# matpalm/cartpoleplusplus

Hardware: AMD Instinct MI355X
Metric: DDPG training steps/sec, 64x64x18 pixel obs, batch=256 (higher is better)
Workload: dtype f32-acc/f16x2,bf16x6

## Files before the change

### cartpoleplusplus_amd/_lib.py

```python
import ctypes as C
import os

import numpy as np

_HERE = os.path.dirname(os.path.abspath(__file__))
_variant = os.environ.get("CARTPOLEPP_ABLATION", "")
if _variant and not _variant.replace("_", "").isalnum():
    raise ImportError("cartpoleplusplus_amd: CARTPOLEPP_ABLATION=%r is not a build name" % _variant)
if _variant == "exact":
    raise ImportError("cartpoleplusplus_amd: CARTPOLEPP_ABLATION=exact names a build that no longer exists -- the exact-product "
                      "arithmetic is a mode of the release library (Context.set_precision('exact'), --exact-products, "
                      "bench.py --precision exact)")
LIB_PATH = os.path.join(_HERE, "lib", "libcartpolepp_hip%s.so" % (
    "" if _variant in ("", "0") else "_ablation" if _variant == "1" else "_" + _variant))

CPP_F32, CPP_F16, CPP_U8 = 0, 1, 2
CPP_ACTOR, CPP_CRITIC, CPP_HEAD = 0, 1, 2
CPP_OPT_SGD, CPP_OPT_MOMENTUM, CPP_OPT_ADAM = 0, 1, 2
CPP_PRECISION_FAST, CPP_PRECISION_EXACT = 0, 1


class NetSpec(C.Structure):
    _fields_ = [("kind", C.c_int32), ("pixel", C.c_int32), ("H", C.c_int32), ("W", C.c_int32),
                ("C", C.c_int32), ("state_elems", C.c_int32), ("action_dim", C.c_int32),
# ... 85 lines not shown
    "cpp_replay_set_n_step": (_I, [_P, _I, _F]),
    "cpp_replay_get_n_step": (_I, [_P, C.POINTER(_I), C.POINTER(_F)]),
    "cpp_replay_set_random_shift": (_I, [_P, _I, _I, _I, _U64]),
    "cpp_replay_get_random_shift": (_I, [_P, C.POINTER(_I), C.POINTER(_U64), C.POINTER(_U64)]),
    "cpp_replay_last_shifts": (_I, [_P, _I, _P]),
    "cpp_replay_gather_shifted": (_I, [_P, _I, _P, _I, _P]),
    "cpp_ddpg_create": (_I, [_P, _P, _P, _P, _P, C.POINTER(DdpgHyper), _PP]),
    "cpp_ddpg_destroy": (_I, [_P]),
    "cpp_ddpg_train_actor": (_I, [_P, _P]),
    "cpp_ddpg_train_critic": (_I, [_P, _P]),
    "cpp_ddpg_check_loss": (_I, [_P, _P, _P, _P, _P]),
    "cpp_ddpg_q_gradients_wrt_actions": (_I, [_P, _P, _P, _P, _P]),
    "cpp_ddpg_compute_gradients": (_I, [_P, _P]),
    "cpp_ddpg_grad_buffer": (_I, [_P, _PP, C.POINTER(_L)]),
    "cpp_ddpg_apply_gradients": (_I, [_P, _F]),
    "cpp_ddpg_update_targets": (_I, [_P]),
    "cpp_ddpg_set_optimiser": (_I, [_P, _I, _F, _F, _F, _F]),
    "cpp_ddpg_set_target_smoothing": (_I, [_P, _F, _F, _U64]),
    "cpp_ddpg_last_target_noise": (_I, [_P, _I, _P, C.POINTER(_U64)]),
    "cpp_ddpg_set_policy_delay": (_I, [_P, _I]),
    "cpp_ddpg_policy_delay_status": (_I, [_P, C.POINTER(_I), C.POINTER(_U64), C.POINTER(_I)]),
    "cpp_ddpg_opt_state_size": (_L, [_P]),
    "cpp_ddpg_get_opt_state": (_I, [_P, _P, _P, _L, _P]),
    "cpp_ddpg_set_opt_state": (_I, [_P, _P, _P, _L, _P]),
    "cpp_ddpg_train_step": (_I, [_P, _P, _I, _I, _P, _U64]),
    "cpp_ddpg_train_rows": (_I, [_P, _P, _I, _P]),
    "cpp_ddpg_sample_and_compute": (_I, [_P, _P, _I, _U64]),
    "cpp_ddpg_last_stats": (_I, [_P, _P]),
    "cpp_ddpg_last_values": (_I, [_P, _I, _P, _P, _P, _P]),
    "cpp_ddpg_last_twin_values": (_I, [_P, _I, _P, _P, _P, _P]),
    "cpp_ddpg_last_distribution": (_I, [_P, _I, _P, _P, _P]),
    "cpp_ddpg_set_quantile_target": (_I, [_P, C.c_float, _I]),
    "cpp_ddpg_last_quantiles": (_I, [_P, _I, _P, _P, _P]),
    "cpp_ddpg_set_sac": (_I, [_P, C.c_float, C.c_float, C.c_float, _U64]),
    "cpp_ddpg_last_sac": (_I, [_P, _I, _P, _P, _P, _P, _P, _P, _P, C.POINTER(C.c_float), C.POINTER(C.c_float), C.POINTER(_U64), _P]),
    "cpp_ddpg_sac_temperature": (_I, [_P, _I, C.POINTER(C.c_float), C.POINTER(C.c_float), C.POINTER(C.c_float), C.POINTER(_U64)]),
    "cpp_comm_unique_id": (_I, [_P, _I]),
    "cpp_comm_create": (_I, [_P, _P, _I, _I, _PP]),
    "cpp_comm_destroy": (_I, [_P]),
    "cpp_comm_info": (_I, [_P, C.POINTER(_I), C.POINTER(_I)]),
    "cpp_comm_allreduce": (_I, [_P, _P, _L, _I]),
    "cpp_comm_max_double": (_I, [_P, C.POINTER(C.c_double)]),
    "cpp_comm_max_doubles": (_I, [_P, C.POINTER(C.c_double), _I]),
    "cpp_comm_barrier": (_I, [_P]),
    "cpp_ddpg_allreduce_grads": (_I, [_P, _P]),
    "cpp_ddpg_average_params": (_I, [_P, _P]),
    "cpp_ddpg_dp_train_step": (_I, [_P, _P, _P, _I, _I, _U64, _I, _I]),
    "cpp_naf_sample_and_compute": (_I, [_P, _P, _I, _U64]),
    "cpp_naf_allreduce_grads": (_I, [_P, _P]),
    "cpp_naf_average_params": (_I, [_P, _P]),
    "cpp_naf_dp_train_step": (_I, [_P, _P, _P, _I, _I, _U64, _I]),
    "cpp_naf_clear_numeric_error": (_I, [_P]),
    "cpp_ddpg_dp_status": (_I, [_P, C.POINTER(_I), C.c_char_p, _I]),
    "cpp_naf_dp_status": (_I, [_P, C.POINTER(_I), C.c_char_p, _I]),
    "cpp_naf_create": (_I, [_P, _P, _P, _P, _P, _I, C.POINTER(NafHyper), _PP]),
    "cpp_naf_destroy": (_I, [_P]),
    "cpp_naf_action": (_I, [_P, _P, _I, _I, _P]),
    "cpp_naf_train": (_I, [_P, _P, C.POINTER(_F)]),
    "cpp_naf_debug_values": (_I, [_P, _P, _P, _P, _P, _P, _P]),
    "cpp_naf_compute_gradients": (_I, [_P, _P]),
    "cpp_naf_grad_buffer": (_I, [_P, _PP, C.POINTER(_L)]),
    "cpp_naf_apply_gradients": (_I, [_P, _F]),
    "cpp_naf_update_targets": (_I, [_P]),
    "cpp_naf_train_step": (_I, [_P, _P, _I, _I, _P, _U64]),
    "cpp_naf_train_rows": (_I, [_P, _P, _I, _P, C.POINTER(_F)]),
    "cpp_naf_train_rows_async": (_I, [_P, _P, _I, _P, C.POINTER(_U64)]),
    "cpp_naf_loss_wait": (_I, [_P, _U64, C.POINTER(_F)]),
    "cpp_naf_last_stats": (_I, [_P, _P]),
    "cpp_naf_opt_state_size": (_L, [_P]),
    "cpp_naf_get_opt_state": (_I, [_P, _P, _P, _L, C.POINTER(_U64)]),
    "cpp_naf_set_opt_state": (_I, [_P, _P, _P, _L, _U64]),
}


def _load():
    if not os.path.isfile(LIB_PATH):
        raise ImportError(
            "cartpoleplusplus_amd: %s not found. This package has no CPU fallback; build the HIP "
            "library first (python -c 'import __graft_entry__ as g; g.build()')." % LIB_PATH)
    lib = C.CDLL(LIB_PATH)
    for name, (res, args) in SIGNATURES.items():
        fn = getattr(lib, name)
        fn.restype, fn.argtypes = res, args
    if lib.cpp_abi_version() != 1:
        raise ImportError("cartpoleplusplus_amd: ABI version mismatch")
    return lib


lib = _load()


def check(rc):
    if rc != 0:
        raise RuntimeError((lib.cpp_last_error() or b"").decode("utf-8", "replace"))


def ptr(arr):
    if arr is None:
        return None
    assert arr.flags["C_CONTIGUOUS"]
    return arr.ctypes.data_as(C.c_void_p)


def as_state_array(x):
    x = np.asarray(x)
    if x.dtype == np.float16:
# ... 78 lines not shown
```

### cartpoleplusplus_amd/csrc/common.h

```cpp
#pragma once
#include <hip/hip_runtime.h>
#include <hip/hip_fp16.h>
#include <stdint.h>

typedef float f32x4 __attribute__((ext_vector_type(4)));

#ifdef CPP_ABLATION
#include <cstdlib>
inline bool cpp_switch_off(const char* name) { const char* v = getenv(name); return v != nullptr && atoi(v) == 0; }
inline bool cpp_switch_set(const char* name) { return getenv(name) != nullptr; }
inline int cpp_switch_int(const char* name, int dflt) { const char* v = getenv(name); return v ? atoi(v) : dflt; }
#else
constexpr bool cpp_switch_off(const char*) { return false; }
constexpr bool cpp_switch_set(const char*) { return false; }
constexpr int cpp_switch_int(const char*, int dflt) { return dflt; }
#endif

__host__ __device__ inline bool pair_grid_place(int i, int na, int nb, int order, int* idx) {
  if (order == 1) { if (i < nb) { *idx = i; return true; } *idx = i - nb; return false; }
  if (order == 2 && nb > 0 && na > 0) {
    const int k = (na + nb) / nb;
    const int head = nb * k;
    if (i < head) {
      if (i % k == 0) { *idx = i / k; return true; }
// ... 174 lines not shown
  const float* B; long sBk, sBn;
  float* C; long ldc;
  const float* Y; long ldy;
  int M, N, K, epi;
  int accumulate;
  float* C2; long ldc2;
  const uint64_t* drop_counter; uint32_t drop_seed, drop_layer;
  double* sq_part;
};
#define GEMM_BATCH_MAX 16
struct GemmBatch { GemmArgs g[GEMM_BATCH_MAX]; int tile_start[GEMM_BATCH_MAX + 1]; int n; };
#define CPP_MAX_DEVICES 16
static inline int cpp_dev_slot(const cpp_ctx* ctx) { return ctx->device >= 0 && ctx->device < CPP_MAX_DEVICES ? ctx->device : 0; }
#ifndef GEMM_SUB_MIN_K
#define GEMM_SUB_MIN_K 100000
#endif
static inline __host__ __device__ int gemm_sub(int M, int N, int K) { return (K >= GEMM_SUB_MIN_K && M > 16 && N > 16) ? 2 : 1; }
static inline int gemm_tiles(int M, int N, int K) { const int e = 16 * gemm_sub(M, N, K); return ((M + e - 1) / e) * ((N + e - 1) / e); }
int launch_gemm(cpp_ctx* ctx, const GemmArgs& g);
int launch_gemm_batch(cpp_ctx* ctx, const GemmArgs* list, int n);
int launch_copy_cols(cpp_ctx* ctx, float* dst, long ldd, int dcol0, const float* src, long lds_,
                     int scol0, int ncols, int rows);
int launch_fill(cpp_ctx* ctx, float* dst, long ld, int col0, int ncols, int rows, float v);
int launch_state_to_f32(cpp_ctx* ctx, float* dst, long ldd, const void* src, int dtype, long elems,
                        int rows);
int launch_actor_head_grad(cpp_ctx* ctx, float* dz, const float* dq_da, const float* act, int n);
int launch_td(cpp_ctx* ctx, const float* q, const float* tq, const float* r, const float* mask,
              float discount, int B, float* td, float* dq, float* loss, const float* w = nullptr);
int launch_td_twin(cpp_ctx* ctx, const float* q1, const float* q2, const float* tq1, const float* tq2, const float* r, const float* mask, float discount,
                   int B, float* td1, float* td2, float* dq1, float* dq2, float* loss, const float* w = nullptr);

struct GatherArgs {
  const void* store[2];
  const int32_t* s_idx[2];
  const int32_t* rows;
  int32_t* rows_out;
  const float* action; const float* reward; const float* mask;
  void* out_state[2];
  int32_t* out_slot[2];
  float* out_action; float* out_reward; float* out_mask;
  double* part;
  const double* slot_stats;
  uint64_t seed; const uint64_t* counter;
  int counter_add;
  const __half* lut;
  long elems; int B; int size; int action_dim; int C;
  const int32_t* size_ptr;
  const struct NStepWords* nstep;
  int rows_cap;
  struct ShiftWords* shift;
  int32_t* shifts_out;
  uint64_t shift_seed;
  int shift_pad, shift_H, shift_W, shift_C;
};
struct NStepWords { int32_t n; float discount; };
struct ShiftWords { uint64_t counter; uint32_t ticket; uint32_t reserved; };
constexpr int SHIFT_MAX_PAD = 16;
constexpr int NSTEP_MAX = 64;
int launch_gather_stats(cpp_ctx* ctx, const GatherArgs& a, int dtype);
int launch_slot_stats(cpp_ctx* ctx, const void* store, int dtype, long elems, int C, double* slot_stats, const int32_t* slots, int first, int n,
                      const __half* lut);
struct DwReduceBatch;
int launch_reduce_gather(cpp_ctx* ctx, const DwReduceBatch& rb, const GatherArgs& a, int dtype);
int launch_u8_to_f16(cpp_ctx* ctx, __half* dst, const uint8_t* src, long n, const __half* lut);
int launch_to_u8(cpp_ctx* ctx, uint8_t* dst, const void* src, int src_dtype, long n, const __half* lut, int* bad);
int launch_replay_fill_u8(cpp_ctx* ctx, uint8_t* store, long total, uint64_t seed);
struct BnNet {
  float* z;
  float* stat;
  const float* beta;
  float* pool; long pool_bstride; uint8_t* amax;
  const float* dpool; long dpool_bstride;
  double* part;
  float* means;
  float* dbeta;
};
struct BnBatch { BnNet n[CONV_BATCH_MAX]; int count; int B, H, W, C; };
size_t bn_part_doubles(int C);
int launch_bn_forward(cpp_ctx* ctx, const BnBatch& bb, double eps);
int launch_bn_backward(cpp_ctx* ctx, const BnBatch& bb);
void ctx_route_update(cpp_ctx* ctx);
int ctx_route_publish(cpp_ctx* ctx);
inline hipError_t ctx_sync_stream(cpp_ctx* ctx) {
  const hipError_t e = hipStreamSynchronize(ctx->stream);
  if (e == hipSuccess) ctx->route_done = ctx->route_calls;
  return e;
}
__device__ __forceinline__ void route_publish_device(unsigned* wmax_dev, const unsigned* tag_dev, unsigned long long* pin) {
  const unsigned m = *wmax_dev;
  *wmax_dev = 0u;
  const unsigned t = __hip_atomic_load(tag_dev, __ATOMIC_RELAXED, __HIP_MEMORY_SCOPE_SYSTEM);
  __hip_atomic_store(pin + (t & 1u), ((unsigned long long)t << 32) | (unsigned long long)m, __ATOMIC_RELAXED, __HIP_MEMORY_SCOPE_SYSTEM);
}
int launch_stats_finalize(cpp_ctx* ctx, const double* part, int nparts, int which_count, int C,
                          double count, float* white, double eps = 1e-6, uint64_t* bump = nullptr, unsigned* wmax = nullptr);
int launch_stats_generic(cpp_ctx* ctx, const void* x, int dtype, long npix, int C, float* white, double eps = 1e-6);
int launch_replay_fill(cpp_ctx* ctx, __half* store, long elems, int slots, int32_t* s1, int32_t* s2,
                       float* action, float* reward, float* mask, int rows, int action_dim,
                       uint64_t seed);
int launch_f32_to_f16(cpp_ctx* ctx, __half* dst, const float* src, long n);
int launch_counter_add(cpp_ctx* ctx, uint64_t* counter, uint64_t inc, const int* unless = nullptr);

enum OptKind { OPT_SGD = 0, OPT_MOMENTUM = 1, OPT_ADAM = 2 };
#define OPT_MAX_SEGS 4
struct OptSegs {
  float* p[OPT_MAX_SEGS]; const float* g[OPT_MAX_SEGS]; float* m[OPT_MAX_SEGS]; float* v[OPT_MAX_SEGS];
  long n[OPT_MAX_SEGS]; float lr[OPT_MAX_SEGS]; int group[OPT_MAX_SEGS];
  int nseg; int kind; float momentum, beta1, beta2, epsilon;
  const double* sq; int sq_begin[2], sq_count[2];
  const uint64_t* step;
  const uint64_t* step_seg[OPT_MAX_SEGS];
  uint64_t* bump;
  float* tgt[OPT_MAX_SEGS]; float tgt_coeff;
  unsigned* pub_wmax; const unsigned* pub_tag; unsigned long long* pub_pin;
  const int* skip_if;
  const double* st_part; float* st_white; int st_nparts, st_jobs, st_C; double st_count, st_eps; unsigned* st_wmax;
  int img_n; int img_cin;
  long img_skip[OPT_MAX_SEGS];
  struct { float* w; float* bias; const float* gw; const float* gb; unsigned char* rec; int seg, col, nout;
           const float* white; float* mw; float* mb; float* vw; float* vb; } img[4];
  uint64_t* bump2;
  const uint64_t* hold[OPT_MAX_SEGS];
};
__host__ __device__ inline float sgd_update(float p, float g, float scale, float lr) { return __builtin_fmaf(-lr, g * scale, p); }
__host__ __device__ inline float momentum_accum(float m, float g, float scale, float momentum) { return __builtin_fmaf(momentum, m, g * scale); }
__host__ __device__ inline float momentum_step(float p, float accum, float lr) { return __builtin_fmaf(-lr, accum, p); }
struct AdamElem { float p, m, v; };
__host__ __device__ inline AdamElem adam_update(float p, float g, float m, float v, float scale, float lr_t, float beta1, float beta2, float epsilon) {
  const float gi = g * scale;
  AdamElem e;
  e.m = __builtin_fmaf(beta1, m, (1.f - beta1) * gi);
  e.v = __builtin_fmaf(beta2, v, ((1.f - beta2) * gi) * gi);
  e.p = p - (lr_t * e.m) / (sqrtf(e.v) + epsilon);
  return e;
}
__host__ __device__ inline float adam_rate(float lr, float beta1, float beta2, uint64_t t) {
  const double td = (double)t;
  return (float)((double)lr * sqrt(1.0 - pow((double)beta2, td)) / (1.0 - pow((double)beta1, td)));
}
__host__ __device__ inline float soft_update_value(float t, float s, float coeff) { return __builtin_fmaf(-coeff, t - s, t); }
int launch_sumsq(cpp_ctx* ctx, const OptSegs& s, float grad_scale, double* part, int nparts);
int launch_opt_apply(cpp_ctx* ctx, const OptSegs& s, float grad_scale, float clip, const double* part,
                     int nparts, float* norms_out);
int launch_soft_update(cpp_ctx* ctx, float* t0, const float* s0, long n0, float* t1, const float* s1,
                       long n1, float coeff);

struct TpsArgs {
  const unsigned long long* n;
  float sigma, clip; unsigned seed_lo, seed_hi;
  float* eps;
  unsigned long long* n_out;
};
__device__ __forceinline__ float tps_noise(const TpsArgs& s, unsigned long long n, unsigned row, unsigned comp) {
  const u32x4 r = philox4x32_10(u32x4{row, 0x100u + comp, (uint32_t)n, (uint32_t)(n >> 32)}, s.seed_lo, s.seed_hi);
  const float u1 = (float)((r.x >> 8) + 1u) * 0x1p-24f;
  const float u2 = (float)(r.y >> 8) * 0x1p-24f;
  const float z = sqrtf(-2.f * logf(u1)) * cospif(2.f * u2);
  return fminf(fmaxf(s.sigma * z, -s.clip), s.clip);
}
__device__ __forceinline__ float tps_apply(float a, float eps) { return fminf(fmaxf(a + eps, -1.f), 1.f); }
int launch_tps_smooth(cpp_ctx* ctx, const TpsArgs& s, const float* in, int ld_in, float* out, int ld_out, int B, int A);

struct DdpgHeadsArgs {
  int B, A; float discount;
  const float *h2a, *h2ta; int ld_h2a, n2a;
  const float *Wo, *Wo_t;
  const float *h2c, *h2tc; int ld_h2c, n2c;
  const float *W3, *W3_t; int n3;
  const float *wq, *wq_t;
  const float *act, *r, *mask;
  float *a_out, *dq_da, *adz, *dz_h2a; int relu_x2;
  float* cat_splice;
  float* h3_out; int ld_h3;
  float *q_out, *tq_out, *td, *dzq, *dz3, *dz2c;
  double* loss_part;
// ... 131 lines not shown
```

### cartpoleplusplus_amd/csrc/conv_rs16.h

```cpp
#pragma once
#include "conv_k16.h"

template <int CIN, int NPCS = F16_PIECES>
struct Rs16Geom {
  static constexpr int KS = 5, P = 2, NO = KYO_NO, RK = 30;
  static constexpr int KROW = KS * CIN, NCH = (KROW + RK - 1) / RK, NPC = NPCS;
  static constexpr int NSET = KS + 1;
  static constexpr int NRC = 2 * P + 1;
  static constexpr int NUNIT = KS * NCH * 4 * 16;
  static constexpr int UNIT_BYTES = KS * NCH * NPC * 1024;
  static constexpr int CT_OFF = UNIT_BYTES;
  static constexpr int CT_BYTES = NRC * 5 * 16 * 4;
  static constexpr int PW_OFF = CT_OFF + CT_BYTES;
  static constexpr int PW_BYTES = NCH * 16 * 4;
  static constexpr int SC_OFF = PW_OFF + PW_BYTES;
  static constexpr int REC_BYTES = (SC_OFF + 16 + 255) & ~255;
};

struct Conv1ImageArgs {
  const float* w; const float* bias; const float* scale; const float* shift; float wscale; int nout; unsigned char* rec;
  const float* gw; const float* gb; float lr, gscale;
  float* mw; float* mb; float momentum;
  float* w_out; float* b_out;
  float* vw; float* vb; float beta1, beta2, epsilon;
};
struct Conv1ImageArgsN { Conv1ImageArgs a[CONV_BATCH_MAX]; int n; };

struct Conv1ImageNoPre { __device__ __forceinline__ float operator()(float gscale, float&) const { return gscale; } };
template <int CIN, int NPCS = F16_PIECES, typename Pre = Conv1ImageNoPre, bool ADAM = false>
__device__ __forceinline__ void conv1_image_body(const Conv1ImageArgs& a, unsigned char* lds_raw, Pre pre = Pre()) {
  typedef Rs16Geom<CIN, NPCS> G;
  constexpr int KS = G::KS, P = G::P, NO = G::NO, NCH = G::NCH, NPC = G::NPC, RK = G::RK;
  const int tid = threadIdx.x, lane = tid & 63, wave = tid >> 6;
  const int nout = a.nout;
  unsigned char* rec = lds_raw;
  double* mu = reinterpret_cast<double*>(lds_raw + G::REC_BYTES);
  constexpr int NU = KS * NCH * 4 * NO;
  double* opart = mu + ((CIN + 1) & ~1);
  constexpr int NB = 7 / CIN + 2;
  float* bpart = reinterpret_cast<float*>(opart + NU);
  float* scl = bpart + NU * NB;
  float* dmu = scl + CIN;
  float* red = dmu + CIN;
  float* ctab = red + 8;
  unsigned short* pivot = reinterpret_cast<unsigned short*>(ctab + G::NRC * NO * 4);
  constexpr int NUW = (NU + CONV_THREADS - 1) / CONV_THREADS;
  float* wst = reinterpret_cast<float*>(lds_raw);
  const int nwts = KS * G::KROW * nout;
  float gscale_b = a.gscale, lr = a.lr;
  {
    constexpr int NWT = (KS * G::KROW * NO + CONV_THREADS - 1) / CONV_THREADS;
    float wr[NWT], gr[NWT];
#pragma unroll
    for (int n = 0; n < NWT; ++n) { const int i = tid + n * CONV_THREADS; wr[n] = a.w[i < nwts ? i : 0]; }
    float mr[NWT];
    if (a.gw) {
#pragma unroll
      for (int n = 0; n < NWT; ++n) { const int i = tid + n * CONV_THREADS; gr[n] = a.gw[i < nwts ? i : 0]; }
      if (a.mw && !(ADAM && a.vw)) {
#pragma unroll
        for (int n = 0; n < NWT; ++n) { const int i = tid + n * CONV_THREADS; mr[n] = a.mw[i < nwts ? i : 0]; }
      }
    }
    const float gscale = pre(a.gscale, lr);
    gscale_b = gscale;
    if (ADAM && a.gw && a.vw) {
      float vr[NWT];
      int i0 = 0;
      asm volatile("" : "+v"(i0));
#pragma unroll
      for (int n = 0; n < NWT; ++n) { const int i = tid + n * CONV_THREADS; mr[n] = a.mw[i < nwts ? i : i0]; }
#pragma unroll
      for (int n = 0; n < NWT; ++n) { const int i = tid + n * CONV_THREADS; vr[n] = a.vw[i < nwts ? i : i0]; }
#pragma unroll
      for (int n = 0; n < NWT; ++n) {
        const int i = tid + n * CONV_THREADS;
        if (i < nwts) {
          const AdamElem e = adam_update(wr[n], gr[n], mr[n], vr[n], gscale, lr, a.beta1, a.beta2, a.epsilon);
          a.mw[i] = e.m; a.vw[i] = e.v;
          wst[i] = e.p;
          if (a.w_out) a.w_out[i] = e.p;
        }
        if ((n & 3) == 3) __builtin_amdgcn_sched_barrier(0);
      }
    } else {
#pragma unroll
    for (int n = 0; n < NWT; ++n) {
      const int i = tid + n * CONV_THREADS;
      if (i < nwts) {
        float w = wr[n];
        if (a.gw && a.mw) {
          const float acc = momentum_accum(mr[n], gr[n], gscale, a.momentum);
          a.mw[i] = acc;
          w = momentum_step(w, acc, lr);
        } else if (a.gw) w = sgd_update(w, gr[n], gscale, lr);
        wst[i] = w;
        if (a.gw && a.w_out) a.w_out[i] = w;
      }
    }
    }
  }
  __syncthreads();
  float wv[NUW][8];
  float vmax = 0.f;
#pragma unroll
  for (int n = 0; n < NUW; ++n) {
    const int u = tid + n * CONV_THREADS;
    const int o = u % NO, g = (u / NO) & 3, ch = (u / (4 * NO)) % NCH, ky = u / (4 * NO * NCH);
#pragma unroll
    for (int e = 0; e < 8; ++e) {
      const int kl = 8 * g + e, k = RK * ch + kl;
      const bool real = u < NU && o < nout && kl < RK && k < G::KROW;
      wv[n][e] = real ? wst[(ky * G::KROW + k) * nout + o] : 0.f;
    }
  }
  float* biasn = reinterpret_cast<float*>(pivot + ((CIN + 7) & ~7));
  if (tid < 16) {
    float bo = (a.bias && tid < nout) ? a.bias[tid] : 0.f;
    if (a.bias && a.gb && tid < nout) {
      if (ADAM && a.vb) { const AdamElem e = adam_update(bo, a.gb[tid], a.mb[tid], a.vb[tid], gscale_b, lr, a.beta1, a.beta2, a.epsilon); a.mb[tid] = e.m; a.vb[tid] = e.v; bo = e.p; }
      else if (a.mb) { const float acc = momentum_accum(a.mb[tid], a.gb[tid], gscale_b, a.momentum); a.mb[tid] = acc; bo = momentum_step(bo, acc, lr); }
      else bo = sgd_update(bo, a.gb[tid], gscale_b, lr);
      if (a.b_out) a.b_out[tid] = bo;
    }
    biasn[tid] = bo;
  }
  if (tid < CIN) {
    const float s_c = a.scale[tid], t_c = a.shift[tid];
    const double m_c = s_c != 0.f ? -(double)t_c / (double)s_c : 0.0;
    const _Float16 p_c = (_Float16)(float)m_c;
    mu[tid] = m_c;
    pivot[tid] = __builtin_bit_cast(unsigned short, p_c);
    scl[tid] = s_c;
    dmu[tid] = (float)((double)(float)p_c - m_c);
  }
  __syncthreads();
#pragma unroll
  for (int n = 0; n < NUW; ++n) {
    const int u = tid + n * CONV_THREADS;
    const int g = (u / NO) & 3, ch = (u / (4 * NO)) % NCH;
#pragma unroll
    for (int e = 0; e < 8; ++e) {
      float v = wv[n][e];
      v *= scl[(RK * ch + 8 * g + e) % CIN];
      if (a.wscale != 0.f) v *= a.wscale;
      wv[n][e] = v;
      vmax = fmaxf(vmax, fabsf(v));
    }
  }
  for (int o = 32; o > 0; o >>= 1) vmax = fmaxf(vmax, __shfl_xor(vmax, o));
  if (lane == 0) red[wave] = vmax;
  __syncthreads();
  vmax = fmaxf(fmaxf(red[0], red[1]), fmaxf(red[2], red[3]));
  for (int i = tid; i < G::REC_BYTES / 16; i += CONV_THREADS) reinterpret_cast<k16_u32x4*>(rec)[i] = (k16_u32x4){0u, 0u, 0u, 0u};
  __syncthreads();
  int S = 0;
  if (vmax > 0.f && vmax < 3.0e38f) S = 14 - ilogbf(vmax);
  S = S > 100 ? 100 : (S < -100 ? -100 : S);
  const float sc = ldexpf(1.f, S), inv = ldexpf(1.f, -S);
#pragma unroll
  for (int n = 0; n < NUW; ++n) {
    const int u = tid + n * CONV_THREADS;
    const int o = u % NO, g = (u / NO) & 3, ch = (u / (4 * NO)) % NCH, ky = u / (4 * NO * NCH);
    unsigned short pcs[3][8];
    double po = 0.0;
    float pb[NB];
#pragma unroll
    for (int b = 0; b < NB; ++b) pb[b] = 0.f;
    const int kx0 = (RK * ch + 8 * g) / CIN;
#pragma unroll
    for (int e = 0; e < 8; ++e) {
      const float v = wv[n][e] * sc;
      const _Float16 hh = (_Float16)v;
      const float r1 = v - (float)hh;
      const _Float16 mm = (_Float16)r1;
      const float r2 = r1 - (float)mm;
      const _Float16 ll = (_Float16)r2;
// ... 409 lines not shown
```

### cartpoleplusplus_amd/csrc/gather_body.h

```cpp
#pragma once
#include "common.h"
constexpr int GATHER_SH = 16;
constexpr int GATHER_LDS_BYTES = 256 * GATHER_SH * 4 + CPP_MAX_CHANNELS * 16 * 8 + 256 * 4;

__device__ __forceinline__ int sample_row(uint64_t seed, uint64_t counter, int b, int size) {
  u32x4 c = {(uint32_t)b, 0u, (uint32_t)counter, (uint32_t)(counter >> 32)};
  const u32x4 r = philox4x32_10(c, (uint32_t)seed, (uint32_t)(seed >> 32));
  return (int)(((uint64_t)r.x * (uint64_t)size) >> 32);
}

template <typename T> struct Vec8;
template <> struct Vec8<__half> {
  typedef __half Out;
  uint4 raw;
  __device__ void load(const __half* p) { raw = *reinterpret_cast<const uint4*>(p); }
  __device__ void store(__half* p) const { *reinterpret_cast<uint4*>(p) = raw; }
  __device__ float get(int e) const {
    const uint32_t w = e < 2 ? raw.x : (e < 4 ? raw.y : (e < 6 ? raw.z : raw.w));
    const unsigned short h = (e & 1) ? (unsigned short)(w >> 16) : (unsigned short)(w & 0xffffu);
    return __half2float(__ushort_as_half(h));
  }
};
template <> struct Vec8<uint8_t> {
  typedef __half Out;
// ... 129 lines not shown
      }
#pragma unroll
      for (int j = 0; j < NW; ++j) o[j] = __builtin_amdgcn_alignbit(m[j + 1], m[j], bits);
    }
    set_raw(x, o);
  }
  static __device__ __forceinline__ void set_raw(Vec8<__half>& x, const uint32_t* o) { x.raw = make_uint4(o[0], o[1], o[2], o[3]); }
  static __device__ __forceinline__ void set_raw(Vec8<uint8_t>& x, const uint32_t* o) { x.raw = make_uint2(o[0], o[1]); }
};

__device__ __forceinline__ void shift_draw(const GatherArgs& a, const int b, const int which, int* shw, int* dy, int* dx) {
  if (threadIdx.x == 0) {
    const uint64_t n = __hip_atomic_load(&a.shift->counter, __ATOMIC_RELAXED, __HIP_MEMORY_SCOPE_AGENT);
    u32x4 c = {(uint32_t)b, 2u + (uint32_t)which, (uint32_t)n, (uint32_t)(n >> 32)};
    const u32x4 r = philox4x32_10(c, (uint32_t)a.shift_seed, (uint32_t)(a.shift_seed >> 32));
    const uint64_t span = 2u * (uint32_t)a.shift_pad + 1u;
    const int y = (int)(((uint64_t)r.x * span) >> 32) - a.shift_pad, x = (int)(((uint64_t)r.y * span) >> 32) - a.shift_pad;
    shw[0] = y; shw[1] = x;
    a.shifts_out[((long)which * a.B + b) * 2] = y; a.shifts_out[((long)which * a.B + b) * 2 + 1] = x;
    const uint32_t ticket = __hip_atomic_fetch_add(&a.shift->ticket, 1u, __ATOMIC_ACQ_REL, __HIP_MEMORY_SCOPE_AGENT);
    if (ticket == 2u * (uint32_t)a.B - 1u) {
      __hip_atomic_store(&a.shift->counter, n + 1, __ATOMIC_RELAXED, __HIP_MEMORY_SCOPE_AGENT);
      __hip_atomic_store(&a.shift->ticket, 0u, __ATOMIC_RELAXED, __HIP_MEMORY_SCOPE_AGENT);
    }
  }
  __syncthreads();
  *dy = shw[0]; *dx = shw[1];
}

template <typename T, bool NSTEP = false, bool SHIFT = false>
__device__ __forceinline__ void gather_stats_body(const GatherArgs& a, const int b, const int which, float* sh, double* dsh, float* lut) {
  const int tid = threadIdx.x, lane = tid & 63, wave = tid >> 6;
  constexpr bool U8 = sizeof(T) == 1;
  if (U8) { lut[tid] = __half2float(a.lut[tid]); __syncthreads(); }
  typedef typename Vec8<T>::Out OutT;

  int row = 0, slot = 0;
  if (lane == 0) {
    if (a.s_idx[0] == nullptr) { row = b; slot = b; }
    else {
      row = a.rows ? a.rows[b] : sample_row(a.seed, (a.counter ? *a.counter : 0) + (uint64_t)a.counter_add, b, a.size_ptr ? *a.size_ptr : a.size);
      if (!NSTEP) slot = a.s_idx[which][row];
    }
  }
  row = __shfl(row, 0);
  slot = __shfl(slot, 0);
  float nreward = 0.f, nmask = 0.f;
  if (NSTEP && a.s_idx[0] != nullptr) nstep_walk(a, row, which, lane, &slot, &nreward, &nmask);
  int shift_dy = 0, shift_dx = 0;
  if constexpr (SHIFT) shift_draw(a, b, which, reinterpret_cast<int*>(dsh), &shift_dy, &shift_dx);

  if (tid == 0 && a.out_slot[which]) a.out_slot[which][b] = slot;
  if (which == 0 && a.s_idx[0] != nullptr) {
    if (tid == 0 && a.rows_out) a.rows_out[b] = row;
    if (tid < a.action_dim) a.out_action[(long)b * a.action_dim + tid] = a.action[(long)row * a.action_dim + tid];
    if (tid == 64) a.out_reward[b] = NSTEP ? nreward : a.reward[row];
    if (tid == 65) a.out_mask[b] = NSTEP ? nmask : a.mask[row];
  }

  const T* src = (const T*)a.store[which] + (long)slot * a.elems;
  OutT* dst = a.out_state[which] ? (OutT*)a.out_state[which] + (long)b * a.elems : nullptr;
  const long nvec = a.elems >> 3;
  const int C = a.C;

  if (a.slot_stats != nullptr && dst == nullptr && C > 0) {
    if (tid < 2 * C) a.part[((long)which * a.B + b) * 2 * C + tid] = a.slot_stats[(long)slot * 2 * C + tid];
    return;
  }

  if (C <= 0) {
    for (long v = tid; v < nvec; v += 256) { Vec8<T> x; vec_init(x, lut); x.load(src + v * 8); if (dst) x.store(dst + v * 8); }
    for (long e = nvec * 8 + tid; e < a.elems; e += 256) if (dst) dst[e] = elem_convert<T, OutT>(src[e], lut);
    return;
  }

  const int P = C / gcd_int(8, C);
  const int act = (64 / P) * P;
  double s[8], ss[8];
#pragma unroll
  for (int e = 0; e < 8; ++e) { s[e] = 0.0; ss[e] = 0.0; }
  if constexpr (SHIFT) {
    if (lane < act) {
      constexpr int GU = 6;
      ShiftGeom g;
      g.L = a.shift_W * a.shift_C; g.H = a.shift_H; g.C = a.shift_C; g.dy = shift_dy; g.dxC = shift_dx * a.shift_C; g.nvec = nvec;
#pragma unroll
      for (int e = 0; e < 8; ++e) g.ch[e] = (8 * (wave * act + lane) + e) % a.shift_C;
      long v = wave * act + lane;
      const long stride = 4 * act;
      for (; v + (GU - 1) * stride < nvec; v += GU * stride) {
        ShiftVec<T> s0, s1, s2, s3, s4, s5;
        static_assert(GU == 6, "one ShiftVec per vector in flight");
        s0.issue(src, g, v); s1.issue(src, g, v + stride); s2.issue(src, g, v + 2 * stride);
        s3.issue(src, g, v + 3 * stride); s4.issue(src, g, v + 4 * stride); s5.issue(src, g, v + 5 * stride);
        auto finish = [&](const ShiftVec<T>& sv, const long vo) __attribute__((always_inline)) {
          Vec8<T> x;
          vec_init(x, lut);
          sv.finish(x);
          x.store(dst + vo * 8);
#pragma unroll
          for (int e = 0; e < 8; ++e) { const double f = (double)x.get(e); s[e] += f; ss[e] = fma(f, f, ss[e]); }
        };
        finish(s0, v); finish(s1, v + stride); finish(s2, v + 2 * stride);
        finish(s3, v + 3 * stride); finish(s4, v + 4 * stride); finish(s5, v + 5 * stride);
      }
      for (; v < nvec; v += stride) {
        ShiftVec<T> sv;
// ... 67 lines not shown
```

### cartpoleplusplus_amd/csrc/optim.hip

```cpp
#include "common.h"
#include "stats_body.h"
#include "conv_rs16.h"

constexpr int OPT_THREADS = 256;
static_assert(OPT_THREADS == CONV_THREADS, "conv1_image_body (the rider in opt_apply_kernel) strides its loops by CONV_THREADS and assumes four waves");

__global__ __launch_bounds__(OPT_THREADS) void sumsq_kernel(const OptSegs s, float grad_scale,
                                                            double* part, int nparts) {
  __shared__ double red[OPT_THREADS];
  const int seg = blockIdx.y;
  const float* g = s.g[seg];
  const long n = s.n[seg];
  double acc = 0.0;
  const long stride = (long)nparts * OPT_THREADS;
  long i = (long)blockIdx.x * OPT_THREADS + threadIdx.x;
  for (; i + 7 * stride < n; i += 8 * stride) {
    float v[8];
#pragma unroll
    for (int u = 0; u < 8; ++u) v[u] = g[i + u * stride] * grad_scale;
#pragma unroll
    for (int u = 0; u < 8; ++u) acc += (double)v[u] * (double)v[u];
  }
  for (; i < n; i += stride) {
    const float v = g[i] * grad_scale;
    acc += (double)v * (double)v;
  }
  red[threadIdx.x] = acc;
  __syncthreads();
  for (int o = OPT_THREADS / 2; o > 0; o >>= 1) {
    if (threadIdx.x < o) red[threadIdx.x] += red[threadIdx.x + o];
    __syncthreads();
  }
  if (threadIdx.x == 0) part[seg * nparts + blockIdx.x] = red[0];
}

int launch_sumsq(cpp_ctx* ctx, const OptSegs& s, float grad_scale, double* part, int nparts) {
  prof_begin(ctx);
  hipLaunchKernelGGL(sumsq_kernel, dim3(nparts, s.nseg), dim3(OPT_THREADS), 0, ctx->stream, s, grad_scale,
                     part, nparts);
  LAUNCH_CHECK();
  prof_end(ctx, K_SUMSQ);
  return 0;
}

__device__ __forceinline__ double lane_sum_f64(const double* q, const int count, const int lane, double tot = 0.0) {
  for (int i = lane; i < count; i += 8 * 64) {
    double v[8];
#pragma unroll
    for (int u = 0; u < 8; ++u) { const int j = i + 64 * u; v[u] = q[j < count ? j : i]; }
#pragma unroll
    for (int u = 0; u < 8; ++u) tot += (i + 64 * u < count) ? v[u] : 0.0;
  }
  return tot;
}

template <bool ADAM>
__global__ __launch_bounds__(OPT_THREADS) void opt_apply_kernel(const OptSegs s, float grad_scale,
                                                                float clip, const double* part,
                                                                int nparts, float* norms_out) {
  __shared__ float sh_scale, sh_lr;
  const int seg = blockIdx.y;
  if (s.img_n > 0 && seg == s.nseg + (s.st_part ? 1 : 0)) {
    if ((int)blockIdx.x >= s.img_n) return;
    extern __shared__ __attribute__((aligned(16))) unsigned char img_lds[];
    __shared__ float wh[2 * CPP_MAX_CHANNELS];
    const int j = blockIdx.x, ws = s.img[j].seg;
    const float* const gwj = (s.hold[ws] && *s.hold[ws]) ? nullptr : s.img[j].gw;
    auto pre = [&](float, float& lr_io) __attribute__((always_inline)) -> float {
      if (gwj) {
        double tot = 0.0;
        if (threadIdx.x < 64) {
          if (s.sq) {
            const int gr = s.group[ws];
            const double* q = s.sq + s.sq_begin[gr];
            tot = lane_sum_f64(q, s.sq_count[gr], (int)threadIdx.x);
          } else {
            for (int k = 0; k < s.nseg; ++k)
              if (s.group[k] == s.group[ws])
                tot = lane_sum_f64(part + k * nparts, nparts, (int)threadIdx.x, tot);
          }
          for (int o = 32; o > 0; o >>= 1) tot += __shfl_xor(tot, o);
        }
        if (threadIdx.x == 0) {
          const float norm = (float)sqrt(tot);
          float sc = 1.f;
          if (clip > 0.f) sc = clip * fminf(1.f / norm, 1.f / clip);
          sh_scale = sc * grad_scale;
          if (ADAM) sh_lr = adam_rate(s.lr[ws], s.beta1, s.beta2, *(s.step_seg[ws] ? s.step_seg[ws] : s.step));
        }
      }
      if (s.img[j].white) {
        if ((int)threadIdx.x < 2 * s.img_cin) wh[threadIdx.x] = s.img[j].white[threadIdx.x];
      } else {
        constexpr int NW = OPT_THREADS / 64, MAXC = (18 + NW - 1) / NW, MAXR = 8;
        const int wv = (int)(threadIdx.x >> 6), ln = (int)(threadIdx.x & 63), C = s.st_C, np_ = s.st_nparts;
        if (np_ <= 64 * MAXR) {
          double v[MAXC][MAXR][2];
#pragma unroll
          for (int k = 0; k < MAXC; ++k) {
            const int c = wv + NW * k;
#pragma unroll
            for (int r = 0; r < MAXR; ++r) {
              const int b = ln + 64 * r;
              const bool ok = c < C && b < np_;
              const double* q = s.st_part + ((long)s.img[j].col * np_ + (ok ? b : 0)) * 2 * C;
              v[k][r][0] = ok ? q[c] : 0.0; v[k][r][1] = ok ? q[C + c] : 0.0;
            }
          }
#pragma unroll
          for (int k = 0; k < MAXC; ++k) {
            const int c = wv + NW * k;
            double a0 = 0.0, a1 = 0.0;
#pragma unroll
            for (int r = 0; r < MAXR; ++r) if (ln + 64 * r < np_) { a0 += v[k][r][0]; a1 += v[k][r][1]; }
            for (int o = 32; o > 0; o >>= 1) { a0 += __shfl_xor(a0, o); a1 += __shfl_xor(a1, o); }
            if (ln == 0 && c < C) white_from_moments(a0, a1, s.st_count, s.st_eps, &wh[c], &wh[C + c]);
          }
        } else {
          for (int c = wv; c < C; c += NW)
            stats_finalize_wave_to(s.st_part, np_, C, s.st_count, &wh[c], &wh[C + c], s.st_eps, s.img[j].col, c, ln);
        }
      }
      __syncthreads();
      if (ADAM && gwj) lr_io = sh_lr;
      return gwj ? sh_scale : 0.f;
    };
    Conv1ImageArgs ia;
    ia.w = s.img[j].w; ia.bias = s.img[j].bias; ia.scale = wh; ia.shift = wh + s.img_cin; ia.wscale = 0.f; ia.nout = s.img[j].nout; ia.rec = s.img[j].rec;
    ia.gw = gwj; ia.gb = s.img[j].gb; ia.lr = gwj ? s.lr[ws] : 0.f; ia.gscale = 0.f;
    ia.w_out = gwj ? s.img[j].w : nullptr; ia.b_out = gwj ? s.img[j].bias : nullptr;
    const bool slots = gwj && (ADAM || s.kind == OPT_MOMENTUM), adam = ADAM && gwj;
    ia.mw = slots ? s.img[j].mw : nullptr; ia.mb = slots ? s.img[j].mb : nullptr; ia.momentum = s.momentum;
    ia.vw = adam ? s.img[j].vw : nullptr; ia.vb = adam ? s.img[j].vb : nullptr; ia.beta1 = s.beta1; ia.beta2 = s.beta2; ia.epsilon = s.epsilon;
    switch (s.img_cin) {
      case 3: conv1_image_body<3, F16_PIECES, decltype(pre), ADAM>(ia, img_lds, pre); break;
      case 6: conv1_image_body<6, F16_PIECES, decltype(pre), ADAM>(ia, img_lds, pre); break;
      case 9: conv1_image_body<9, F16_PIECES, decltype(pre), ADAM>(ia, img_lds, pre); break;
      case 12: conv1_image_body<12, F16_PIECES, decltype(pre), ADAM>(ia, img_lds, pre); break;
      default: conv1_image_body<18, F16_PIECES, decltype(pre), ADAM>(ia, img_lds, pre); break;
    }
    return;
  }
  if (s.st_part && seg == s.nseg) {
    const int job = (int)blockIdx.x * (OPT_THREADS / 64) + (int)(threadIdx.x >> 6);
    if (job < s.st_jobs) stats_finalize_wave(s.st_part, s.st_nparts, s.st_C, s.st_count, s.st_white, s.st_eps, job, (int)(threadIdx.x & 63), s.st_wmax);
    return;
  }
  if (s.skip_if && *s.skip_if) return;
  double tot = 0.0;
  if (threadIdx.x < 64) {
    if (s.sq) {
      const int gr = s.group[seg];
      const double* q = s.sq + s.sq_begin[gr];
      tot = lane_sum_f64(q, s.sq_count[gr], (int)threadIdx.x);
    } else {
      for (int k = 0; k < s.nseg; ++k)
        if (s.group[k] == s.group[seg])
          tot = lane_sum_f64(part + k * nparts, nparts, (int)threadIdx.x, tot);
    }
    for (int o = 32; o > 0; o >>= 1) tot += __shfl_xor(tot, o);
  }
  if (threadIdx.x == 0) {
    const float norm = (float)sqrt(tot);
    float sc = 1.f;
    if (clip > 0.f) sc = clip * fminf(1.f / norm, 1.f / clip);
    sh_scale = sc * grad_scale;
    float lr = s.lr[seg];
    if (ADAM) lr = adam_rate(lr, s.beta1, s.beta2, *(s.step_seg[seg] ? s.step_seg[seg] : s.step));
    sh_lr = lr;
    if (blockIdx.x == 0 && norms_out && s.n[seg] > 0) norms_out[s.group[seg]] = norm;
    if (blockIdx.x == 0 && seg == 0 && s.bump) *s.bump += 1;
    if (blockIdx.x == 0 && seg == 0 && s.bump2) *s.bump2 += 1;
    if (blockIdx.x == 0 && seg == 0 && s.pub_wmax) route_publish_device(s.pub_wmax, s.pub_tag, s.pub_pin);
  }
  __syncthreads();
  const float sc = sh_scale, lr = sh_lr;
  const long skip = s.img_n > 0 ? s.img_skip[seg] : 0;
  float* p = s.p[seg] + skip;
  const float* g = s.g[seg] + skip;
  const long n = s.n[seg] - skip;
  const long stride = (long)gridDim.x * OPT_THREADS;
  float* tp = s.tgt[seg] ? s.tgt[seg] + skip : nullptr;
  const float tc = s.tgt_coeff;
  if (s.hold[seg] && *s.hold[seg]) {
    if (tp)
      for (long i = (long)blockIdx.x * OPT_THREADS + threadIdx.x; i < n; i += stride) tp[i] = soft_update_value(tp[i], p[i], tc);
    return;
  }
  if (!ADAM && s.kind == OPT_SGD) {
    long i = (long)blockIdx.x * OPT_THREADS + threadIdx.x;
    for (; i + 3 * stride < n; i += 4 * stride) {
      float pv[4], gv[4], tv[4];
#pragma unroll
      for (int u = 0; u < 4; ++u) { pv[u] = p[i + u * stride]; gv[u] = g[i + u * stride]; if (tp) tv[u] = tp[i + u * stride]; }
#pragma unroll
      for (int u = 0; u < 4; ++u) {
        const float pn = sgd_update(pv[u], gv[u], sc, lr);
        p[i + u * stride] = pn;
        if (tp) tp[i + u * stride] = soft_update_value(tv[u], pn, tc);
      }
    }
    for (; i < n; i += stride) {
      const float pn = sgd_update(p[i], g[i], sc, lr);
      p[i] = pn;
      if (tp) tp[i] = soft_update_value(tp[i], pn, tc);
    }
  } else if (!ADAM) {
    float* m = s.m[seg] + skip;
    for (long i = (long)blockIdx.x * OPT_THREADS + threadIdx.x; i < n; i += stride) {
      const float acc = momentum_accum(m[i], g[i], sc, s.momentum);
      m[i] = acc;
      const float pn = momentum_step(p[i], acc, lr);
      p[i] = pn;
      if (tp) tp[i] = soft_update_value(tp[i], pn, tc);
    }
  } else {
    float* m = s.m[seg] + skip;
    float* v = s.v[seg] + skip;
    const float b1 = s.beta1, b2 = s.beta2;
    long i = (long)blockIdx.x * OPT_THREADS + threadIdx.x;
    for (; i + 3 * stride < n; i += 4 * stride) {
      float pv[4], gv[4], mv[4], vv[4], tv[4];
#pragma unroll
      for (int u = 0; u < 4; ++u) {
        pv[u] = p[i + u * stride]; gv[u] = g[i + u * stride]; mv[u] = m[i + u * stride]; vv[u] = v[i + u * stride];
        if (tp) tv[u] = tp[i + u * stride];
      }
#pragma unroll
      for (int u = 0; u < 4; ++u) {
        const AdamElem e = adam_update(pv[u], gv[u], mv[u], vv[u], sc, lr, b1, b2, s.epsilon);
        m[i + u * stride] = e.m; v[i + u * stride] = e.v; p[i + u * stride] = e.p;
        if (tp) tp[i + u * stride] = soft_update_value(tv[u], e.p, tc);
      }
    }
    for (; i < n; i += stride) {
      const AdamElem e = adam_update(p[i], g[i], m[i], v[i], sc, lr, b1, b2, s.epsilon);
      m[i] = e.m; v[i] = e.v; p[i] = e.p;
      if (tp) tp[i] = soft_update_value(tp[i], e.p, tc);
    }
  }
}

static_assert(Rs16ImageLds<18>::BYTES >= Rs16ImageLds<12>::BYTES && Rs16ImageLds<18>::BYTES >= Rs16ImageLds<9>::BYTES &&
              Rs16ImageLds<18>::BYTES >= Rs16ImageLds<6>::BYTES && Rs16ImageLds<18>::BYTES >= Rs16ImageLds<3>::BYTES, "the rider's LDS is sized for the largest instance");
int launch_opt_apply(cpp_ctx* ctx, const OptSegs& s, float grad_scale, float clip, const double* part,
                     int nparts, float* norms_out) {
  prof_begin(ctx);
  const bool img = s.img_n > 0 && (s.st_part || s.img[0].white);
  const size_t lds = img ? (size_t)Rs16ImageLds<18>::BYTES : 0;
  if (img) {
    if ((s.kind != OPT_SGD && s.kind != OPT_MOMENTUM && s.kind != OPT_ADAM) || (s.st_part && s.st_C != s.img_cin) || !conv_rs16_channels_ok(s.img_cin) || s.skip_if) {
      cpp_set_error("opt_apply: the conv1 image rider needs a known optimiser kind and a channel count conv_rs16.h is instantiated for (%d)", s.img_cin); return 1;
    }
    static bool attr_done[CPP_MAX_DEVICES] = {};
    if (!attr_done[cpp_dev_slot(ctx)]) {
      HIP_CHECK(hipFuncSetAttribute((const void*)opt_apply_kernel<false>, hipFuncAttributeMaxDynamicSharedMemorySize, (int)Rs16ImageLds<18>::BYTES));
      HIP_CHECK(hipFuncSetAttribute((const void*)opt_apply_kernel<true>, hipFuncAttributeMaxDynamicSharedMemorySize, (int)Rs16ImageLds<18>::BYTES));
      attr_done[cpp_dev_slot(ctx)] = true;
    }
  }
  hipLaunchKernelGGL(s.kind == OPT_ADAM ? opt_apply_kernel<true> : opt_apply_kernel<false>, dim3(128, s.nseg + (s.st_part ? 1 : 0) + (img ? 1 : 0)), dim3(OPT_THREADS), lds, ctx->stream, s, grad_scale,
                     clip, part, nparts, norms_out);
  LAUNCH_CHECK();
  prof_end(ctx, K_CLIP_SGD);
  return 0;
}

__global__ void soft_update_kernel(float* t0, const float* s0, long n0, float* t1, const float* s1,
                                   long n1, float coeff, unsigned* wmax_dev, const unsigned* tag_dev, unsigned long long* pin) {
  if (wmax_dev && blockIdx.x == 0 && blockIdx.y == 0 && threadIdx.x == 0) route_publish_device(wmax_dev, tag_dev, pin);
  float* t = blockIdx.y == 0 ? t0 : t1;
  const float* s = blockIdx.y == 0 ? s0 : s1;
  const long n = blockIdx.y == 0 ? n0 : n1;
  for (long i = (long)blockIdx.x * blockDim.x + threadIdx.x; i < n; i += (long)gridDim.x * blockDim.x) t[i] = soft_update_value(t[i], s[i], coeff);
}

int launch_soft_update(cpp_ctx* ctx, float* t0, const float* s0, long n0, float* t1, const float* s1,
                       long n1, float coeff) {
  prof_begin(ctx);
  const bool pub = ctx->route_rider && ctx->route_pin_dev != nullptr;
  ctx->route_rider = false;
  hipLaunchKernelGGL(soft_update_kernel, dim3(128, t1 ? 2 : 1), dim3(256), 0, ctx->stream, t0, s0, n0,
                     t1, s1, n1, coeff, pub ? ctx->white_max_dev : nullptr, ctx->route_tag_dev, ctx->route_pin_dev);
  LAUNCH_CHECK();
  prof_end(ctx, K_SOFT_UPDATE);
  return 0;
}
```

### cartpoleplusplus_amd/csrc/rt_core.cpp

```cpp
#include "rt_internal.h"

static thread_local char g_err[1024] = "";

void cpp_set_error(const char* fmt, ...) {
  va_list ap;
  va_start(ap, fmt);
  vsnprintf(g_err, sizeof(g_err), fmt, ap);
  va_end(ap);
}

extern "C" const char* cpp_last_error(void) { return g_err; }

#include <map>
#include <mutex>
static std::mutex g_arena_mu;
static std::map<const char*, size_t> g_arena_blocks;
void cpp_arena_register(const void* raw, size_t bytes) {
  std::lock_guard<std::mutex> lk(g_arena_mu);
  g_arena_blocks[(const char*)raw] = bytes;
}
void cpp_arena_unregister(const void* raw) {
  std::lock_guard<std::mutex> lk(g_arena_mu);
  g_arena_blocks.erase((const char*)raw);
}
// ... 119 lines not shown
    *last_max_scale = m;
  }
  return CPP_OK;
}
extern "C" int cpp_ctx_set_precision(cpp_ctx* c, int mode) {
  ARG_CHECK(c, "cpp_ctx_set_precision: ctx is NULL");
  ARG_CHECK(mode == CPP_PRECISION_FAST || mode == CPP_PRECISION_EXACT, "cpp_ctx_set_precision: mode %d is neither CPP_PRECISION_FAST nor CPP_PRECISION_EXACT", mode);
  ARG_CHECK(c->n_trainers == 0 || mode == c->precision,
            "cpp_ctx_set_precision: %d trainer(s) exist on this ctx (their step graphs hold the kernels of the current mode): set the mode first", c->n_trainers);
  c->precision = mode;
  return CPP_OK;
}

extern "C" int cpp_ctx_get_precision(cpp_ctx* c, int* mode) {
  ARG_CHECK(c && mode, "cpp_ctx_get_precision: NULL argument");
  *mode = c->precision;
  return CPP_OK;
}

extern "C" int cpp_ctx_destroy(cpp_ctx* c) {
  if (!c) return CPP_OK;
  (void)hipSetDevice(c->device);
  (void)hipStreamSynchronize(c->stream);
  (void)hipEventDestroy(c->t0); (void)hipEventDestroy(c->t1);
  (void)hipEventDestroy(c->pe0); (void)hipEventDestroy(c->pe1);
  if (c->sq_part) (void)hipFree(c->sq_part);
  if (c->white_max_dev) (void)hipFree(c->white_max_dev);
  if (c->route_tag_dev) (void)hipFree(c->route_tag_dev);
  if (c->route_pin) { (void)hipHostFree(c->route_pin); for (hipEvent_t e : c->route_ev) (void)hipEventDestroy(e); }
  if (c->own_stream) (void)hipStreamDestroy(c->stream);
  delete c;
  return CPP_OK;
}

extern "C" int cpp_sync(cpp_ctx* c) {
  ARG_CHECK(c, "cpp_sync: ctx is NULL");
  HIP_CHECK(ctx_sync_stream(c));
  return CPP_OK;
}

void StepGraph::drop() {
  if (e) { (void)hipGraphExecDestroy(e); e = nullptr; }
  if (g) { (void)hipGraphDestroy(g); g = nullptr; }
  ok = false;
}
int StepGraph::capture(cpp_ctx* ctx, const GraphKey& k, const std::function<int()>& body) {
  drop();
  HIP_CHECK(hipStreamBeginCapture(ctx->stream, hipStreamCaptureModeThreadLocal));
  int rc = body();
  const hipError_t err = hipStreamEndCapture(ctx->stream, &g);
  if (!rc && err != hipSuccess) { cpp_set_error("hipStreamEndCapture -> %s", hipGetErrorString(err)); rc = CPP_ERR_HIP; }
  if (!rc) rc = [this]() -> int { HIP_CHECK(hipGraphInstantiate(&e, g, nullptr, nullptr, 0)); return CPP_OK; }();
  if (rc) { drop(); return rc; }
  key = k; ok = true;
  return CPP_OK;
}
int StepGraph::launch(cpp_ctx* ctx) {
  HIP_CHECK(hipGraphLaunch(e, ctx->stream));
  return CPP_OK;
}
int StepGraph::rebuild(cpp_ctx* ctx, const GraphKey& k, const std::function<int()>& body, StepRan* ran) {
  drop();
  RC(body());
  HIP_CHECK(ctx_sync_stream(ctx));
  const int rc = capture(ctx, k, body);
  *ran = rc ? STEP_CAPTURE_FAILED : STEP_CAPTURED;
  return rc;
}
int dp_graph_refused(DpGraph& D, const char* learner) {
  (void)hipGetLastError();
  D.graph.drop();
  D.refused = true;
  snprintf(D.reason, sizeof(D.reason), "%s", cpp_last_error());
  fprintf(stderr, "cartpolepp: the data-parallel %s step could not be captured as a hipGraph (%s); running it as stream launches\n", learner, D.reason);
  return CPP_OK;
}

extern "C" int cpp_timer_begin(cpp_ctx* c) {
  ARG_CHECK(c, "ctx is NULL");
  HIP_CHECK(hipEventRecord(c->t0, c->stream));
  return CPP_OK;
}
extern "C" int cpp_timer_end(cpp_ctx* c, float* ms) {
  ARG_CHECK(c && ms, "ctx/ms is NULL");
  HIP_CHECK(hipEventRecord(c->t1, c->stream));
  HIP_CHECK(hipEventSynchronize(c->t1));
  HIP_CHECK(hipEventElapsedTime(ms, c->t0, c->t1));
  return CPP_OK;
}
extern "C" int cpp_prof_enable(cpp_ctx* c, int on) { ARG_CHECK(c, "ctx is NULL"); c->prof = on != 0; return CPP_OK; }
extern "C" int cpp_prof_reset(cpp_ctx* c) {
  ARG_CHECK(c, "ctx is NULL");
  memset(c->prof_ms, 0, sizeof(c->prof_ms)); memset(c->prof_n, 0, sizeof(c->prof_n));
  return CPP_OK;
}
extern "C" int cpp_prof_num_kernels(void) { return K_NUM_KERNELS; }
extern "C" const char* cpp_prof_kernel_name(int k) { return (k >= 0 && k < K_NUM_KERNELS) ? kKernelNames[k] : ""; }
extern "C" int cpp_prof_read(cpp_ctx* c, int k, double* total_ms, int64_t* launches) {
  ARG_CHECK(c && k >= 0 && k < K_NUM_KERNELS, "cpp_prof_read: bad kernel id %d", k);
  if (total_ms) *total_ms = c->prof_ms[k];
  if (launches) *launches = c->prof_n[k];
  return CPP_OK;
}
```

### cartpoleplusplus_amd/csrc/rt_ddpg.cpp

```cpp
#include "rt_internal.h"


struct cpp_ddpg {
  cpp_ctx* ctx; cpp_net *actor, *critic, *tactor, *tcritic; cpp_ddpg_hyper hp;
  int maxB; long nA, nC;
  float* gradbuf; float *dq_da, *td, *dq, *loss_norms , *ones;
  double* norm_part;
  double* heads_part;
  int heads_grid, heads_B;
  int loss_parts, loss_B;
  StepGraph graph;
  cpp_batch* step_batch;
  StepGraph rgraph;
  uint64_t graph_gen = 0;
  uint64_t epoch;
  bool publish_in_apply;
  bool targets_in_apply, targets_applied;
  DpGraph dgraph;
  struct HalfGraphs { StepGraph g[3][2]; int next[3] = {0, 0, 0}; } hg[2];
  GraphKey half_key; uint64_t h_write_gen;
  uint64_t dp_local;
  int sq_cnt[2];
  int pre_variant;
  int32_t* slot_set[2][2];
  const float* per_w; std::function<int()> per_hook;
  int opt_kind; float opt_momentum, opt_beta1, opt_beta2, opt_epsilon;
  float *opt_m, *opt_v; uint64_t* opt_step;
  bool bump_in_heads;
  bool step_bumped;
  bool tps_on; float tps_sigma, tps_clip; uint64_t tps_seed; uint64_t* tps_n; float *tps_eps, *tps_act;
  bool tps_pending;
  int pd_d; uint64_t* pd;
  Arena arena;
  bool twin = false; float* td2 = nullptr;
  int dist_n = 0; float *dist_p = nullptr, *dist_tp = nullptr, *dist_m = nullptr;
  bool quant = false; float quant_kappa = 1.f; int quant_drop = 0;
  bool sac = false; float sac_hbar = 0.f, sac_lr = 0.f; uint64_t sac_seed = 0;
  float* sac_w = nullptr; uint64_t* sac_step = nullptr; double* sac_part = nullptr; int sac_B = 0;
  float *sac_eps[2] = {nullptr, nullptr}, *sac_logp[2] = {nullptr, nullptr}, *sac_rsoft = nullptr;
};

static SacSampleArgs sac_sample_args(const cpp_ddpg* d, bool target, bool draw, const cpp_batch* b = nullptr) {
  const cpp_net* n = target ? d->tactor : d->actor;
  SacSampleArgs s; memset(&s, 0, sizeof(s));
  s.logits = n->ws[0].logits; s.A = n->spec.action_dim; s.lo = n->ls_lo; s.hi = n->ls_hi;
  s.n = draw ? (const unsigned long long*)d->tps_n : nullptr;
  s.stream = target ? 0x300u : 0x200u; s.seed_lo = (unsigned)d->sac_seed; s.seed_hi = (unsigned)(d->sac_seed >> 32);
  s.eps = d->sac_eps[target ? 1 : 0]; s.a_out = n->ws[0].out; s.logp = d->sac_logp[target ? 1 : 0];
  if (target) {
    s.n_out = draw ? (unsigned long long*)(d->tps_n + 1) : nullptr;
    s.log_alpha = d->sac_w + SAC_W_TARGET; s.r = b->r; s.mask = b->m; s.discount = d->hp.discount; s.r_soft = d->sac_rsoft;
  }
  return s;
}
static SacGradArgs sac_grad_args(const cpp_ddpg* d, int B) {
  const cpp_net* a = d->actor;
  SacGradArgs g; memset(&g, 0, sizeof(g));
  g.logits = a->ws[0].logits; g.a = a->ws[0].out; g.eps = d->sac_eps[0]; g.dq_da = d->dq_da; g.logp = d->sac_logp[0];
  g.log_alpha = d->sac_w + SAC_W_LOG_ALPHA; g.B = B; g.A = a->spec.action_dim; g.lo = a->ls_lo; g.hi = a->ls_hi; g.target_entropy = d->sac_hbar;
  g.dz = a->ws[0].dz[a->fc.size() - 1]; g.part = d->sac_part; g.alpha_out = d->sac_w + SAC_W_ALPHA;
  return g;
}
static int sac_sync_target(cpp_ddpg* d) {
  hipStream_t st = d->ctx->stream;
  if (d->tactor != d->actor)
    HIP_CHECK(hipMemcpyAsync(d->tactor->params, d->actor->params, (size_t)d->nA * sizeof(float), hipMemcpyDeviceToDevice, st));
  HIP_CHECK(hipMemcpyAsync(d->sac_w + SAC_W_TARGET, d->sac_w + SAC_W_LOG_ALPHA, sizeof(float), hipMemcpyDeviceToDevice, st));
  d->tactor->wimg_key = nullptr;
  return CPP_OK;
}
static void reconfigured(cpp_ddpg* d);
static int sac_configure(cpp_ddpg* d, float init_temperature, float target_entropy, float lr, uint64_t seed) {
  cpp_ctx* ctx = d->ctx;
  HIP_CHECK(ctx_sync_stream(ctx));
  float w[SAC_WORDS]; memset(w, 0, sizeof(w));
  w[SAC_W_LOG_ALPHA] = w[SAC_W_TARGET] = logf(init_temperature); w[SAC_W_ALPHA] = init_temperature;
  HIP_CHECK(hipMemcpyAsync(d->sac_w, w, sizeof(w), hipMemcpyHostToDevice, ctx->stream));
// ... 3 lines not shown
  HIP_CHECK(ctx_sync_stream(ctx));
  d->sac_hbar = target_entropy; d->sac_lr = lr; d->sac_seed = seed; d->sac_B = 0; d->tps_pending = false;
  reconfigured(d);
  return CPP_OK;
}

static float loss_of_parts(const double* parts, int n, int B) {
  double s = 0.0;
  for (int i = 0; i < n; ++i) s += parts[i];
  return (float)(s / (double)B);
}

static int dist_td(cpp_ddpg* d, const cpp_batch* b, int B, bool backward, const float* w) {
  cpp_net *c = d->critic, *tc = d->tcritic;
  if (d->quant)
    return launch_quant_td(d->ctx, c->ws[0].logits, tc->ws[0].logits, b->r, b->m, d->hp.discount, B, d->dist_n, d->quant_kappa, d->quant_drop,
                           c->ws[0].out, tc->ws[0].out, d->dist_p, d->dist_tp, d->dist_m, d->td, backward ? c->ws[0].dz[c->fc.size() - 1] : nullptr,
                           d->heads_part, w);
  return launch_dist_td(d->ctx, c->ws[0].logits, tc->ws[0].logits, b->r, b->m, d->hp.discount, B, d->dist_n, c->dist_vmin, c->dist_vmax,
                        c->ws[0].out, tc->ws[0].out, d->dist_p, d->dist_tp, d->dist_m, d->td, backward ? c->ws[0].dz[c->fc.size() - 1] : nullptr,
                        d->heads_part, w);
}

extern "C" int cpp_ddpg_create(cpp_ctx* ctx, cpp_net* actor, cpp_net* critic, cpp_net* tactor, cpp_net* tcritic,
                               const cpp_ddpg_hyper* hp, cpp_ddpg** out) {
  ARG_CHECK(ctx && actor && critic && tactor && tcritic && hp && out, "cpp_ddpg_create: NULL argument");
  ARG_CHECK(actor->spec.kind == CPP_ACTOR && tactor->spec.kind == CPP_ACTOR, "cpp_ddpg_create: actor kinds");
  ARG_CHECK(critic->spec.kind == CPP_CRITIC && tcritic->spec.kind == CPP_CRITIC, "cpp_ddpg_create: critic kinds");
  ARG_CHECK(!actor->twin && !tactor->twin, "cpp_ddpg_create: a twin actor");
  ARG_CHECK(critic->twin == tcritic->twin, "cpp_ddpg_create: a twin critic needs a twin target critic (and a plain one a plain one)");
  ARG_CHECK(!actor->dist_n && !tactor->dist_n, "cpp_ddpg_create: a distributional actor");
  ARG_CHECK(critic->dist_n == tcritic->dist_n && critic->dist_vmin == tcritic->dist_vmin && critic->dist_vmax == tcritic->dist_vmax,
            "cpp_ddpg_create: critic and target critic must carry one value distribution (N, v_min, v_max), or none");
  ARG_CHECK(!(critic->dist_n && critic->twin), "cpp_ddpg_create: a distributional critic with twin Q heads");
  ARG_CHECK(critic->quant == tcritic->quant, "cpp_ddpg_create: a quantile critic needs a quantile target critic with the same N (never a categorical or a plain one)");
  ARG_CHECK(actor->gauss == tactor->gauss && actor->ls_lo == tactor->ls_lo && actor->ls_hi == tactor->ls_hi,
            "cpp_ddpg_create: a Gaussian actor needs a Gaussian target actor with the same log std bounds (and a plain one a plain one)");
  ARG_CHECK(!(actor->gauss && critic->dist_n), "cpp_ddpg_create: a Gaussian actor with a distributional or quantile critic");
  for (cpp_net* n : {actor, critic, tactor, tcritic})
    ARG_CHECK(!(actor->gauss && (n->spec.use_batch_norm || n->spec.use_dropout)), "cpp_ddpg_create: a Gaussian actor with batch norm or dropout");
  ARG_CHECK(actor->nparams == tactor->nparams && critic->nparams == tcritic->nparams, "cpp_ddpg_create: target shapes differ");
  ARG_CHECK(actor->state_elems == critic->state_elems && actor->spec.action_dim == critic->spec.action_dim,
            "cpp_ddpg_create: actor/critic input shapes differ");
  HIP_CHECK(hipSetDevice(ctx->device));
  cpp_ddpg* d = new cpp_ddpg();
  d->arena.stream = ctx->stream;
  d->ctx = ctx; d->actor = actor; d->critic = critic; d->tactor = tactor; d->tcritic = tcritic; d->hp = *hp;
  d->maxB = actor->maxB < critic->maxB ? actor->maxB : critic->maxB;
  d->nA = actor->nparams; d->nC = critic->nparams;
  d->step_batch = nullptr;
  d->epoch = ctx->kernel_epoch;
  d->dp_local = 0; d->sq_cnt[0] = d->sq_cnt[1] = 0;
  d->h_write_gen = 0; d->pre_variant = 0;
  memset(d->slot_set, 0, sizeof(d->slot_set));
  d->heads_grid = d->heads_B = d->loss_parts = d->loss_B = 0;
  d->per_w = nullptr;
  d->opt_kind = OPT_SGD; d->opt_momentum = 0.f; d->opt_beta1 = 0.9f; d->opt_beta2 = 0.999f; d->opt_epsilon = 1e-8f;
  d->opt_m = d->opt_v = nullptr; d->opt_step = nullptr; d->bump_in_heads = d->step_bumped = false;
  d->pd_d = 1; d->pd = nullptr;
  d->tps_on = d->tps_pending = false; d->tps_sigma = d->tps_clip = 0.f; d->tps_seed = 0; d->tps_n = nullptr; d->tps_eps = d->tps_act = nullptr;
  const int A = actor->spec.action_dim;
  int rc = dalloc(d->arena, &d->gradbuf, (size_t)(d->nA + d->nC));
  if (!rc) rc = dalloc(d->arena, &d->dq_da, (size_t)d->maxB * A);
  if (!rc) rc = dalloc(d->arena, &d->td, (size_t)d->maxB);
  if (!rc) rc = dalloc(d->arena, &d->dq, (size_t)d->maxB);
  if (!rc) rc = dalloc(d->arena, &d->ones, (size_t)d->maxB);
  if (!rc) rc = dalloc(d->arena, &d->loss_norms, (size_t)4);
  if (!rc) rc = dalloc(d->arena, &d->norm_part, (size_t)OPT_MAX_SEGS * NORM_PARTS);
  if (!rc) rc = dalloc(d->arena, &d->heads_part, (size_t)DDPG_HEADS_MAX_WGS);
  d->twin = critic->twin;
  if (!rc && d->twin) rc = dalloc(d->arena, &d->td2, (size_t)d->maxB);
  d->dist_n = critic->dist_n; d->quant = critic->quant;
  if (d->dist_n && dist_td_grid(d->maxB) > DDPG_HEADS_MAX_WGS) {
    cpp_set_error("cpp_ddpg_create: a distributional trainer takes batches up to %d (got %d)", 4 * DDPG_HEADS_MAX_WGS, d->maxB);
    rc = CPP_ERR_ARG;
  }
  for (float** p : {&d->dist_p, &d->dist_tp, &d->dist_m})
    if (!rc && d->dist_n) rc = dalloc(d->arena, p, (size_t)d->maxB * d->dist_n);
  d->sac = actor->gauss;
  if (d->sac && sac_grid(d->maxB) > DDPG_HEADS_MAX_WGS) {
    cpp_set_error("cpp_ddpg_create: a soft actor-critic trainer takes batches up to %d (got %d)", 4 * DDPG_HEADS_MAX_WGS, d->maxB);
    rc = CPP_ERR_ARG;
  }
  if (d->sac) {
    if (!rc) rc = dalloc(d->arena, &d->sac_w, (size_t)SAC_WORDS);
    if (!rc) rc = dalloc(d->arena, &d->sac_step, (size_t)1);
    if (!rc) rc = dalloc(d->arena, &d->tps_n, (size_t)2);
    if (!rc) rc = dalloc(d->arena, &d->sac_part, (size_t)DDPG_HEADS_MAX_WGS);
    if (!rc) rc = dalloc(d->arena, &d->sac_rsoft, (size_t)d->maxB);
    for (int k = 0; k < 2; ++k) {
      if (!rc) rc = dalloc(d->arena, &d->sac_eps[k], (size_t)d->maxB * A);
      if (!rc) rc = dalloc(d->arena, &d->sac_logp[k], (size_t)d->maxB);
    }
    if (!rc) rc = sac_configure(d, 0.1f, -(float)A, 1e-4f, 0);
  }
  if (!rc) rc = launch_fill(ctx, d->ones, 1, 0, 1, d->maxB, 1.0f);
  if (rc) { d->arena.release(); delete d; return rc; }
  actor->grads = d->gradbuf; critic->grads = d->gradbuf + d->nA;
  HIP_CHECK(ctx_sync_stream(ctx));
  ctx->n_trainers += 1;
  *out = d;
  return CPP_OK;
}

static void invalidate_graphs(cpp_ddpg* d) { ++d->graph_gen; }
static void reconfigured(cpp_ddpg* d) { invalidate_graphs(d); d->pre_variant = 0; }

static void after_replay(cpp_ddpg* d, bool step) {
  if (step) d->pre_variant = 0;
  d->loss_parts = d->heads_grid; d->loss_B = d->heads_B;
}
static int step_ran(cpp_ddpg* d, int rc, StepRan how) {
  if (!rc && how == STEP_REPLAYED) after_replay(d, true);
  return rc;
}

static void route_check(cpp_ddpg* d) {
  if (route_check(d->ctx, &d->epoch, &d->graph_gen, {d->actor, d->critic, d->tactor, d->tcritic})) d->pre_variant = 0;
}

extern "C" int cpp_ddpg_destroy(cpp_ddpg* d) {
  if (!d) return CPP_OK;
  (void)hipSetDevice(d->ctx->device);
  (void)ctx_sync_stream(d->ctx);
  if (d->step_batch) cpp_batch_destroy(d->step_batch);
  d->actor->grads = nullptr; d->critic->grads = nullptr;
  d->ctx->n_trainers -= 1;
  d->arena.release(); delete d; return CPP_OK;
}

static int check_batch(cpp_ddpg* d, cpp_batch* b, const char* who) {
  ARG_CHECK(d && b, "%s: NULL argument", who);
  ARG_CHECK(b->B >= 1 && b->B <= d->maxB, "%s: batch size %d outside [1,%d]", who, b->B, d->maxB);
  ARG_CHECK(b->elems == d->actor->state_elems && b->A == d->actor->spec.action_dim, "%s: batch shape does not match the networks", who);
  return CPP_OK;
}

static TpsArgs tps_args(const cpp_ddpg* d) {
  TpsArgs t; memset(&t, 0, sizeof(t));
  if (!d->tps_on) return t;
  t.n = (const unsigned long long*)d->tps_n; t.n_out = (unsigned long long*)(d->tps_n + 1); t.eps = d->tps_eps;
  t.sigma = d->tps_sigma; t.clip = d->tps_clip; t.seed_lo = (unsigned)d->tps_seed; t.seed_hi = (unsigned)(d->tps_seed >> 32);
  return t;
}
static int tps_settle(cpp_ddpg* d, int rc) {
  const bool owed = d->tps_pending;
  d->tps_pending = false;
  if (rc) return rc;
  return owed ? launch_counter_add(d->ctx, d->tps_n, 1) : CPP_OK;
}

const float* white_of(cpp_batch* b, int which, int C) { return b->white + (long)which * 2 * C; }

static int critic_prefix(cpp_net* c, const void* state, int dtype, const float* white, int B) {
  RC(net_forward_trunk(c, c->ws[0], state, dtype, white, B));
  if (c->cat_layer > 0) {
    for (int l = 0; l < c->cat_layer; ++l) {
      const FcL& L = c->fc[l];
      RC(gemm(c->ctx, c->ws[0].fcin[l], L.n_in + 1, 1, c->params + L.w_off, L.n_out, 1, c->ws[0].fcin[l + 1],
              c->fc[l + 1].n_in + 1, B, L.n_out, L.n_in + 1, L.act));
    }
  }
// ... 53 lines not shown
static int critic_gradients(cpp_ddpg* d, cpp_batch* b, bool critic_prefix_done, bool backward) {
  cpp_net* nets[3] = {d->critic, d->tactor, d->tcritic};
  for (cpp_net* n : nets) n->is_training = backward;
  const int rc = critic_gradients_impl(d, b, critic_prefix_done, backward);
  for (cpp_net* n : nets) n->is_training = true;
  return rc;
}
static int critic_gradients_impl(cpp_ddpg* d, cpp_batch* b, bool critic_prefix_done, bool backward) {
  cpp_net *c = d->critic, *ta = d->tactor, *tc = d->tcritic;
  const int B = b->B, C = c->spec.pixel ? c->spec.C : 0;
  const float *w1 = white_of(b, 0, C), *w2 = white_of(b, 1, C);
  RC(net_forward_trunk(ta, ta->ws[0], b->s[1], b->dtype, w2, B));
  RC(net_forward_fc(ta, ta->ws[0], 0, B, nullptr));
  RC(critic_prefix(tc, b->s[1], b->dtype, w2, B));
  const float* tact = ta->ws[0].out;
  if (d->sac) {
    SacSampleArgs st = sac_sample_args(d, true, backward, b); st.B = B;
    RC(launch_sac_sample(d->ctx, st));
    if (backward) d->tps_pending = true;
  }
  const float* rw = d->sac ? d->sac_rsoft : b->r;
  if (backward && d->tps_on) {
    const int A = ta->spec.action_dim;
    RC(launch_tps_smooth(d->ctx, tps_args(d), tact, A, d->tps_act, A, B, A));
    tact = d->tps_act;
    d->tps_pending = true;
  }
  RC(critic_head(tc, 0, tact, B));
  if (!critic_prefix_done) RC(critic_prefix(c, b->s[0], b->dtype, w1, B));
  RC(critic_head(c, 0, b->a, B));
  const int last = (int)c->fc.size() - 1;
  if (d->dist_n) {
    RC(dist_td(d, b, B, backward, nullptr));
    d->loss_parts = dist_td_grid(B); d->loss_B = B;
    if (backward) RC(net_backward(c, c->ws[0], B, true, nullptr, b->s[0], b->dtype, w1));
    return CPP_OK;
  }
  if (d->twin)
    RC(launch_td_twin(d->ctx, c->ws[0].out, c->ws[0].out2, tc->ws[0].out, tc->ws[0].out2, rw, b->m, d->hp.discount, B, d->td, d->td2,
                      backward ? c->ws[0].dz[last] : nullptr, backward ? c->ws[0].dz2[last] : nullptr, d->loss_norms));
  else
  RC(launch_td(d->ctx, c->ws[0].out, tc->ws[0].out, rw, b->m, d->hp.discount, B, d->td,
               backward ? c->ws[0].dz[last] : nullptr, d->loss_norms));
  d->loss_parts = 0;
  if (backward) RC(net_backward(c, c->ws[0], B, true, nullptr, b->s[0], b->dtype, w1));
  return CPP_OK;
}

static int apply(cpp_ddpg* d, bool do_actor, bool do_critic, float grad_scale, uint64_t* bump = nullptr, bool folded = false,
                 const NextBatch& nx = NextBatch()) {
  OptSegs s; memset(&s, 0, sizeof(s));
  s.bump = bump;
  if (d->tps_pending) { s.bump2 = d->tps_n; d->tps_pending = false; }
  if (d->targets_in_apply && !nx.b && do_actor && do_critic) {
    s.tgt[0] = d->tactor->params; s.tgt[1] = d->tcritic->params; s.tgt_coeff = d->hp.target_update_rate;
    d->tactor->wimg_key = nullptr; d->tcritic->wimg_key = nullptr;
    d->targets_applied = true;
  }
  d->targets_in_apply = false;
  if (d->publish_in_apply && !nx.b && d->ctx->route_pin_dev) {
    s.pub_wmax = d->ctx->white_max_dev; s.pub_tag = d->ctx->route_tag_dev; s.pub_pin = d->ctx->route_pin_dev;
  }
  d->publish_in_apply = false;
  opt_next_stats(d->ctx, s, nx);
  d->actor->wimg_key = nullptr; d->critic->wimg_key = nullptr;
  s.nseg = 2; s.kind = d->opt_kind;
  const bool bumped = d->step_bumped;
  d->step_bumped = false;
  const bool pd_on = d->pd_d > 1;
  if (pd_on && do_actor) s.hold[0] = d->pd + PD_HOLD;
  if (pd_on && !bumped)
    RC(launch_pd_tick(d->ctx, d->pd, (unsigned)d->pd_d, s.kind != OPT_SGD ? d->opt_step : nullptr, do_actor, do_critic, do_actor && !do_critic));
  if (s.kind != OPT_SGD) {
    s.momentum = d->opt_momentum; s.beta1 = d->opt_beta1; s.beta2 = d->opt_beta2; s.epsilon = d->opt_epsilon;
    s.m[0] = d->opt_m; s.m[1] = d->opt_m + d->nA; s.v[0] = d->opt_v; s.v[1] = d->opt_v ? d->opt_v + d->nA : nullptr;
    s.step_seg[0] = d->opt_step; s.step_seg[1] = d->opt_step + 1;
    if (!bumped && !pd_on) {
      if (do_actor) RC(launch_counter_add(d->ctx, d->opt_step, 1));
      if (do_critic) RC(launch_counter_add(d->ctx, d->opt_step + 1, 1));
    }
  }
  s.p[0] = d->actor->params; s.g[0] = d->gradbuf; s.n[0] = do_actor ? d->nA : 0; s.lr[0] = d->hp.actor_learning_rate; s.group[0] = 0;
  s.p[1] = d->critic->params; s.g[1] = d->gradbuf + d->nA; s.n[1] = do_critic ? d->nC : 0; s.lr[1] = d->hp.critic_learning_rate; s.group[1] = 1;
  if (folded && do_actor && do_critic && grad_scale == 1.0f && d->sq_cnt[0] > 0 && d->sq_cnt[1] > 0) {
    s.sq = d->ctx->sq_part; s.sq_begin[0] = 0; s.sq_begin[1] = SQ_REGION; s.sq_count[0] = d->sq_cnt[0]; s.sq_count[1] = d->sq_cnt[1];
  } else {
    RC(launch_sumsq(d->ctx, s, grad_scale, d->norm_part, NORM_PARTS));
  }
  cpp_net* inets[4] = {d->actor, d->critic, d->tactor, d->tcritic};
  const ConvL* L0 = d->actor->spec.pixel ? &d->actor->conv[0] : nullptr;
  static const bool no_img = cpp_switch_off("CPP_RIDE_IMAGE_UPDATE");
  const bool img = nx.b && nx.C > 0 && do_actor && do_critic && L0 && !d->actor->spec.use_batch_norm && !d->critic->spec.use_batch_norm &&
                   conv_rs16_ok(d->ctx, L0->Cin, L0->H, L0->W, kConvOut) && nx.B >= 2 && !no_img &&
                   conv1_opens_params(d->actor) && conv1_opens_params(d->critic);
  if (img) {
    s.img_n = 4; s.img_cin = L0->Cin;
    for (int j = 0; j < 4; ++j) {
      opt_img_net(s, j, inets[j], j < 2 ? j : -1, j < 2 ? 0 : 1, nx);
      const ConvL& L = inets[j]->conv[0];
      if (j < 2 && s.kind != OPT_SGD) { s.img[j].mw = s.m[j] + L.w_off; s.img[j].mb = s.m[j] + L.b_off; }
      if (j < 2 && s.kind == OPT_ADAM) { s.img[j].vw = s.v[j] + L.w_off; s.img[j].vb = s.v[j] + L.b_off; }
    }
  }
  if (d->sac && do_actor && d->sac_lr > 0.f && d->sac_B > 0) RC(launch_sac_temperature(d->ctx, d->sac_part, d->sac_B, d->sac_lr, d->sac_w, d->sac_step));
  RC(launch_opt_apply(d->ctx, s, grad_scale, d->hp.gradient_clip, d->norm_part, NORM_PARTS, d->loss_norms + 1));
  opt_img_built(s, inets, nx);
  if (d->sac && do_critic) RC(sac_sync_target(d));
  return CPP_OK;
}

static int prep_batch(cpp_ddpg* d, cpp_batch* b) {
  if (d->actor->spec.pixel) RC(batch_ensure_stats(b, d->actor->spec.C));
  return CPP_OK;
}

extern "C" int cpp_ddpg_train_actor(cpp_ddpg* d, cpp_batch* b) {
  RC(check_batch(d, b, "cpp_ddpg_train_actor"));
  HIP_CHECK(hipSetDevice(d->ctx->device));
  RC(prep_batch(d, b));
  RC(actor_gradients(d, b, false));
  RC(apply(d, true, false, 1.0f));
  return CPP_OK;
}

extern "C" int cpp_ddpg_train_critic(cpp_ddpg* d, cpp_batch* b) {
  RC(check_batch(d, b, "cpp_ddpg_train_critic"));
  HIP_CHECK(hipSetDevice(d->ctx->device));
  RC(prep_batch(d, b));
  const int rc = critic_gradients(d, b, false, true);
  if (rc) { d->tps_pending = false; return rc; }
  RC(apply(d, false, true, 1.0f));
  return CPP_OK;
}

extern "C" int cpp_ddpg_check_loss(cpp_ddpg* d, cpp_batch* b, float* loss, float* td, float* q) {
  RC(check_batch(d, b, "cpp_ddpg_check_loss"));
  HIP_CHECK(hipSetDevice(d->ctx->device));
  RC(prep_batch(d, b));
  RC(critic_gradients(d, b, false, false));
  double parts[DDPG_HEADS_MAX_WGS];
  const int nparts = d->dist_n ? d->loss_parts : 0;
  const size_t nB = (size_t)b->B * sizeof(float);
  RC(read_back(d->ctx, {{loss && nparts ? parts : nullptr, d->heads_part, (size_t)nparts * sizeof(double)}, {nparts ? nullptr : loss, d->loss_norms, sizeof(float)},
                        {td, d->td, nB}, {q, d->critic->ws[0].out, nB}}));
  if (loss && nparts) *loss = loss_of_parts(parts, nparts, d->loss_B);
  return CPP_OK;
}

extern "C" int cpp_ddpg_q_gradients_wrt_actions(cpp_ddpg* d, cpp_batch* b, float* dq_da, float* actions, float* q) {
  RC(check_batch(d, b, "cpp_ddpg_q_gradients_wrt_actions"));
  HIP_CHECK(hipSetDevice(d->ctx->device));
  RC(prep_batch(d, b));
  RC(actor_gradients(d, b, false, false));
  const size_t nB = (size_t)b->B * sizeof(float), nA = nB * d->actor->spec.action_dim;
  return read_back(d->ctx, {{dq_da, d->dq_da, nA}, {actions, d->actor->ws[0].out, nA}, {q, d->critic->ws[1].out, nB}});
// ... 317 lines not shown
  if (n) *n = w[PD_N];
  if (held) *held = (d->pd_d > 1 && w[PD_HOLD]) ? 1 : 0;
  return CPP_OK;
}

extern "C" int cpp_ddpg_last_target_noise(cpp_ddpg* d, int B, float* eps, uint64_t* n) {
  ARG_CHECK(d, "cpp_ddpg_last_target_noise: NULL argument");
  ARG_CHECK(B >= 1 && B <= d->maxB, "cpp_ddpg_last_target_noise: batch %d outside [1,%d]", B, d->maxB);
  if (!d->tps_on) { cpp_set_error("cpp_ddpg_last_target_noise: target policy smoothing is off"); return CPP_ERR_STATE; }
  HIP_CHECK(hipSetDevice(d->ctx->device));
  return read_back(d->ctx, {{eps, d->tps_eps, (size_t)B * d->actor->spec.action_dim * sizeof(float)}, {n, d->tps_n + 1, sizeof(uint64_t)}}, true);
}

extern "C" int64_t cpp_ddpg_opt_state_size(const cpp_ddpg* d) { return d ? (int64_t)(d->nA + d->nC) : -1; }
extern "C" int cpp_ddpg_get_opt_state(cpp_ddpg* d, float* m, float* v, int64_t n, uint64_t steps[2]) {
  ARG_CHECK(d && steps, "cpp_ddpg_get_opt_state: NULL argument");
  ARG_CHECK(d->opt_kind != OPT_SGD, "cpp_ddpg_get_opt_state: GradientDescent has no slots");
  ARG_CHECK(n == d->nA + d->nC, "cpp_ddpg_get_opt_state: asked %ld values, the optimisers have %ld", (long)n, d->nA + d->nC);
  HIP_CHECK(hipSetDevice(d->ctx->device));
  return read_back(d->ctx, {{m, d->opt_m, (size_t)n * sizeof(float)}, {d->opt_kind == OPT_ADAM ? v : nullptr, d->opt_v, (size_t)n * sizeof(float)},
                            {steps, d->opt_step, 2 * sizeof(uint64_t)}}, true);
}
extern "C" int cpp_ddpg_set_opt_state(cpp_ddpg* d, const float* m, const float* v, int64_t n, const uint64_t steps[2]) {
  ARG_CHECK(d && m && steps, "cpp_ddpg_set_opt_state: NULL argument");
  ARG_CHECK(d->opt_kind != OPT_SGD, "cpp_ddpg_set_opt_state: GradientDescent has no slots");
  ARG_CHECK(d->opt_kind != OPT_ADAM || v, "cpp_ddpg_set_opt_state: Adam needs v");
  ARG_CHECK(n == d->nA + d->nC, "cpp_ddpg_set_opt_state: got %ld values, the optimisers have %ld", (long)n, d->nA + d->nC);
  HIP_CHECK(hipSetDevice(d->ctx->device));
  hipStream_t st = d->ctx->stream;
  HIP_CHECK(hipMemcpyAsync(d->opt_m, m, (size_t)n * sizeof(float), hipMemcpyHostToDevice, st));
  if (d->opt_kind == OPT_ADAM) HIP_CHECK(hipMemcpyAsync(d->opt_v, v, (size_t)n * sizeof(float), hipMemcpyHostToDevice, st));
  HIP_CHECK(hipMemcpyAsync(d->opt_step, steps, 2 * sizeof(uint64_t), hipMemcpyHostToDevice, st));
  HIP_CHECK(ctx_sync_stream(d->ctx));
  return CPP_OK;
}

extern "C" int cpp_ddpg_update_targets(cpp_ddpg* d) {
  ARG_CHECK(d, "cpp_ddpg_update_targets: NULL argument");
  HIP_CHECK(hipSetDevice(d->ctx->device));
  d->tactor->wimg_key = nullptr; d->tcritic->wimg_key = nullptr;
  return launch_soft_update(d->ctx, d->tactor->params, d->actor->params, d->nA, d->tcritic->params, d->critic->params,
                            d->nC, d->hp.target_update_rate);
}

bool direct_replay_ok(cpp_net* a, cpp_replay* r, int B) {
  static const bool off = cpp_switch_off("CPP_DIRECT_REPLAY");
  if (off || !a->spec.pixel || r->store_dtype != CPP_F16 || r->shift_pad > 0) return false;
  const int C = a->spec.C;
  int g = 8, c = C; while (c) { int t = g % c; g = c; c = t; }
  if (r->elems % 8 != 0 || C / g > 16 || r->elems % C != 0) return false;
  return conv1_f16_pipes_ok(a->ctx, C, a->conv[0].H, a->conv[0].W, B, a->spec.use_batch_norm != 0);
}

static int step_body(cpp_ddpg* d, cpp_replay* r, int B, int n_batches, const int32_t* rows_dev, uint64_t seed, bool targets = true,
                     bool dp = false, cpp_comm* comm = nullptr) {
  d->pre_variant = 0;
  cpp_ctx* ctx = d->ctx;
  MinibatchLoop L;
  L.ctx = ctx; L.r = r; L.step_batch = d->step_batch; L.trunk = d->actor;
  L.per_w = &d->per_w; L.per_hook = &d->per_hook; L.td = d->td; L.stats_switch = true;
  L.gradients = [=] {
    d->bump_in_heads = true;
    const int rc = compute_gradients(d, d->step_batch);
    d->bump_in_heads = false;
    if (rc) { d->step_bumped = false; d->tps_pending = false; }
    return rc;
  };
  L.apply = [=](bool more, const NextBatch& next) {
    if (dp) RC(step_allreduce(ctx, comm, d->gradbuf, (size_t)(d->nA + d->nC)));
    static const bool no_tgt_ride = cpp_switch_off("CPP_RIDE_TARGETS");
    d->targets_applied = false;
    d->targets_in_apply = !more && targets && !dp && !no_tgt_ride;
    d->publish_in_apply = !more && (!targets || d->targets_in_apply);
    return apply(d, true, true, (dp && comm) ? 1.0f / (float)comm->world : 1.0f, rows_dev ? nullptr : r->counter, !dp, next);
  };
  RC(run_minibatches(L, B, n_batches, rows_dev, seed));
  if (targets && d->targets_applied) { d->targets_applied = false; return CPP_OK; }
  if (targets) { ctx->route_rider = true; return cpp_ddpg_update_targets(d); }
  return CPP_OK;
}

extern "C" int cpp_ddpg_train_rows(cpp_ddpg* d, cpp_replay* r, int B, const int32_t* idxs) {
  ARG_CHECK(d && r && idxs, "cpp_ddpg_train_rows: NULL argument");
  RC(train_entry_checks("cpp_ddpg_train_rows", r, B, d->maxB, d->actor->state_elems, d->actor->spec.action_dim, d->hp.discount));
  route_check(d);
  cpp_ctx* ctx = d->ctx;
  HIP_CHECK(hipSetDevice(ctx->device));
  if (!d->step_batch) RC(cpp_batch_create(ctx, d->maxB, r->elems, r->A, &d->step_batch));
  RC(replay_stage_rows(r, idxs, B, "cpp_ddpg_train_rows"));
  static const bool no_graph = cpp_switch_set("CPP_NO_GRAPH");
  StepRan how;
  const int rc = run_step_graph(ctx, d->rgraph, GraphKey{B, 1, 0, r->uid, 0, d->graph_gen}, [&] { return step_body(d, r, B, 1, r->rows_in, 0, false); }, &how, no_graph);
  return step_ran(d, rc, how);
}

extern "C" int cpp_ddpg_train_step(cpp_ddpg* d, cpp_replay* r, int B, int n_batches, const int32_t* idxs, uint64_t seed) {
  ARG_CHECK(d && r, "cpp_ddpg_train_step: NULL argument");
  RC(train_entry_checks("cpp_ddpg_train_step", r, B, d->maxB, d->actor->state_elems, d->actor->spec.action_dim, d->hp.discount, &n_batches));
  route_check(d);
  cpp_ctx* ctx = d->ctx;
  HIP_CHECK(hipSetDevice(ctx->device));
  if (!d->step_batch) RC(cpp_batch_create(ctx, d->maxB, r->elems, r->A, &d->step_batch));
  if (idxs) {
    RC(replay_upload_rows(r, idxs, n_batches * B, "cpp_ddpg_train_step"));
    return step_body(d, r, B, n_batches, r->rows_in, seed);
  }
  static const bool no_graph = cpp_switch_set("CPP_NO_GRAPH");
  StepRan how;
  const int rc = run_step_graph(ctx, d->graph, GraphKey{B, n_batches, seed, r->uid, 0, d->graph_gen}, [&] { return step_body(d, r, B, n_batches, nullptr, seed); }, &how, no_graph);
  return step_ran(d, rc, how);
}

static int half_step_body(cpp_ddpg* d, cpp_replay* r, int B, uint64_t seed, int variant, int* next, int phase) {
  const int C = d->actor->spec.pixel ? d->actor->spec.C : 0;
  cpp_ctx* ctx = d->ctx;
  cpp_batch* b = d->step_batch;
  const bool direct = direct_replay_ok(d->actor, r, B);
  static const bool no_ride = cpp_switch_off("CPP_RIDE_DP");
  const int cur = variant == 1 ? 1 : 0;
  for (int k = 0; k < 2; ++k) { b->slot[k] = d->slot_set[cur][k]; b->slot_alt[k] = d->slot_set[1 - cur][k]; }
  int Cg = 0;
  GatherArgs ga = replay_gather_args(r, B, nullptr, seed, r->counter, C, b, direct, &Cg);
  if (phase != 2) {
    if (variant == 0) RC(launch_gather_stats(ctx, ga, r->store_dtype));
    bool bumped = false;
    RC(replay_sample_finish(r, B, Cg, C, b, r->counter, &bumped));
    if (!bumped) RC(launch_counter_add(ctx, r->counter, 1));
  }
  if (phase == 1) return tps_settle(d, compute_gradients(d, b, 1));
  const bool ride_ok = !no_ride && direct && Cg > 0 && r->store_dtype == CPP_F16;
  int rc;
  {
    RideScope ride(ctx);
    if (ride_ok) ride.arm(&ga, b, r->store_dtype, true, true);
    rc = tps_settle(d, compute_gradients(d, b, phase));
    *next = ride.rode() ? (cur == 0 ? 1 : 2) : 0;
  }
  if (rc) return rc;
  return ctx_route_publish(ctx);
}

static int half_step(cpp_ddpg* d, cpp_replay* r, int B, uint64_t seed, bool split, const std::function<int()>& between) {
  cpp_ctx* ctx = d->ctx;
  if (!d->step_batch) RC(cpp_batch_create(ctx, d->maxB, r->elems, r->A, &d->step_batch));
  if (d->slot_set[0][0] == nullptr)
    for (int k = 0; k < 2; ++k) { d->slot_set[0][k] = d->step_batch->slot[k]; d->slot_set[1][k] = d->step_batch->slot_alt[k]; }
  const GraphKey key{B, 0, seed, r->uid, 0, d->graph_gen};
  if (!(d->half_key == key)) {
    for (auto& F : d->hg) for (auto& variant : F.g) for (StepGraph& g : variant) g.drop();
    d->pre_variant = 0;
    d->half_key = key;
  }
  if (d->h_write_gen != r->write_gen) { d->pre_variant = 0; d->h_write_gen = r->write_gen; }
  cpp_ddpg::HalfGraphs& H = d->hg[split ? 1 : 0];
  const int v = d->pre_variant;
  d->pre_variant = 0;
  auto eager = [&](int variant, int* nx) -> int {
    if (!split) return half_step_body(d, r, B, seed, variant, nx, 0);
    RC(half_step_body(d, r, B, seed, variant, nx, 1));
    if (between) RC(between());
    return half_step_body(d, r, B, seed, variant, nx, 2);
  };
  const int parts = split ? 2 : 1;
  auto capture = [&](int variant, int* nx) -> int {
    for (int k = 0; k < parts; ++k)
      RC(H.g[variant][k].capture(ctx, key, [&] { return half_step_body(d, r, B, seed, variant, nx, split ? k + 1 : 0); }));
    return CPP_OK;
  };
  int next = 0;
  if (ctx->prof) { RC(eager(v, &next)); d->pre_variant = next; return CPP_OK; }
  if (!H.g[v][parts - 1].hit(key)) {
    int nx = 0;
    if (v == 0) {
      RC(eager(0, &next));
      HIP_CHECK(ctx_sync_stream(ctx));
      RC(capture(0, &nx));
      H.next[0] = nx;
      d->pre_variant = next;
      return CPP_OK;
    }
    HIP_CHECK(ctx_sync_stream(ctx));
    RC(capture(v, &nx));
    H.next[v] = nx;
  }
  RC(H.g[v][0].launch(ctx));
  if (split) {
    if (between) RC(between());
    RC(H.g[v][1].launch(ctx));
  }
  after_replay(d, false);
  d->pre_variant = H.next[v];
  return CPP_OK;
}

static int sac_refuse(const cpp_ddpg* d, const char* who) {
  ARG_CHECK(!(d && d->sac), "%s: a soft actor-critic trainer has no data-parallel step (the temperature's gradient is not in the reduced buffer)", who);
// ... 54 lines not shown
  HIP_CHECK(hipSetDevice(ctx->device));
  const float inv = c ? 1.0f / (float)c->world : 1.0f;
  const long fa = fc_start(d->actor), fcr = fc_start(d->critic);
  static const bool no_dp_graph = cpp_switch_off("CPP_DP_GRAPH");
  if (sync_every == 1 && !overlap && !no_dp_graph) {
    if (!d->step_batch) RC(cpp_batch_create(ctx, d->maxB, r->elems, r->A, &d->step_batch));
    StepRan how;
    const int rc = run_dp_graph(ctx, d->dgraph, GraphKey{B, n_batches, seed, r->uid, c ? c->uid : 0, d->graph_gen}, "DDPG",
                                [&] { return step_body(d, r, B, n_batches, nullptr, seed, true, true, c); }, &how);
    return step_ran(d, rc, how);
  }
  for (int i = 0; i < n_batches; ++i) {
    if (sync_every > 1) {
      RC(half_step(d, r, B, seed, false, nullptr));
      RC(apply(d, true, true, 1.0f));
      if (++d->dp_local >= (uint64_t)sync_every && c) RC(cpp_ddpg_average_params(d, c));
      continue;
    }
    if (c && overlap) {
      RC(half_step(d, r, B, seed, true, [&]() -> int {
        HIP_CHECK(hipEventRecord(c->ev_fc, ctx->stream));
        HIP_CHECK(hipStreamWaitEvent(c->side, c->ev_fc, 0));
        NCCL_CHECK(ncclGroupStart());
        NCCL_CHECK(ncclAllReduce(d->gradbuf + fa, d->gradbuf + fa, (size_t)(d->nA - fa), ncclFloat, ncclSum, c->comm, c->side));
        NCCL_CHECK(ncclAllReduce(d->gradbuf + d->nA + fcr, d->gradbuf + d->nA + fcr, (size_t)(d->nC - fcr), ncclFloat, ncclSum, c->comm, c->side));
        NCCL_CHECK(ncclGroupEnd());
        return CPP_OK; }));
      HIP_CHECK(hipEventRecord(c->ev_bwd, ctx->stream));
      HIP_CHECK(hipStreamWaitEvent(c->side, c->ev_bwd, 0));
      if (fa > 0 || fcr > 0) {
        NCCL_CHECK(ncclGroupStart());
        if (fa > 0) NCCL_CHECK(ncclAllReduce(d->gradbuf, d->gradbuf, (size_t)fa, ncclFloat, ncclSum, c->comm, c->side));
        if (fcr > 0) NCCL_CHECK(ncclAllReduce(d->gradbuf + d->nA, d->gradbuf + d->nA, (size_t)fcr, ncclFloat, ncclSum, c->comm, c->side));
        NCCL_CHECK(ncclGroupEnd());
      }
      HIP_CHECK(hipEventRecord(c->ev_done, c->side));
      HIP_CHECK(hipStreamWaitEvent(ctx->stream, c->ev_done, 0));
    } else {
      RC(half_step(d, r, B, seed, false, nullptr));
      if (c) RC(cpp_ddpg_allreduce_grads(d, c));
    }
    RC(apply(d, true, true, inv));
  }
  return cpp_ddpg_update_targets(d);
}

extern "C" int cpp_ddpg_dp_status(const cpp_ddpg* d, int* mode, char* reason, int cap) {
  ARG_CHECK(d && mode, "cpp_ddpg_dp_status: NULL argument");
  *mode = d->dgraph.mode(d->graph_gen);
  if (reason && cap > 0) snprintf(reason, (size_t)cap, "%s", d->dgraph.reason);
  return CPP_OK;
}

extern "C" int cpp_ddpg_last_stats(cpp_ddpg* d, float out[3]) {
  ARG_CHECK(d && out, "cpp_ddpg_last_stats: NULL argument");
  double parts[DDPG_HEADS_MAX_WGS];
  RC(read_back(d->ctx, {{out, d->loss_norms, 3 * sizeof(float)}, {d->loss_parts > 0 ? parts : nullptr, d->heads_part, (size_t)d->loss_parts * sizeof(double)}}, true));
  if (d->loss_parts > 0) out[0] = loss_of_parts(parts, d->loss_parts, d->loss_B);
  return CPP_OK;
}

extern "C" int cpp_ddpg_last_values(cpp_ddpg* d, int B, float* actions, float* dq_da, float* q, float* td) {
  ARG_CHECK(d, "cpp_ddpg_last_values: NULL argument");
  ARG_CHECK(B >= 1 && B <= d->maxB, "cpp_ddpg_last_values: batch %d outside [1,%d]", B, d->maxB);
  HIP_CHECK(hipSetDevice(d->ctx->device));
  const size_t nB = (size_t)B * sizeof(float), nA = nB * d->actor->spec.action_dim;
  return read_back(d->ctx, {{actions, d->actor->ws[0].out, nA}, {dq_da, d->dq_da, nA}, {q, d->critic->ws[0].out, nB}, {td, d->td, nB}});
}


extern "C" int cpp_ddpg_last_twin_values(cpp_ddpg* d, int B, float* q2, float* target_q1, float* target_q2, float* td2) {
  ARG_CHECK(d, "cpp_ddpg_last_twin_values: NULL argument");
  ARG_CHECK(B >= 1 && B <= d->maxB, "cpp_ddpg_last_twin_values: batch %d outside [1,%d]", B, d->maxB);
  if (!d->twin) { cpp_set_error("cpp_ddpg_last_twin_values: the trainer's critics are not twin critics"); return CPP_ERR_STATE; }
  HIP_CHECK(hipSetDevice(d->ctx->device));
  const size_t n = (size_t)B * sizeof(float);
  return read_back(d->ctx, {{q2, d->critic->ws[0].out2, n}, {target_q1, d->tcritic->ws[0].out, n}, {target_q2, d->tcritic->ws[0].out2, n}, {td2, d->td2, n}});
}

extern "C" int cpp_ddpg_set_quantile_target(cpp_ddpg* d, float kappa, int drop_top) {
  ARG_CHECK(d, "cpp_ddpg_set_quantile_target: NULL argument");
  if (!d->quant) { cpp_set_error("cpp_ddpg_set_quantile_target: the trainer's critics are not quantile critics"); return CPP_ERR_STATE; }
  ARG_CHECK(std::isfinite(kappa) && kappa > 0.f, "cpp_ddpg_set_quantile_target: kappa %g (finite, positive)", (double)kappa);
  ARG_CHECK(drop_top >= 0 && drop_top <= d->dist_n - 1, "cpp_ddpg_set_quantile_target: %d dropped atoms outside [0, %d]", drop_top, d->dist_n - 1);
  HIP_CHECK(hipSetDevice(d->ctx->device));
  HIP_CHECK(ctx_sync_stream(d->ctx));
  d->quant_kappa = kappa; d->quant_drop = drop_top;
  reconfigured(d);
  return CPP_OK;
}

extern "C" int cpp_ddpg_last_quantiles(cpp_ddpg* d, int B, float* theta, float* sorted_target_theta, float* y) {
  ARG_CHECK(d, "cpp_ddpg_last_quantiles: NULL argument");
  ARG_CHECK(B >= 1 && B <= d->maxB, "cpp_ddpg_last_quantiles: batch %d outside [1,%d]", B, d->maxB);
  if (!d->quant) { cpp_set_error("cpp_ddpg_last_quantiles: the trainer's critics are not quantile critics"); return CPP_ERR_STATE; }
  HIP_CHECK(hipSetDevice(d->ctx->device));
  const size_t n = (size_t)B * d->dist_n * sizeof(float);
  return read_back(d->ctx, {{theta, d->dist_p, n}, {sorted_target_theta, d->dist_tp, n}, {y, d->dist_m, n}});
}

extern "C" int cpp_ddpg_last_distribution(cpp_ddpg* d, int B, float* p, float* target_p, float* m) {
  ARG_CHECK(d, "cpp_ddpg_last_distribution: NULL argument");
  ARG_CHECK(B >= 1 && B <= d->maxB, "cpp_ddpg_last_distribution: batch %d outside [1,%d]", B, d->maxB);
  if (!d->dist_n || d->quant) { cpp_set_error("cpp_ddpg_last_distribution: the trainer's critics are not distributional"); return CPP_ERR_STATE; }
  HIP_CHECK(hipSetDevice(d->ctx->device));
  const size_t n = (size_t)B * d->dist_n * sizeof(float);
// ... 60 lines not shown
```

### cartpoleplusplus_amd/csrc/rt_internal.h

```cpp
#pragma once
#include "../../include/cartpolepp_abi.h"
#include "common.h"

#include <cmath>
#include <cstdarg>
#include <cstdio>
#include <cstdlib>
#include <cstring>
#include <functional>
#include <string>
#include <vector>
#include <algorithm>

#include <rccl/rccl.h>

#define ARG_CHECK(cond, ...)                \
  do {                                      \
    if (!(cond)) {                          \
      cpp_set_error(__VA_ARGS__);           \
      return CPP_ERR_ARG;                   \
    }                                       \
  } while (0)
#define RC(expr)                  \
  do {                            \
// ... 42 lines not shown
  std::vector<float*> fcin2, dz2;
  float* out2 = nullptr;
  float* logits = nullptr;
};

struct cpp_net {
  cpp_ctx* ctx; cpp_net_spec spec; int maxB;
  std::vector<ConvL> conv; std::vector<FcL> fc; std::vector<VarInfo> vars;
  long nparams; int flat; int cat_layer; long state_elems;
  float* params; float* grads; float* own_grads;
  Workspace ws[2];
  bool use_b16;
  void* wimg;
  const float* wimg_key;
  const int32_t* img_slot;
  float* white;
  float* white_rows;
  double* stats_part;
  float* dw_partial[3];
  bool is_training;
  uint64_t* drop_counter;
  double* bn_part; float* bn_means; float* bn_scratch;
  void* stage_state; float* stage_action; float* stage_out;
  Arena arena;
  bool twin = false; std::vector<FcL> fc2;
  int dist_n = 0; float dist_vmin = 0.f, dist_vmax = 0.f;
  bool quant = false;
  bool gauss = false; float ls_lo = 0.f, ls_hi = 0.f; float* gauss_stage = nullptr;
};

struct cpp_batch {
  cpp_ctx* ctx; int maxB, B; long elems; int A; int dtype;
  void* s[2]; float *a, *r, *m;
  float* white;
  double* part;
  int stats_C;
  int32_t* slot[2]; const void* direct_store;
  int32_t* slot_alt[2];
  Arena arena;
};

#define CPP_ROWS_RING 8
#define CPP_ROWS_RING_SLOT 4096
struct cpp_replay {
  cpp_ctx* ctx; int rows, slots, A, size; long elems;
  int store_dtype;
  void* store; int32_t *s1, *s2, *rows_in, *rows_out; float *action, *reward, *mask;
  uint64_t* counter;
  uint64_t* counter_adhoc;
  int32_t* size_dev;
  uint64_t uid;
  bool sampled;
  uint64_t write_gen;
  __half* lut; int* bad; uint16_t lut_host[256];
  double* slot_stats; int stats_C, stats_cap; int32_t* slot_list; size_t slot_list_cap;
  void* stage; size_t stage_cap;
  void* pinned; size_t pinned_cap; hipEvent_t pinned_free; bool pinned_busy;
  int32_t* rows_pin; hipEvent_t rows_pin_ev[CPP_ROWS_RING]; bool rows_pin_used[CPP_ROWS_RING]; int rows_pin_k;
  double* per_tree; int per_L; float per_alpha, per_eps;
  float* per_maxp; float* per_beta;
  int32_t* per_rows; float* per_w;
  int32_t* per_list; float* per_vals;
  NStepWords* nstep_dev; int nstep_n; float nstep_discount;
  ShiftWords* shift_dev; int32_t* shift_out; int shift_pad, shift_H, shift_W; uint64_t shift_seed;
  Arena arena;
};
static size_t replay_esz(const cpp_replay* r) { return r->store_dtype == CPP_U8 ? 1 : sizeof(__half); }

constexpr int NORM_PARTS = 64;

struct OpGraph {
  struct Op { bool is_gemm; GemmArgs g; std::function<int()> fn; std::vector<int> deps; bool done; };
  std::vector<Op> ops;
  int gemm(const GemmArgs& g, std::initializer_list<int> deps) {
    Op o; o.is_gemm = true; o.g = g; o.done = false;
    for (int d : deps) if (d >= 0) o.deps.push_back(d);
    ops.push_back(o); return (int)ops.size() - 1;
  }
  int fn(std::function<int()> f, std::initializer_list<int> deps) {
    Op o; o.is_gemm = false; o.fn = f; o.done = false; memset(&o.g, 0, sizeof(o.g));
    for (int d : deps) if (d >= 0) o.deps.push_back(d);
    ops.push_back(o); return (int)ops.size() - 1;
  }
  int run(cpp_ctx* ctx, int skip = -1) {
    size_t remaining = ops.size();
    if (skip >= 0 && skip < (int)ops.size() && !ops[skip].done) { ops[skip].done = true; --remaining; }
    std::vector<int> ready; std::vector<GemmArgs> batch;
    while (remaining) {
      ready.clear(); batch.clear();
      for (size_t i = 0; i < ops.size(); ++i) {
        if (ops[i].done) continue;
        bool ok = true;
        for (int d : ops[i].deps) if (!ops[d].done) { ok = false; break; }
        if (ok) ready.push_back((int)i);
      }
      if (ready.empty()) { cpp_set_error("OpGraph: dependency cycle"); return CPP_ERR_STATE; }
      static const bool dbg = cpp_switch_set("CPP_OPGRAPH_DEBUG");
      if (dbg) {
        fprintf(stderr, "[opgraph] level:");
        for (int i : ready) {
          if (ops[i].is_gemm) fprintf(stderr, " gemm#%d(M%d N%d K%d e%d)", i, ops[i].g.M, ops[i].g.N, ops[i].g.K, ops[i].g.epi);
          else fprintf(stderr, " fn#%d", i);
        }
        fprintf(stderr, "\n");
      }
      for (int i : ready) if (!ops[i].is_gemm) RC(ops[i].fn());
      for (int i : ready) ops[i].done = true;
      remaining -= ready.size();
      for (int i : ready) if (ops[i].is_gemm) batch.push_back(ops[i].g);
      if (!batch.empty()) RC(launch_gemm_batch(ctx, batch.data(), (int)batch.size()));
    }
    return CPP_OK;
  }
};

struct GraphKey {
  int B = 0, nb = 0; uint64_t seed = 0, replay_uid = 0, comm_uid = 0, gen = 0;
  bool operator==(const GraphKey& o) const {
    return B == o.B && nb == o.nb && seed == o.seed && replay_uid == o.replay_uid && comm_uid == o.comm_uid && gen == o.gen;
  }
};
enum StepRan { STEP_EAGER, STEP_CAPTURED, STEP_REPLAYED, STEP_CAPTURE_FAILED };
struct StepGraph {
  hipGraph_t g = nullptr; hipGraphExec_t e = nullptr; bool ok = false; GraphKey key;
  StepGraph() = default;
  StepGraph(const StepGraph&) = delete;
  StepGraph& operator=(const StepGraph&) = delete;
  ~StepGraph() { drop(); }
  bool hit(const GraphKey& k) const { return ok && key == k; }
  void drop();
  int capture(cpp_ctx* ctx, const GraphKey& k, const std::function<int()>& body);
  int launch(cpp_ctx* ctx);
  int rebuild(cpp_ctx* ctx, const GraphKey& k, const std::function<int()>& body, StepRan* ran);
};
template <class Body>
int run_step_graph(cpp_ctx* ctx, StepGraph& G, const GraphKey& key, Body&& body, StepRan* ran = nullptr, bool eager = false) {
  StepRan how_;
  StepRan& how = ran ? *ran : how_;
  how = STEP_EAGER;
  if (ctx->prof || eager) return body();
  if (!G.hit(key)) return G.rebuild(ctx, key, body, &how);
  how = STEP_REPLAYED;
  return G.launch(ctx);
}
struct DpGraph {
  StepGraph graph; bool refused = false; char reason[256] = "";
  int mode(uint64_t gen) const { return refused ? 2 : (graph.ok && graph.key.gen == gen ? 1 : 0); }
};
int dp_graph_refused(DpGraph& D, const char* learner);
template <class Body>
int run_dp_graph(cpp_ctx* ctx, DpGraph& D, const GraphKey& key, const char* learner, Body&& body, StepRan* ran = nullptr) {
  StepRan how_;
  StepRan& how = ran ? *ran : how_;
  const int rc = run_step_graph(ctx, D.graph, key, body, &how, D.refused);
  return (rc && how == STEP_CAPTURE_FAILED) ? dp_graph_refused(D, learner) : rc;
}

static const int kFwdKid[3] = {K_CONV1_FWD, K_CONV2_FWD, K_CONV3_FWD};
static const int kDwKid[3] = {K_CONV1_DW, K_CONV2_DW, K_CONV3_DW};
static const int kDxKid[3] = {-1, K_CONV2_DX, K_CONV3_DX};

int gemm(cpp_ctx* ctx, const float* A, long sAm, long sAk, const float* Bm, long sBk, long sBn, float* C, long ldc, int M, int N, int K, int epi, const float* Y = nullptr, long ldy = 0, int accumulate = 0);
ConvArgs conv_fwd_args(cpp_net* n, Workspace& w, int i, const void* state, int dtype, const float* white, int B, int* mode, long white_bstride = 0);
void conv_dy_desc(cpp_net* n, Workspace& w, int i, ConvArgs& a, int B);
ConvArgs conv_dw_args(cpp_net* n, Workspace& w, int i, const void* state, int dtype, const float* white, int B, int* mode);
ConvArgs conv_dx_args(cpp_net* n, Workspace& w, int i, int B);
BnNet bn_net_desc(cpp_net* n, Workspace& w, int i);
BnBatch bn_batch(cpp_net* const* nets, int nn, int i, int B);
bool trunk_b16(const cpp_net* n, int dtype, int B, long white_bstride);
int net_forward_trunk(cpp_net* n, Workspace& w, const void* state, int dtype, const float* white, int B, long white_bstride = 0);
int nets_forward_trunk_fused(cpp_ctx* ctx, cpp_net* const* nets, int nn, const void* const* sts, const float* const* whs, int first_target, int dt, int B);
int nets_forward_trunk_bn(cpp_ctx* ctx, cpp_net* const* nets, int nn, const void* const* states, const float* const* whites, int dtype, int B);
GemmArgs mk_gemm(const float* A, long sAm, long sAk, const float* Bm, long sBk, long sBn, float* C, long ldc, int M, int N, int K, int epi);
GemmArgs mk_gemm(const float* A, long sAm, long sAk, const float* Bm, long sBk, long sBn, float* C, long ldc, int M, int N, int K, int epi, const float* Y, long ldy);
void set_dropout(GemmArgs& g, cpp_net* n, int l);
int relu_grad_epi(const cpp_net* n, int producer_layer);
int bump_dropout(cpp_net* n);
int net_forward_fc(cpp_net* n, Workspace& w, int from, int B, const float* action);
int net_backward_conv(cpp_net* n, Workspace& w, int B, const void* state, int dtype, const float* white);
int nets_backward_conv(cpp_ctx* ctx, cpp_net* const* nets, int nn, int B, const void* state, int dtype, const float* white);
int net_backward(cpp_net* n, Workspace& w, int B, bool want_params, float* d_action, const void* state, int dtype, const float* white, int start_layer = -2);
GemmArgs fc_fwd_args(cpp_net* n, Workspace& w, int l, int B);
GemmArgs fc_dw_args(cpp_net* n, Workspace& w, int l, int B, const float* dz);
GemmArgs fc_dx_args(cpp_net* n, int l, int B, const float* dz, long dz_ld, int col0, int ncols, float* C, long ldc, int epi, const float* Y, long ldy);
GemmArgs twin_fwd_args(cpp_net* n, Workspace& w, int l, int B);
GemmArgs twin_dw_args(cpp_net* n, Workspace& w, int l, int B);
GemmArgs twin_dx_args(cpp_net* n, Workspace& w, int l, int B);
int twin_forward_fc(cpp_net* n, Workspace& w, int B);
inline float* fc_last_out(const Workspace& w) { return w.logits ? w.logits : w.out; }
int dist_expect(cpp_net* n, Workspace& w, int B, float* dz);
int gauss_mean(cpp_net* n, Workspace& w, int B, float* m_out = nullptr, float* ls_out = nullptr);
int batch_stats(cpp_ctx* ctx, const void* s0, const void* s1, int dtype, long elems, int B, int C, double* part, float* white);
int batch_ensure_stats(cpp_batch* b, int C);
uint64_t replay_next_uid();
int nstep_refuse(const cpp_replay* r, float discount, const char* who);
int train_entry_checks(const char* who, const cpp_replay* r, int B, int maxB, long state_elems, int A, float discount, const int* n_batches = nullptr,
                       bool nstep = true);
GatherArgs replay_gather_args(cpp_replay* r, int B, const int32_t* rows_dev, uint64_t seed, const uint64_t* counter_dev, int channels, cpp_batch* out, bool direct, int* C_out,
                              bool augment = true);
int replay_sample_finish(cpp_replay* r, int B, int C, int channels, cpp_batch* out, uint64_t* bump = nullptr, bool* bumped = nullptr);
int replay_sample_device(cpp_replay* r, int B, const int32_t* rows_dev, uint64_t seed, const uint64_t* counter_dev, int channels, cpp_batch* out, bool direct = false,
                         uint64_t* bump = nullptr, bool* bumped = nullptr, bool augment = true);
int replay_stage_rows(cpp_replay* r, const int32_t* idxs, int n, const char* who);
PerArgs per_args(const cpp_replay* r);
int per_refuse(const cpp_replay* r, const char* who);
int replay_upload_rows(cpp_replay* r, const int32_t* idxs, int n, const char* who);
const float* white_of(cpp_batch* b, int which, int C);
bool direct_replay_ok(cpp_net* a, cpp_replay* r, int B);

struct cpp_comm {
  cpp_ctx* ctx; ncclComm_t comm; int rank, world;
  uint64_t uid;
  hipStream_t side;
  hipEvent_t ev_fc, ev_bwd, ev_done;
  double* scratch;
};
#define CPP_COMM_SCRATCH_WORDS 8
#define NCCL_CHECK(expr)                                                                   \
  do {                                                                                     \
    ncclResult_t _r = (expr);                                                              \
    if (_r != ncclSuccess) {                                                               \
      cpp_set_error("%s:%d: %s -> %s", __FILE__, __LINE__, #expr, ncclGetErrorString(_r)); \
      return CPP_ERR_HIP;                                                                  \
    }                                                                                      \
  } while (0)

struct SqScope {
  cpp_ctx* c; int* cnt; int lists;
  SqScope(cpp_ctx* c_, int* cnt_, int lists_, std::initializer_list<int> groups, bool on) : c(c_), cnt(cnt_), lists(lists_) {
    for (int l = 0; l < lists; ++l) cnt[l] = 0;
    if (!on) return;
    for (int l = 0; l < 2; ++l) c->sq_n[l] = l < lists ? 0 : -1;
    int k = 0;
    for (int g : groups) c->sq_conv_group[k++] = g;
  }
  ~SqScope() {
    bool all = true;
    for (int l = 0; l < lists; ++l) all = all && c->sq_n[l] > 0;
    for (int l = 0; l < lists && all; ++l) cnt[l] = c->sq_n[l];
    c->sq_n[0] = c->sq_n[1] = -1;
    for (int& g : c->sq_conv_group) g = -1;
  }
};
GemmArgs sq_gemm(cpp_ctx* ctx, int list, GemmArgs g);
struct SlotScope {
  cpp_net* n[4]; int nn = 0;
  SlotScope(const cpp_batch* b, std::initializer_list<cpp_net*> s1, std::initializer_list<cpp_net*> s2) {
    for (cpp_net* x : s1) { n[nn++] = x; if (b->direct_store) x->img_slot = b->slot[0]; }
    for (cpp_net* x : s2) { n[nn++] = x; if (b->direct_store) x->img_slot = b->slot[1]; }
  }
  ~SlotScope() { for (int k = 0; k < nn; ++k) n[k]->img_slot = nullptr; }
};
struct PerScope {
  const float** w; std::function<int()>* hook;
  PerScope(const float** w_, std::function<int()>* hook_, const cpp_replay* r) : w(w_), hook(hook_) { *w = r->per_tree ? r->per_w : nullptr; }
  ~PerScope() { *w = nullptr; *hook = nullptr; }
};
struct RideScope {
  cpp_ctx* c;
  explicit RideScope(cpp_ctx* c_) : c(c_) {}
  ~RideScope() { c->ride = nullptr; c->st_ride = nullptr; }
  void arm(GatherArgs* ga, const cpp_batch* b, int store_dtype, bool direct, bool at_dw) {
    if (direct) { ga->out_slot[0] = b->slot_alt[0]; ga->out_slot[1] = b->slot_alt[1]; }
    c->ride = ga; c->ride_done = false; c->ride_dtype = store_dtype; c->ride_at_dw = at_dw;
  }
  void arm_stats(const StatsRide* sr) { c->st_ride = sr; c->st_ride_done = false; }
  bool rode() const { return c->ride != nullptr && c->ride_done; }
  bool tables_done() const { return c->st_ride != nullptr && c->st_ride_done && rode(); }
};

struct NextBatch { const cpp_batch* b = nullptr; int B = 0, C = 0; long elems = 0; bool tables_done = false; };
StatsRide next_stats_ride(cpp_ctx* ctx, const NextBatch& nx);
void opt_next_stats(cpp_ctx* ctx, OptSegs& s, const NextBatch& nx);
bool conv1_opens_params(const cpp_net* n);
void opt_img_net(OptSegs& s, int j, cpp_net* n, int seg, int col, const NextBatch& nx);
void opt_img_built(const OptSegs& s, cpp_net* const* nets, const NextBatch& nx);

struct MinibatchLoop {
  cpp_ctx* ctx; cpp_replay* r; cpp_batch* step_batch;
  cpp_net* trunk;
  const float** per_w; std::function<int()>* per_hook;
  const float* td;
  const int* skip_if_set = nullptr;
  bool draws_bump = false;
  bool ride_ok = true;
  bool stats_switch = false;
  std::function<int()> gradients;
  std::function<int(bool more, const NextBatch& next)> apply;
};
int run_minibatches(const MinibatchLoop& L, int B, int n_batches, const int32_t* rows_dev, uint64_t seed);
int step_allreduce(cpp_ctx* ctx, cpp_comm* comm, float* grads, size_t n);
bool route_check(cpp_ctx* ctx, uint64_t* epoch, uint64_t* gen, std::initializer_list<cpp_net*> nets);
struct Readback { void* dst; const void* src; size_t bytes; };
int read_back(cpp_ctx* ctx, std::initializer_list<Readback> items, bool through_ctx = false);
int add_fc_backward(OpGraph& G, cpp_net* n, Workspace& w, int B, int start, int dep, int list, int skip_dx = -1);
```

### cartpoleplusplus_amd/csrc/rt_replay.cpp

```cpp
#include "rt_internal.h"

static int per_write(cpp_replay* r, const int32_t* rows, int n, const float* abs_td);

extern "C" int cpp_batch_create(cpp_ctx* ctx, int max_batch, int64_t state_elems, int action_dim, cpp_batch** out) {
  ARG_CHECK(ctx && out, "cpp_batch_create: NULL argument");
  ARG_CHECK(max_batch >= 1 && state_elems >= 1 && action_dim >= 1, "cpp_batch_create: bad sizes");
  HIP_CHECK(hipSetDevice(ctx->device));
  cpp_batch* b = new cpp_batch();
  b->arena.stream = ctx->stream;
  b->ctx = ctx; b->maxB = max_batch; b->B = 0; b->elems = state_elems; b->A = action_dim; b->dtype = CPP_F16; b->stats_C = 0;
  int rc = 0;
  for (int k = 0; k < 2 && !rc; ++k) rc = b->arena.alloc(&b->s[k], (size_t)max_batch * state_elems * sizeof(float), false);
  if (!rc) rc = dalloc(b->arena, &b->a, (size_t)max_batch * action_dim);
  if (!rc) rc = dalloc(b->arena, &b->r, (size_t)max_batch);
  if (!rc) rc = dalloc(b->arena, &b->m, (size_t)max_batch);
  if (!rc) rc = dalloc(b->arena, &b->white, (size_t)4 * CPP_MAX_CHANNELS);
  if (!rc) rc = dalloc(b->arena, &b->part, (size_t)2 * max_batch * 2 * CPP_MAX_CHANNELS);
  b->direct_store = nullptr;
  for (int k = 0; k < 2 && !rc; ++k) rc = dalloc(b->arena, &b->slot[k], (size_t)max_batch);
  for (int k = 0; k < 2 && !rc; ++k) rc = dalloc(b->arena, &b->slot_alt[k], (size_t)max_batch);
  if (rc) { b->arena.release(); delete b; return rc; }
  *out = b;
  return CPP_OK;
}
// ... 35 lines not shown
  if (action) HIP_CHECK(hipMemcpyAsync(action, b->a, (size_t)b->B * b->A * sizeof(float), hipMemcpyDeviceToHost, st));
  if (reward) HIP_CHECK(hipMemcpyAsync(reward, b->r, (size_t)b->B * sizeof(float), hipMemcpyDeviceToHost, st));
  if (mask) HIP_CHECK(hipMemcpyAsync(mask, b->m, (size_t)b->B * sizeof(float), hipMemcpyDeviceToHost, st));
  HIP_CHECK(hipStreamSynchronize(st));
  return CPP_OK;
}

int batch_ensure_stats(cpp_batch* b, int C) {
  if (C <= 0 || b->stats_C == C) return CPP_OK;
  RC(batch_stats(b->ctx, b->s[0], b->s[1], b->dtype, b->elems, b->B, C, b->part, b->white));
  b->stats_C = C;
  return CPP_OK;
}


static uint16_t f16_of_code(int k) {
  const double d = (double)k / 255.0;
  const uint16_t h0 = __half_as_ushort(__float2half((float)d));
  uint16_t best = h0; double berr = 1e9;
  for (int delta = -1; delta <= 1; ++delta) {
    const int hb = (int)h0 + delta;
    if (hb < 0 || hb > 0x7bff) continue;
    const double err = fabs((double)__half2float(__ushort_as_half((uint16_t)hb)) - d);
    if (err < berr || (err == berr && (hb & 1) == 0)) { berr = err; best = (uint16_t)hb; }
  }
  return best;
}

static int replay_create(cpp_ctx* ctx, int buffer_size, int state_slots, int64_t state_elems, int action_dim, int store_dtype,
                         cpp_replay** out) {
  ARG_CHECK(ctx && out, "cpp_replay_create: NULL argument");
  ARG_CHECK(buffer_size >= 1 && state_elems >= 1 && action_dim >= 1, "cpp_replay_create: bad sizes");
  ARG_CHECK(state_slots >= buffer_size + 1, "cpp_replay_create: %d state slots for %d rows", state_slots, buffer_size);
  ARG_CHECK(store_dtype == CPP_F16 || store_dtype == CPP_U8, "cpp_replay_create: store dtype %d", store_dtype);
  ARG_CHECK(store_dtype != CPP_U8 || state_elems % 8 == 0, "cpp_replay_create: the 8-bit store needs state_elems %% 8 == 0");
  HIP_CHECK(hipSetDevice(ctx->device));
  cpp_replay* r = new cpp_replay();
  r->arena.stream = ctx->stream;
  r->ctx = ctx; r->rows = buffer_size; r->slots = state_slots; r->A = action_dim; r->size = 0; r->elems = state_elems;
  r->store_dtype = store_dtype;
  r->slot_stats = nullptr; r->stats_C = 0; r->stats_cap = 0; r->sampled = false; r->slot_list = nullptr; r->slot_list_cap = 0;
  r->rows_pin = nullptr; r->rows_pin_k = 0; memset(r->rows_pin_used, 0, sizeof(r->rows_pin_used)); memset(r->rows_pin_ev, 0, sizeof(r->rows_pin_ev));
  r->per_tree = nullptr; r->per_L = 0; r->per_alpha = r->per_eps = 0.f; r->per_maxp = r->per_beta = nullptr;
  r->per_rows = nullptr; r->per_w = nullptr; r->per_list = nullptr; r->per_vals = nullptr;
  r->nstep_dev = nullptr; r->nstep_n = 1; r->nstep_discount = 0.f;
  r->shift_dev = nullptr; r->shift_out = nullptr; r->shift_pad = r->shift_H = r->shift_W = 0; r->shift_seed = 0;
  r->stage = nullptr; r->stage_cap = 0; r->pinned = nullptr; r->pinned_cap = 0; r->pinned_busy = false; r->lut = nullptr; r->bad = nullptr;
  HIP_CHECK(hipEventCreateWithFlags(&r->pinned_free, hipEventDisableTiming));
  int rc = r->arena.alloc(&r->store, (size_t)state_slots * state_elems * replay_esz(r), false);
  if (!rc) rc = dalloc(r->arena, &r->s1, (size_t)buffer_size);
  if (!rc) rc = dalloc(r->arena, &r->s2, (size_t)buffer_size);
  if (!rc) rc = dalloc(r->arena, &r->rows_in, (size_t)65536);
  if (!rc) rc = dalloc(r->arena, &r->rows_out, (size_t)65536);
  if (!rc) rc = dalloc(r->arena, &r->action, (size_t)buffer_size * action_dim);
  if (!rc) rc = dalloc(r->arena, &r->reward, (size_t)buffer_size);
  if (!rc) rc = dalloc(r->arena, &r->mask, (size_t)buffer_size);
  if (!rc) rc = dalloc(r->arena, &r->counter, (size_t)1);
  if (!rc) rc = dalloc(r->arena, &r->counter_adhoc, (size_t)1);
  if (!rc) rc = dalloc(r->arena, &r->size_dev, (size_t)1);
  if (!rc) {
    rc = r->arena.alloc((void**)&r->lut, 256 * sizeof(__half), false);
    if (!rc) rc = r->arena.alloc((void**)&r->bad, sizeof(int), true);
    if (!rc) {
      for (int k = 0; k < 256; ++k) r->lut_host[k] = f16_of_code(k);
      if (hipMemcpy(r->lut, r->lut_host, sizeof(r->lut_host), hipMemcpyHostToDevice) != hipSuccess) rc = CPP_ERR_HIP;
    }
  }
  if (rc) { r->arena.release(); delete r; return rc; }
  r->uid = replay_next_uid();
  *out = r;
  return CPP_OK;
}
static int replay_set_size(cpp_replay* r, int size) {
  r->size = size;
  HIP_CHECK(hipMemcpyAsync(r->size_dev, &r->size, sizeof(int32_t), hipMemcpyHostToDevice, r->ctx->stream));
  HIP_CHECK(ctx_sync_stream(r->ctx));
  return CPP_OK;
}
extern "C" int cpp_replay_create(cpp_ctx* ctx, int buffer_size, int state_slots, int64_t state_elems,
                                 int action_dim, cpp_replay** out) {
  return replay_create(ctx, buffer_size, state_slots, state_elems, action_dim, CPP_F16, out);
}
extern "C" int cpp_replay_create_ex(cpp_ctx* ctx, int buffer_size, int state_slots, int64_t state_elems,
                                    int action_dim, int store_dtype, cpp_replay** out) {
  return replay_create(ctx, buffer_size, state_slots, state_elems, action_dim, store_dtype, out);
}
extern "C" int cpp_replay_destroy(cpp_replay* r) {
  if (!r) return CPP_OK;
  (void)hipSetDevice(r->ctx->device);
  (void)ctx_sync_stream(r->ctx);
  if (r->stage) (void)hipFree(r->stage);
  if (r->slot_list) (void)hipFree(r->slot_list);
  if (r->pinned) (void)hipHostFree(r->pinned);
  if (r->rows_pin) (void)hipHostFree(r->rows_pin);
  for (hipEvent_t e : r->rows_pin_ev) if (e) (void)hipEventDestroy(e);
  (void)hipEventDestroy(r->pinned_free);
  r->arena.release(); delete r; return CPP_OK;
}

uint64_t replay_next_uid() { static uint64_t next_uid = 1; return next_uid++; }

extern "C" int cpp_replay_set_stats_channels(cpp_replay* r, int channels) {
  ARG_CHECK(r && channels >= 0 && channels <= CPP_MAX_CHANNELS, "cpp_replay_set_stats_channels: channels %d", channels);
  HIP_CHECK(hipSetDevice(r->ctx->device));
  int C = channels;
  if (C > 0) {
// ... 143 lines not shown
  std::vector<uint8_t> codes(r->store_dtype == CPP_U8 ? (size_t)n * r->elems : 0);
  for (int i = 0; i < n; ++i) {
    ARG_CHECK(slots[i] >= 0 && slots[i] < r->slots, "cpp_replay_read_states: slot %d", slots[i]);
    if (r->store_dtype == CPP_U8)
      HIP_CHECK(hipMemcpyAsync(codes.data() + (size_t)i * r->elems, (const uint8_t*)r->store + (size_t)slots[i] * r->elems,
                               (size_t)r->elems, hipMemcpyDeviceToHost, st));
    else
      HIP_CHECK(hipMemcpyAsync((__half*)out_f16 + (size_t)i * r->elems, (const __half*)r->store + (size_t)slots[i] * r->elems,
                               (size_t)r->elems * sizeof(__half), hipMemcpyDeviceToHost, st));
  }
  HIP_CHECK(hipStreamSynchronize(st));
  if (r->store_dtype == CPP_U8) {
    uint16_t* o = (uint16_t*)out_f16;
    for (size_t i = 0; i < codes.size(); ++i) o[i] = r->lut_host[codes[i]];
  }
  return CPP_OK;
}

int replay_upload_rows(cpp_replay* r, const int32_t* idxs, int n, const char* who) {
  for (int i = 0; i < n; ++i)
    ARG_CHECK(idxs[i] >= 0 && idxs[i] < r->size, "%s: index %d outside [0,%d)", who, idxs[i], r->size);
  HIP_CHECK(hipMemcpyAsync(r->rows_in, idxs, (size_t)n * sizeof(int32_t), hipMemcpyHostToDevice, r->ctx->stream));
  return CPP_OK;
}
int replay_stage_rows(cpp_replay* r, const int32_t* idxs, int n, const char* who) {
  ARG_CHECK(n >= 1 && n <= 65536, "%s: %d rows", who, n);
  for (int i = 0; i < n; ++i)
    ARG_CHECK(idxs[i] >= 0 && idxs[i] < r->size, "%s: index %d outside [0,%d)", who, idxs[i], r->size);
  hipStream_t st = r->ctx->stream;
  if (n > CPP_ROWS_RING_SLOT) {
    HIP_CHECK(hipMemcpyAsync(r->rows_in, idxs, (size_t)n * sizeof(int32_t), hipMemcpyHostToDevice, st));
    HIP_CHECK(hipStreamSynchronize(st));
    return CPP_OK;
  }
  if (!r->rows_pin) {
    HIP_CHECK(hipHostMalloc((void**)&r->rows_pin, (size_t)CPP_ROWS_RING * CPP_ROWS_RING_SLOT * sizeof(int32_t), hipHostMallocDefault));
    for (hipEvent_t& e : r->rows_pin_ev) HIP_CHECK(hipEventCreateWithFlags(&e, hipEventDisableTiming));
  }
  const int k = r->rows_pin_k;
  r->rows_pin_k = (k + 1) % CPP_ROWS_RING;
  if (r->rows_pin_used[k]) HIP_CHECK(hipEventSynchronize(r->rows_pin_ev[k]));
  int32_t* slot = r->rows_pin + (size_t)k * CPP_ROWS_RING_SLOT;
  memcpy(slot, idxs, (size_t)n * sizeof(int32_t));
  HIP_CHECK(hipMemcpyAsync(r->rows_in, slot, (size_t)n * sizeof(int32_t), hipMemcpyHostToDevice, st));
  HIP_CHECK(hipEventRecord(r->rows_pin_ev[k], st));
  r->rows_pin_used[k] = true;
  return CPP_OK;
}

GatherArgs replay_gather_args(cpp_replay* r, int B, const int32_t* rows_dev, uint64_t seed, const uint64_t* counter_dev,
                                     int channels, cpp_batch* out, bool direct, int* C_out, bool augment) {
  int C = channels;
  r->sampled = true;
  if (C > 0) {
    int g = 8, c = C; while (c) { int t = g % c; g = c; c = t; }
    if (r->elems % 8 != 0 || C / g > 16 || r->elems % C != 0) C = 0;
  }
  GatherArgs a; memset(&a, 0, sizeof(a));
  a.store[0] = r->store; a.store[1] = r->store; a.s_idx[0] = r->s1; a.s_idx[1] = r->s2; a.lut = r->lut;
  a.rows = rows_dev; a.rows_out = r->rows_out;
  a.action = r->action; a.reward = r->reward; a.mask = r->mask;
  a.out_state[0] = direct ? nullptr : out->s[0]; a.out_state[1] = direct ? nullptr : out->s[1];
  a.out_slot[0] = direct ? out->slot[0] : nullptr; a.out_slot[1] = direct ? out->slot[1] : nullptr;
  out->direct_store = direct ? r->store : nullptr;
  a.slot_stats = (direct && C > 0 && r->slot_stats && r->stats_C == C) ? r->slot_stats : nullptr;
  a.out_action = out->a; a.out_reward = out->r; a.out_mask = out->m;
  a.part = out->part; a.seed = seed; a.counter = counter_dev;
  a.elems = r->elems; a.B = B; a.size = r->size; a.size_ptr = r->size_dev; a.action_dim = r->A; a.C = C;
  a.nstep = r->nstep_dev; a.rows_cap = r->rows;
  if (augment && r->shift_pad > 0 && !direct && C > 0) {
    a.shift = r->shift_dev; a.shifts_out = r->shift_out; a.shift_seed = r->shift_seed;
    a.shift_pad = r->shift_pad; a.shift_H = r->shift_H; a.shift_W = r->shift_W; a.shift_C = r->stats_C;
  }
  *C_out = C;
  return a;
}
int replay_sample_finish(cpp_replay* r, int B, int C, int channels, cpp_batch* out, uint64_t* bump, bool* bumped) {
  out->B = B; out->dtype = CPP_F16; out->stats_C = 0;
  if (bumped) *bumped = false;
  if (C > 0) {
    RC(launch_stats_finalize(r->ctx, out->part, B, 2, C, (double)B * (double)(r->elems / C), out->white, 1e-6, bump, r->ctx->white_max_dev));
    if (bumped && bump) *bumped = true;
    out->stats_C = C;
  } else if (channels > 0) {
    RC(batch_ensure_stats(out, channels));
  }
  return CPP_OK;
}
int replay_sample_device(cpp_replay* r, int B, const int32_t* rows_dev, uint64_t seed, const uint64_t* counter_dev,
                                int channels, cpp_batch* out, bool direct, uint64_t* bump, bool* bumped, bool augment) {
  int C = 0;
  const GatherArgs a = replay_gather_args(r, B, rows_dev, seed, counter_dev, channels, out, direct, &C, augment);
  RC(launch_gather_stats(r->ctx, a, r->store_dtype));
  return replay_sample_finish(r, B, C, channels, out, bump, bumped);
}

extern "C" int cpp_replay_sample(cpp_replay* r, int B, const int32_t* idxs, uint64_t seed, uint64_t counter,
                                 int channels, cpp_batch* out) {
  ARG_CHECK(r && out, "cpp_replay_sample: NULL argument");
  ARG_CHECK(B >= 1 && B <= out->maxB && B <= 65536, "cpp_replay_sample: batch %d outside [1,%d]", B, out->maxB);
  ARG_CHECK(out->elems == r->elems && out->A == r->A, "cpp_replay_sample: batch/replay shapes differ");
  ARG_CHECK(channels >= 0 && channels <= CPP_MAX_CHANNELS, "cpp_replay_sample: channels %d", channels);
  if (r->size <= 0) { cpp_set_error("cpp_replay_sample: replay memory is empty"); return CPP_ERR_STATE; }
  hipStream_t st = r->ctx->stream;
  HIP_CHECK(hipSetDevice(r->ctx->device));
  const int32_t* rows_dev = nullptr;
// ... 156 lines not shown
  HIP_CHECK(hipMemcpyAsync(w, r->per_w, (size_t)B * sizeof(float), hipMemcpyDeviceToHost, r->ctx->stream));
  HIP_CHECK(ctx_sync_stream(r->ctx));
  return CPP_OK;
}

extern "C" int cpp_replay_draw_prioritized(cpp_replay* r, int B, uint64_t seed, int32_t* idxs, float* w) {
  ARG_CHECK(r && r->per_tree, "cpp_replay_draw_prioritized: not a prioritized replay memory");
  ARG_CHECK(B >= 1 && B <= PER_MAX_ROWS, "cpp_replay_draw_prioritized: batch %d outside [1,%d]", B, PER_MAX_ROWS);
  if (r->size <= 0) { cpp_set_error("cpp_replay_draw_prioritized: replay memory is empty"); return CPP_ERR_STATE; }
  HIP_CHECK(hipSetDevice(r->ctx->device));
  PerArgs p = per_args(r);
  p.B = B; p.seed = seed; p.counter = r->counter; p.bump = 1; p.out_rows = r->per_rows; p.out_w = r->per_w;
  RC(launch_per_update_sample(r->ctx, p));
  if (idxs) HIP_CHECK(hipMemcpyAsync(idxs, r->per_rows, (size_t)B * sizeof(int32_t), hipMemcpyDeviceToHost, r->ctx->stream));
  if (w) HIP_CHECK(hipMemcpyAsync(w, r->per_w, (size_t)B * sizeof(float), hipMemcpyDeviceToHost, r->ctx->stream));
  HIP_CHECK(ctx_sync_stream(r->ctx));
  return CPP_OK;
}


extern "C" int cpp_replay_set_n_step(cpp_replay* r, int n, float discount) {
  ARG_CHECK(r, "cpp_replay_set_n_step: NULL argument");
  ARG_CHECK(n >= 1 && n <= NSTEP_MAX, "cpp_replay_set_n_step: n %d outside [1,%d]", n, NSTEP_MAX);
  ARG_CHECK(std::isfinite(discount) && discount >= 0.f, "cpp_replay_set_n_step: discount %g (must be finite and >= 0)", discount);
  HIP_CHECK(hipSetDevice(r->ctx->device));
  if (!r->nstep_dev) {
    HIP_CHECK(ctx_sync_stream(r->ctx));
    RC(dalloc(r->arena, &r->nstep_dev, (size_t)1));
    r->uid = replay_next_uid(); r->sampled = false;
  }
  ++r->write_gen;
  r->nstep_n = n; r->nstep_discount = discount;
  RC(per_write_scalar(r, reinterpret_cast<float*>(&r->nstep_dev->discount), discount));
  float nbits; memcpy(&nbits, &n, sizeof(nbits));
  return per_write_scalar(r, reinterpret_cast<float*>(&r->nstep_dev->n), nbits);
}

extern "C" int cpp_replay_get_n_step(cpp_replay* r, int* n, float* discount) {
  ARG_CHECK(r, "cpp_replay_get_n_step: NULL argument");
  if (n) *n = r->nstep_n;
  if (discount) *discount = r->nstep_discount;
  return CPP_OK;
}

int nstep_refuse(const cpp_replay* r, float discount, const char* who) {
  if (r && r->nstep_n > 1 && memcmp(&r->nstep_discount, &discount, sizeof(float)) != 0) {
    cpp_set_error("%s: the memory folds %d-step returns with discount %.9g, the trainer's discount is %.9g (cpp_replay_set_n_step)", who,
                  r->nstep_n, (double)r->nstep_discount, (double)discount);
    return CPP_ERR_ARG;
  }
  return CPP_OK;
}

int train_entry_checks(const char* who, const cpp_replay* r, int B, int maxB, long state_elems, int A, float discount, const int* n_batches, bool nstep) {
  ARG_CHECK(B >= 1 && B <= maxB, "%s: batch %d outside [1,%d]", who, B, maxB);
  ARG_CHECK(!n_batches || (*n_batches >= 1 && (size_t)*n_batches * B <= 65536), "%s: n_batches %d", who, n_batches ? *n_batches : 0);
  ARG_CHECK(r->elems == state_elems && r->A == A, "%s: replay shape does not match the networks", who);
  if (nstep) RC(nstep_refuse(r, discount, who));
  if (r->size <= 0) { cpp_set_error("%s: replay memory is empty", who); return CPP_ERR_STATE; }
  ARG_CHECK(!r->per_tree || B <= PER_MAX_ROWS, "%s: a prioritized memory takes batches of at most %d rows", who, PER_MAX_ROWS);
  return CPP_OK;
}

extern "C" int cpp_replay_set_random_shift(cpp_replay* r, int H, int W, int pad, uint64_t seed) {
  ARG_CHECK(r, "cpp_replay_set_random_shift: NULL argument");
  ARG_CHECK(r->stats_C > 0, "cpp_replay_set_random_shift: not a pixel memory (cpp_replay_set_stats_channels has not been called with channels > 0)");
  ARG_CHECK(H >= 1 && W >= 1 && (double)H * (double)W * (double)r->stats_C == (double)r->elems,
            "cpp_replay_set_random_shift: H %d x W %d x %d channels is not the state's %ld elements", H, W, r->stats_C, r->elems);
  ARG_CHECK(pad >= 0 && pad <= SHIFT_MAX_PAD && pad < (H < W ? H : W), "cpp_replay_set_random_shift: pad %d outside [0,%d] or >= min(H, W) = %d", pad,
            SHIFT_MAX_PAD, H < W ? H : W);
  ARG_CHECK((long)W * r->stats_C >= 8 && r->elems < (1L << 31), "cpp_replay_set_random_shift: rows of %ld elements (8 at least), states of %ld (2^31 at most)",
            (long)W * r->stats_C, r->elems);
  HIP_CHECK(hipSetDevice(r->ctx->device));
  if (pad == 0 && r->shift_pad == 0) return CPP_OK;
  if (pad > 0 && !r->shift_dev) {
    HIP_CHECK(ctx_sync_stream(r->ctx));
    RC(dalloc(r->arena, &r->shift_dev, (size_t)1));
    RC(dalloc(r->arena, &r->shift_out, (size_t)4 * 65536));
  }
  r->uid = replay_next_uid(); r->sampled = false;
  ++r->write_gen;
  r->shift_pad = pad; r->shift_H = pad ? H : 0; r->shift_W = pad ? W : 0; r->shift_seed = pad ? seed : 0;
  if (pad > 0) {
    HIP_CHECK(hipMemsetAsync(r->shift_dev, 0, sizeof(ShiftWords), r->ctx->stream));
    HIP_CHECK(hipMemsetAsync(r->shift_out, 0, (size_t)4 * 65536 * sizeof(int32_t), r->ctx->stream));
  }
  return CPP_OK;
}

extern "C" int cpp_replay_get_random_shift(cpp_replay* r, int* pad, uint64_t* seed, uint64_t* counter) {
  ARG_CHECK(r, "cpp_replay_get_random_shift: NULL argument");
  if (pad) *pad = r->shift_pad;
  if (seed) *seed = r->shift_seed;
  if (counter) {
    *counter = 0;
    if (r->shift_pad > 0) {
      HIP_CHECK(hipSetDevice(r->ctx->device));
      HIP_CHECK(hipMemcpyAsync(counter, &r->shift_dev->counter, sizeof(uint64_t), hipMemcpyDeviceToHost, r->ctx->stream));
      HIP_CHECK(ctx_sync_stream(r->ctx));
    }
  }
  return CPP_OK;
}

extern "C" int cpp_replay_last_shifts(cpp_replay* r, int B, int32_t* out) {
  ARG_CHECK(r && out && B >= 1 && B <= 65536, "cpp_replay_last_shifts: bad argument");
  if (r->shift_pad <= 0) { cpp_set_error("cpp_replay_last_shifts: random shift is not enabled on this memory"); return CPP_ERR_STATE; }
// ... 20 lines not shown
```

### cartpoleplusplus_amd/csrc/rt_step.cpp

```cpp
#include <utility>
#include "rt_internal.h"

GemmArgs sq_gemm(cpp_ctx* ctx, int list, GemmArgs g) {
  const int tiles = gemm_tiles(g.M, g.N, g.K);
  if (ctx->sq_n[list] >= 0 && ctx->sq_n[list] + tiles <= SQ_REGION) { g.sq_part = ctx->sq_part + list * SQ_REGION + ctx->sq_n[list]; ctx->sq_n[list] += tiles; }
  else ctx->sq_n[list] = -1;
  return g;
}

StatsRide next_stats_ride(cpp_ctx* ctx, const NextBatch& nx) {
  StatsRide sr;
  sr.part = nx.b->part; sr.white = nx.b->white; sr.nparts = nx.B; sr.jobs = 2 * nx.C; sr.C = nx.C;
  sr.count = (double)nx.B * (double)(nx.elems / nx.C); sr.eps = 1e-6; sr.wmax = ctx->white_max_dev;
  return sr;
}
void opt_next_stats(cpp_ctx* ctx, OptSegs& s, const NextBatch& nx) {
  if (!nx.b || nx.C <= 0 || nx.tables_done) return;
  const StatsRide sr = next_stats_ride(ctx, nx);
  s.st_part = sr.part; s.st_white = sr.white; s.st_nparts = sr.nparts; s.st_jobs = sr.jobs; s.st_C = sr.C;
  s.st_count = sr.count; s.st_eps = sr.eps; s.st_wmax = sr.wmax;
}

bool conv1_opens_params(const cpp_net* n) {
  const ConvL& L = n->conv[0];
// ... 3 lines not shown
  const ConvL& L = n->conv[0];
  s.img[j].w = n->params + L.w_off; s.img[j].bias = n->params + L.b_off;
  if (seg >= 0) { s.img_skip[seg] = L.b_off + kConvOut; s.img[j].gw = s.g[seg] + L.w_off; s.img[j].gb = s.g[seg] + L.b_off; }
  s.img[j].rec = reinterpret_cast<unsigned char*>(n->wimg); s.img[j].seg = seg >= 0 ? seg : 0; s.img[j].col = col; s.img[j].nout = kConvOut;
  s.img[j].white = nx.tables_done ? nx.b->white + (long)col * 2 * nx.C : nullptr;
}
void opt_img_built(const OptSegs& s, cpp_net* const* nets, const NextBatch& nx) {
  for (int j = 0; j < s.img_n; ++j) nets[j]->wimg_key = nx.b->white + (long)s.img[j].col * 2 * nx.C;
}

int step_allreduce(cpp_ctx* ctx, cpp_comm* comm, float* grads, size_t n) {
  if (!comm) return CPP_OK;
  prof_begin(ctx);
  NCCL_CHECK(ncclAllReduce(grads, grads, n, ncclFloat, ncclSum, comm->comm, ctx->stream));
  prof_end(ctx, K_ALLREDUCE);
  return CPP_OK;
}

bool route_check(cpp_ctx* ctx, uint64_t* epoch, uint64_t* gen, std::initializer_list<cpp_net*> nets) {
  ctx_route_update(ctx);
  if (*epoch == ctx->kernel_epoch) return false;
  *epoch = ctx->kernel_epoch;
  ++*gen;
  for (cpp_net* n : nets) n->wimg_key = nullptr;
  return true;
}

int read_back(cpp_ctx* ctx, std::initializer_list<Readback> items, bool through_ctx) {
  for (const Readback& i : items)
    if (i.dst) HIP_CHECK(hipMemcpyAsync(i.dst, i.src, i.bytes, hipMemcpyDeviceToHost, ctx->stream));
  if (through_ctx) HIP_CHECK(ctx_sync_stream(ctx));
  else HIP_CHECK(hipStreamSynchronize(ctx->stream));
  return CPP_OK;
}

int run_minibatches(const MinibatchLoop& L, int B, int n_batches, const int32_t* rows_dev, uint64_t seed) {
  cpp_ctx* ctx = L.ctx; cpp_replay* r = L.r; cpp_batch* sb = L.step_batch;
  const int C = L.trunk->spec.pixel ? L.trunk->spec.C : 0;
  const bool direct = direct_replay_ok(L.trunk, r, B);
  static const bool no_ride = cpp_switch_off("CPP_RIDE_GATHER");
  static const bool no_dwride = cpp_switch_off("CPP_RIDE_DW");
  static const bool no_stats_ride = cpp_switch_off("CPP_RIDE_STATS");
  const bool ride_ok = !no_ride && C > 0 && L.ride_ok && (r->store_dtype == CPP_F16 || r->store_dtype == CPP_U8);
  const bool per = r->per_tree != nullptr;
  auto rows_of = [&](int i) -> const int32_t* { return rows_dev ? rows_dev + (size_t)i * B : per ? r->per_rows : nullptr; };
  auto sample = [&](int i) { return replay_sample_device(r, B, rows_of(i), seed, rows_of(i) ? nullptr : r->counter, C, sb, direct); };
  auto per_draw = [&](PerArgs& p, int i, int ahead) {
    p.B = B; p.w_rows = rows_dev ? rows_of(i) : nullptr; p.seed = seed; p.counter = rows_dev ? nullptr : r->counter;
    if (L.draws_bump) p.bump = rows_dev ? 0 : 1;
    else p.counter_add = ahead;
    p.out_rows = r->per_rows; p.out_w = r->per_w;
  };
  PerScope per_scope(L.per_w, L.per_hook, r);
  if (per) {
    PerArgs p = per_args(r);
    per_draw(p, 0, 0);
    RC(launch_per_update_sample(ctx, p));
  }
  RC(sample(0));
  for (int i = 0; i < n_batches; ++i) {
    GatherArgs ga; StatsRide sr; int Cg = 0;
    const bool more = i + 1 < n_batches;
    if (per) {
      PerArgs p = per_args(r);
      p.up_rows = rows_of(i); p.n_up = B; p.up_td = L.td; p.skip_if_set = L.skip_if_set;
      if (more) per_draw(p, i + 1, 1);
      *L.per_hook = [ctx, p] { return launch_per_update_sample(ctx, p); };
    }
    bool rode, tables_done; int rc;
    {
      RideScope ride(ctx);
      if (more && ride_ok) {
        ga = replay_gather_args(r, B, rows_of(i + 1), seed, rows_of(i + 1) ? nullptr : r->counter, C, sb, direct, &Cg);
        ga.counter_add = 1;
        ride.arm(&ga, sb, r->store_dtype, direct, direct && !no_dwride);
      }
      if (ctx->ride && ctx->ride_at_dw && Cg > 0 && !no_stats_ride) {
        sr = next_stats_ride(ctx, NextBatch{sb, B, Cg, r->elems, false});
        ride.arm_stats(&sr);
      }
      rc = L.gradients();
      *L.per_hook = nullptr;
      rode = ride.rode(); tables_done = ride.tables_done();
    }
    if (rode && direct) { std::swap(sb->slot[0], sb->slot_alt[0]); std::swap(sb->slot[1], sb->slot_alt[1]); }
    RC(rc);
    const bool stats_ride = rode && Cg > 0 && !(L.stats_switch && no_stats_ride);
    RC(L.apply(more, stats_ride ? NextBatch{sb, B, Cg, r->elems, tables_done} : NextBatch{}));
    if (more) {
      if (stats_ride) { sb->B = B; sb->dtype = CPP_F16; sb->stats_C = Cg; }
      else if (rode) RC(replay_sample_finish(r, B, Cg, C, sb));
      else RC(sample(i + 1));
    }
  }
  return CPP_OK;
}
```

### include/cartpolepp_abi.h

```cpp
#ifndef CARTPOLEPP_ABI_H
#define CARTPOLEPP_ABI_H

#include <stdint.h>

#ifdef __cplusplus
extern "C" {
#endif

#define CPP_ABI_VERSION 1

enum { CPP_OK = 0, CPP_ERR_ARG = 1, CPP_ERR_HIP = 2, CPP_ERR_STATE = 3, CPP_ERR_NUMERIC = 4 };
enum { CPP_F32 = 0, CPP_F16 = 1,
       CPP_U8 = 2 };
enum { CPP_ACTOR = 0, CPP_CRITIC = 1,
       CPP_HEAD = 2 };
enum { CPP_OPT_SGD = 0, CPP_OPT_MOMENTUM = 1, CPP_OPT_ADAM = 2 };

typedef struct cpp_ctx cpp_ctx;
typedef struct cpp_net cpp_net;
typedef struct cpp_batch cpp_batch;
typedef struct cpp_replay cpp_replay;
typedef struct cpp_ddpg cpp_ddpg;
typedef struct cpp_naf cpp_naf;
typedef struct cpp_comm cpp_comm;
// ... 119 lines not shown
                    cpp_net* target_critic, const cpp_ddpg_hyper* hyper, cpp_ddpg** out);
int cpp_ddpg_destroy(cpp_ddpg* ddpg);
int cpp_ddpg_train_actor(cpp_ddpg* ddpg, cpp_batch* batch);
int cpp_ddpg_train_critic(cpp_ddpg* ddpg, cpp_batch* batch);
int cpp_ddpg_check_loss(cpp_ddpg* ddpg, cpp_batch* batch, float* loss, float* td, float* q);
int cpp_ddpg_q_gradients_wrt_actions(cpp_ddpg* ddpg, cpp_batch* batch, float* dq_da, float* actions,
                                     float* q);
int cpp_ddpg_compute_gradients(cpp_ddpg* ddpg, cpp_batch* batch);
int cpp_ddpg_grad_buffer(cpp_ddpg* ddpg, void** device_ptr, int64_t* n_floats);
int cpp_ddpg_apply_gradients(cpp_ddpg* ddpg, float grad_scale);
int cpp_ddpg_update_targets(cpp_ddpg* ddpg);
int cpp_ddpg_set_optimiser(cpp_ddpg* ddpg, int kind, float momentum, float beta1, float beta2, float epsilon);
int cpp_ddpg_set_target_smoothing(cpp_ddpg* ddpg, float sigma, float clip, uint64_t seed);
int cpp_ddpg_last_target_noise(cpp_ddpg* ddpg, int B, float* eps, uint64_t* n);
int cpp_ddpg_set_policy_delay(cpp_ddpg* ddpg, int delay);
int cpp_ddpg_policy_delay_status(cpp_ddpg* ddpg, int* delay, uint64_t* n, int* held);
int64_t cpp_ddpg_opt_state_size(const cpp_ddpg* ddpg);
int cpp_ddpg_get_opt_state(cpp_ddpg* ddpg, float* m, float* v, int64_t n, uint64_t steps[2]);
int cpp_ddpg_set_opt_state(cpp_ddpg* ddpg, const float* m, const float* v, int64_t n, const uint64_t steps[2]);
int cpp_ddpg_train_step(cpp_ddpg* ddpg, cpp_replay* replay, int B, int n_batches,
                        const int32_t* idxs, uint64_t seed);
int cpp_ddpg_train_rows(cpp_ddpg* ddpg, cpp_replay* replay, int B, const int32_t* idxs);
int cpp_ddpg_sample_and_compute(cpp_ddpg* ddpg, cpp_replay* replay, int B, uint64_t seed);
int cpp_ddpg_last_stats(cpp_ddpg* ddpg, float out[3]);
int cpp_ddpg_last_values(cpp_ddpg* ddpg, int B, float* actions, float* dq_da, float* q, float* td);
int cpp_ddpg_last_twin_values(cpp_ddpg* ddpg, int B, float* q2, float* target_q1, float* target_q2, float* td2);
int cpp_ddpg_last_distribution(cpp_ddpg* ddpg, int B, float* p, float* target_p, float* m);
int cpp_ddpg_set_quantile_target(cpp_ddpg* ddpg, float kappa, int drop_top);
int cpp_ddpg_last_quantiles(cpp_ddpg* ddpg, int B, float* theta, float* sorted_target_theta, float* y);
int cpp_ddpg_set_sac(cpp_ddpg* ddpg, float init_temperature, float target_entropy, float temperature_lr, uint64_t seed);
int cpp_ddpg_last_sac(cpp_ddpg* ddpg, int B, float* eps, float* a, float* logp, float* eps2, float* a2, float* logp2, float* r_soft,
                      float* alpha, float* g_alpha, uint64_t* n, float* dz);
int cpp_ddpg_sac_temperature(cpp_ddpg* ddpg, int set, float* log_alpha, float* m, float* v, uint64_t* step);

#define CPP_COMM_ID_BYTES 128
int cpp_comm_unique_id(void* out, int cap);
int cpp_comm_create(cpp_ctx* ctx, const void* unique_id, int rank, int world, cpp_comm** out);
int cpp_comm_destroy(cpp_comm* comm);
int cpp_comm_info(const cpp_comm* comm, int* rank, int* world);
int cpp_comm_allreduce(cpp_comm* comm, void* device_f32, int64_t n, int average);
int cpp_comm_max_double(cpp_comm* comm, double* value);
int cpp_comm_max_doubles(cpp_comm* comm, double* values, int n);
int cpp_comm_barrier(cpp_comm* comm);
int cpp_ddpg_allreduce_grads(cpp_ddpg* ddpg, cpp_comm* comm);
int cpp_ddpg_average_params(cpp_ddpg* ddpg, cpp_comm* comm);
int cpp_ddpg_dp_train_step(cpp_ddpg* ddpg, cpp_replay* replay, cpp_comm* comm, int B, int n_batches, uint64_t seed,
                           int sync_every, int overlap);
int cpp_naf_sample_and_compute(cpp_naf* naf, cpp_replay* replay, int B, uint64_t seed);
int cpp_naf_allreduce_grads(cpp_naf* naf, cpp_comm* comm);
int cpp_naf_average_params(cpp_naf* naf, cpp_comm* comm);
int cpp_naf_dp_train_step(cpp_naf* naf, cpp_replay* replay, cpp_comm* comm, int B, int n_batches, uint64_t seed,
                          int sync_every);
int cpp_ddpg_dp_status(const cpp_ddpg* ddpg, int* mode, char* reason, int cap);
int cpp_naf_dp_status(const cpp_naf* naf, int* mode, char* reason, int cap);

typedef struct cpp_naf_hyper {
  float discount;
  float gradient_clip;
  float target_update_rate;
  int32_t optimiser;
  float learning_rate;
  float momentum;
  float beta1, beta2, epsilon;
} cpp_naf_hyper;

int cpp_naf_create(cpp_ctx* ctx, cpp_net* value, cpp_net* target_value, cpp_net* mu, cpp_net* l_values,
                   int share, const cpp_naf_hyper* hyper, cpp_naf** out);
int cpp_naf_destroy(cpp_naf* naf);
int cpp_naf_action(cpp_naf* naf, const void* state, int state_dtype, int B, float* out);
int cpp_naf_train(cpp_naf* naf, cpp_batch* batch, float* loss);
int cpp_naf_debug_values(cpp_naf* naf, cpp_batch* batch, float* l_values, float* loss, float* value,
                         float* advantage, float* target_value);
int cpp_naf_compute_gradients(cpp_naf* naf, cpp_batch* batch);
int cpp_naf_grad_buffer(cpp_naf* naf, void** device_ptr, int64_t* n_floats);
int cpp_naf_apply_gradients(cpp_naf* naf, float grad_scale);
int cpp_naf_update_targets(cpp_naf* naf);
int cpp_naf_train_step(cpp_naf* naf, cpp_replay* replay, int B, int n_batches, const int32_t* idxs,
                       uint64_t seed);
int cpp_naf_train_rows(cpp_naf* naf, cpp_replay* replay, int B, const int32_t* idxs, float* loss);
#define CPP_NAF_TICKETS 8
int cpp_naf_train_rows_async(cpp_naf* naf, cpp_replay* replay, int B, const int32_t* idxs, uint64_t* ticket);
int cpp_naf_loss_wait(cpp_naf* naf, uint64_t ticket, float* loss);
int cpp_naf_last_stats(cpp_naf* naf, float out[3]);
int64_t cpp_naf_opt_state_size(const cpp_naf* naf);
int cpp_naf_get_opt_state(cpp_naf* naf, float* m, float* v, int64_t n, uint64_t* step);
int cpp_naf_set_opt_state(cpp_naf* naf, const float* m, const float* v, int64_t n, uint64_t step);
int cpp_naf_clear_numeric_error(cpp_naf* naf);

#ifdef __cplusplus
}
#endif
#endif
```

Baseline: 3122.

## Carry next step's first minibatch gather and target conv1 update across step boundary

The last minibatch of a DDPG step now also gathers the first minibatch of the next step and parks its whitening stats. The next step can then skip its initial sample, using separate warm graph variants keyed on that carry. Target-network soft updates for the conv1 image weights are folded into the optimizer apply kernel through a new TGT template path, which avoids separate target-update work. The price is a lot of cross-call state: slot-set swapping, generation counters to invalidate stale carries, and extra graph variants, so correctness depends on invalidation at every entry point.

After: 3143 (median of 3 runs). About the same (+0.7%).

```diff
diff --git a/cartpoleplusplus_amd/_lib.py b/cartpoleplusplus_amd/_lib.py
--- a/cartpoleplusplus_amd/_lib.py
+++ b/cartpoleplusplus_amd/_lib.py
@@ -161,6 +161,7 @@
     "cpp_naf_dp_train_step": (_I, [_P, _P, _P, _I, _I, _U64, _I]),
     "cpp_naf_clear_numeric_error": (_I, [_P]),
     "cpp_ddpg_dp_status": (_I, [_P, C.POINTER(_I), C.c_char_p, _I]),
+    "cpp_ddpg_step_graphs": (_I, [_P, C.POINTER(_I), C.POINTER(_U64)]),
     "cpp_naf_dp_status": (_I, [_P, C.POINTER(_I), C.c_char_p, _I]),
     "cpp_naf_create": (_I, [_P, _P, _P, _P, _P, _I, C.POINTER(NafHyper), _PP]),
     "cpp_naf_destroy": (_I, [_P]),
diff --git a/cartpoleplusplus_amd/csrc/common.h b/cartpoleplusplus_amd/csrc/common.h
--- a/cartpoleplusplus_amd/csrc/common.h
+++ b/cartpoleplusplus_amd/csrc/common.h
@@ -250,6 +250,7 @@
   int32_t* shifts_out;
   uint64_t shift_seed;
   int shift_pad, shift_H, shift_W, shift_C;
+  int32_t* rows_hand;
 };
 struct NStepWords { int32_t n; float discount; };
 struct ShiftWords { uint64_t counter; uint32_t ticket; uint32_t reserved; };
@@ -319,6 +320,8 @@
            const float* white; float* mw; float* mb; float* vw; float* vb; } img[4];
   uint64_t* bump2;
   const uint64_t* hold[OPT_MAX_SEGS];
+  struct { float* tw; float* tb; } img_tgt[4];
+  unsigned* park; int park_merge;
 };
 __host__ __device__ inline float sgd_update(float p, float g, float scale, float lr) { return __builtin_fmaf(-lr, g * scale, p); }
 __host__ __device__ inline float momentum_accum(float m, float g, float scale, float momentum) { return __builtin_fmaf(momentum, m, g * scale); }
diff --git a/cartpoleplusplus_amd/csrc/conv_rs16.h b/cartpoleplusplus_amd/csrc/conv_rs16.h
--- a/cartpoleplusplus_amd/csrc/conv_rs16.h
+++ b/cartpoleplusplus_amd/csrc/conv_rs16.h
@@ -23,11 +23,12 @@
   float* mw; float* mb; float momentum;
   float* w_out; float* b_out;
   float* vw; float* vb; float beta1, beta2, epsilon;
+  float* tw; float* tb; float tcoeff;
 };
 struct Conv1ImageArgsN { Conv1ImageArgs a[CONV_BATCH_MAX]; int n; };
 
 struct Conv1ImageNoPre { __device__ __forceinline__ float operator()(float gscale, float&) const { return gscale; } };
-template <int CIN, int NPCS = F16_PIECES, typename Pre = Conv1ImageNoPre, bool ADAM = false>
+template <int CIN, int NPCS = F16_PIECES, typename Pre = Conv1ImageNoPre, bool ADAM = false, bool TGT = false>
 __device__ __forceinline__ void conv1_image_body(const Conv1ImageArgs& a, unsigned char* lds_raw, Pre pre = Pre()) {
   typedef Rs16Geom<CIN, NPCS> G;
   constexpr int KS = G::KS, P = G::P, NO = G::NO, NCH = G::NCH, NPC = G::NPC, RK = G::RK;
@@ -77,13 +78,23 @@
         const int i = tid + n * CONV_THREADS;
         if (i < nwts) {
           const AdamElem e = adam_update(wr[n], gr[n], mr[n], vr[n], gscale, lr, a.beta1, a.beta2, a.epsilon);
+          if (TGT && a.tw) { const float t = soft_update_value(a.tw[i], e.p, a.tcoeff); a.tw[i] = t; wst[i] = t; }
+          else {
           a.mw[i] = e.m; a.vw[i] = e.v;
           wst[i] = e.p;
           if (a.w_out) a.w_out[i] = e.p;
+          }
         }
         if ((n & 3) == 3) __builtin_amdgcn_sched_barrier(0);
       }
     } else {
+    float tr[NWT];
+    if (TGT && a.tw) {
+      int i0 = 0;
+      asm volatile("" : "+v"(i0));
+#pragma unroll
+      for (int n = 0; n < NWT; ++n) { const int i = tid + n * CONV_THREADS; tr[n] = a.tw[i < nwts ? i : i0]; }
+    }
 #pragma unroll
     for (int n = 0; n < NWT; ++n) {
       const int i = tid + n * CONV_THREADS;
@@ -91,9 +102,10 @@
         float w = wr[n];
         if (a.gw && a.mw) {
           const float acc = momentum_accum(mr[n], gr[n], gscale, a.momentum);
-          a.mw[i] = acc;
+          if (!(TGT && a.tw)) a.mw[i] = acc;
           w = momentum_step(w, acc, lr);
         } else if (a.gw) w = sgd_update(w, gr[n], gscale, lr);
+        if (TGT && a.tw) { w = soft_update_value(tr[n], w, a.tcoeff); a.tw[i] = w; }
         wst[i] = w;
         if (a.gw && a.w_out) a.w_out[i] = w;
       }
@@ -118,11 +130,12 @@
   if (tid < 16) {
     float bo = (a.bias && tid < nout) ? a.bias[tid] : 0.f;
     if (a.bias && a.gb && tid < nout) {
-      if (ADAM && a.vb) { const AdamElem e = adam_update(bo, a.gb[tid], a.mb[tid], a.vb[tid], gscale_b, lr, a.beta1, a.beta2, a.epsilon); a.mb[tid] = e.m; a.vb[tid] = e.v; bo = e.p; }
-      else if (a.mb) { const float acc = momentum_accum(a.mb[tid], a.gb[tid], gscale_b, a.momentum); a.mb[tid] = acc; bo = momentum_step(bo, acc, lr); }
+      if (ADAM && a.vb) { const AdamElem e = adam_update(bo, a.gb[tid], a.mb[tid], a.vb[tid], gscale_b, lr, a.beta1, a.beta2, a.epsilon); if (!(TGT && a.tb)) { a.mb[tid] = e.m; a.vb[tid] = e.v; } bo = e.p; }
+      else if (a.mb) { const float acc = momentum_accum(a.mb[tid], a.gb[tid], gscale_b, a.momentum); if (!(TGT && a.tb)) a.mb[tid] = acc; bo = momentum_step(bo, acc, lr); }
       else bo = sgd_update(bo, a.gb[tid], gscale_b, lr);
       if (a.b_out) a.b_out[tid] = bo;
     }
+    if (TGT && a.tb && a.bias && tid < nout) { bo = soft_update_value(a.tb[tid], bo, a.tcoeff); a.tb[tid] = bo; }
     biasn[tid] = bo;
   }
   if (tid < CIN) {
diff --git a/cartpoleplusplus_amd/csrc/gather_body.h b/cartpoleplusplus_amd/csrc/gather_body.h
--- a/cartpoleplusplus_amd/csrc/gather_body.h
+++ b/cartpoleplusplus_amd/csrc/gather_body.h
@@ -205,7 +205,10 @@
 
   if (tid == 0 && a.out_slot[which]) a.out_slot[which][b] = slot;
   if (which == 0 && a.s_idx[0] != nullptr) {
-    if (tid == 0 && a.rows_out) a.rows_out[b] = row;
+    if (tid == 0 && a.rows_out) {
+      if (a.rows_hand) a.rows_hand[b] = a.rows_out[b];
+      a.rows_out[b] = row;
+    }
     if (tid < a.action_dim) a.out_action[(long)b * a.action_dim + tid] = a.action[(long)row * a.action_dim + tid];
     if (tid == 64) a.out_reward[b] = NSTEP ? nreward : a.reward[row];
     if (tid == 65) a.out_mask[b] = NSTEP ? nmask : a.mask[row];
diff --git a/cartpoleplusplus_amd/csrc/optim.hip b/cartpoleplusplus_amd/csrc/optim.hip
--- a/cartpoleplusplus_amd/csrc/optim.hip
+++ b/cartpoleplusplus_amd/csrc/optim.hip
@@ -54,7 +54,7 @@
   return tot;
 }
 
-template <bool ADAM>
+template <bool ADAM, bool TGT>
 __global__ __launch_bounds__(OPT_THREADS) void opt_apply_kernel(const OptSegs s, float grad_scale,
                                                                 float clip, const double* part,
                                                                 int nparts, float* norms_out) {
@@ -132,12 +132,14 @@
     const bool slots = gwj && (ADAM || s.kind == OPT_MOMENTUM), adam = ADAM && gwj;
     ia.mw = slots ? s.img[j].mw : nullptr; ia.mb = slots ? s.img[j].mb : nullptr; ia.momentum = s.momentum;
     ia.vw = adam ? s.img[j].vw : nullptr; ia.vb = adam ? s.img[j].vb : nullptr; ia.beta1 = s.beta1; ia.beta2 = s.beta2; ia.epsilon = s.epsilon;
+    ia.tw = TGT ? s.img_tgt[j].tw : nullptr; ia.tb = TGT ? s.img_tgt[j].tb : nullptr; ia.tcoeff = s.tgt_coeff;
+    if (TGT && ia.tw) { ia.w_out = nullptr; ia.b_out = nullptr; }
     switch (s.img_cin) {
-      case 3: conv1_image_body<3, F16_PIECES, decltype(pre), ADAM>(ia, img_lds, pre); break;
-      case 6: conv1_image_body<6, F16_PIECES, decltype(pre), ADAM>(ia, img_lds, pre); break;
-      case 9: conv1_image_body<9, F16_PIECES, decltype(pre), ADAM>(ia, img_lds, pre); break;
-      case 12: conv1_image_body<12, F16_PIECES, decltype(pre), ADAM>(ia, img_lds, pre); break;
-      default: conv1_image_body<18, F16_PIECES, decltype(pre), ADAM>(ia, img_lds, pre); break;
+      case 3: conv1_image_body<3, F16_PIECES, decltype(pre), ADAM, TGT>(ia, img_lds, pre); break;
+      case 6: conv1_image_body<6, F16_PIECES, decltype(pre), ADAM, TGT>(ia, img_lds, pre); break;
+      case 9: conv1_image_body<9, F16_PIECES, decltype(pre), ADAM, TGT>(ia, img_lds, pre); break;
+      case 12: conv1_image_body<12, F16_PIECES, decltype(pre), ADAM, TGT>(ia, img_lds, pre); break;
+      default: conv1_image_body<18, F16_PIECES, decltype(pre), ADAM, TGT>(ia, img_lds, pre); break;
     }
     return;
   }
@@ -171,7 +173,9 @@
     if (blockIdx.x == 0 && norms_out && s.n[seg] > 0) norms_out[s.group[seg]] = norm;
     if (blockIdx.x == 0 && seg == 0 && s.bump) *s.bump += 1;
     if (blockIdx.x == 0 && seg == 0 && s.bump2) *s.bump2 += 1;
+    if (blockIdx.x == 0 && seg == 0 && s.park && s.park_merge && s.pub_wmax) { const unsigned a = *s.pub_wmax, b = s.park[0]; *s.pub_wmax = a > b ? a : b; }
     if (blockIdx.x == 0 && seg == 0 && s.pub_wmax) route_publish_device(s.pub_wmax, s.pub_tag, s.pub_pin);
+    if (blockIdx.x == 0 && seg == 0 && s.park) { s.park[0] = s.park[1]; s.park[1] = 0u; }
   }
   __syncthreads();
   const float sc = sh_scale, lr = sh_lr;
@@ -254,12 +258,16 @@
     }
     static bool attr_done[CPP_MAX_DEVICES] = {};
     if (!attr_done[cpp_dev_slot(ctx)]) {
-      HIP_CHECK(hipFuncSetAttribute((const void*)opt_apply_kernel<false>, hipFuncAttributeMaxDynamicSharedMemorySize, (int)Rs16ImageLds<18>::BYTES));
-      HIP_CHECK(hipFuncSetAttribute((const void*)opt_apply_kernel<true>, hipFuncAttributeMaxDynamicSharedMemorySize, (int)Rs16ImageLds<18>::BYTES));
+      for (const void* f : {(const void*)opt_apply_kernel<false, false>, (const void*)opt_apply_kernel<true, false>,
+                            (const void*)opt_apply_kernel<false, true>, (const void*)opt_apply_kernel<true, true>})
+        HIP_CHECK(hipFuncSetAttribute(f, hipFuncAttributeMaxDynamicSharedMemorySize, (int)Rs16ImageLds<18>::BYTES));
       attr_done[cpp_dev_slot(ctx)] = true;
     }
   }
-  hipLaunchKernelGGL(s.kind == OPT_ADAM ? opt_apply_kernel<true> : opt_apply_kernel<false>, dim3(128, s.nseg + (s.st_part ? 1 : 0) + (img ? 1 : 0)), dim3(OPT_THREADS), lds, ctx->stream, s, grad_scale,
+  const bool tgt_img = img && (s.img_tgt[2].tw || s.img_tgt[3].tw);
+  auto kernel = s.kind == OPT_ADAM ? (tgt_img ? opt_apply_kernel<true, true> : opt_apply_kernel<true, false>)
+                                   : (tgt_img ? opt_apply_kernel<false, true> : opt_apply_kernel<false, false>);
+  hipLaunchKernelGGL(kernel, dim3(128, s.nseg + (s.st_part ? 1 : 0) + (img ? 1 : 0)), dim3(OPT_THREADS), lds, ctx->stream, s, grad_scale,
                      clip, part, nparts, norms_out);
   LAUNCH_CHECK();
   prof_end(ctx, K_CLIP_SGD);
diff --git a/cartpoleplusplus_amd/csrc/rt_core.cpp b/cartpoleplusplus_amd/csrc/rt_core.cpp
--- a/cartpoleplusplus_amd/csrc/rt_core.cpp
+++ b/cartpoleplusplus_amd/csrc/rt_core.cpp
@@ -195,7 +195,7 @@
   if (!rc && err != hipSuccess) { cpp_set_error("hipStreamEndCapture -> %s", hipGetErrorString(err)); rc = CPP_ERR_HIP; }
   if (!rc) rc = [this]() -> int { HIP_CHECK(hipGraphInstantiate(&e, g, nullptr, nullptr, 0)); return CPP_OK; }();
   if (rc) { drop(); return rc; }
-  key = k; ok = true;
+  key = k; ok = true; ++captures;
   return CPP_OK;
 }
 int StepGraph::launch(cpp_ctx* ctx) {
diff --git a/cartpoleplusplus_amd/csrc/rt_ddpg.cpp b/cartpoleplusplus_amd/csrc/rt_ddpg.cpp
--- a/cartpoleplusplus_amd/csrc/rt_ddpg.cpp
+++ b/cartpoleplusplus_amd/csrc/rt_ddpg.cpp
@@ -23,6 +23,11 @@
   int sq_cnt[2];
   int pre_variant;
   int32_t* slot_set[2][2];
+  struct Carry { bool valid; int set, B; uint64_t seed, uid, graph_gen, write_gen, draw_gen; } carry;
+  struct StepEnd { bool carried; int set; } step_end[3];
+  StepGraph wgraph[2];
+  unsigned* park;
+  bool close_in_apply, carry_in_apply, warm_in_apply, carry_built;
   const float* per_w; std::function<int()> per_hook;
   int opt_kind; float opt_momentum, opt_beta1, opt_beta2, opt_epsilon;
   float *opt_m, *opt_v; uint64_t* opt_step;
@@ -132,6 +137,8 @@
   d->epoch = ctx->kernel_epoch;
   d->dp_local = 0; d->sq_cnt[0] = d->sq_cnt[1] = 0;
   d->h_write_gen = 0; d->pre_variant = 0;
+  memset(&d->carry, 0, sizeof(d->carry)); memset(d->step_end, 0, sizeof(d->step_end));
+  d->close_in_apply = d->carry_in_apply = d->warm_in_apply = d->carry_built = false;
   memset(d->slot_set, 0, sizeof(d->slot_set));
   d->heads_grid = d->heads_B = d->loss_parts = d->loss_B = 0;
   d->per_w = nullptr;
@@ -148,6 +155,7 @@
   if (!rc) rc = dalloc(d->arena, &d->loss_norms, (size_t)4);
   if (!rc) rc = dalloc(d->arena, &d->norm_part, (size_t)OPT_MAX_SEGS * NORM_PARTS);
   if (!rc) rc = dalloc(d->arena, &d->heads_part, (size_t)DDPG_HEADS_MAX_WGS);
+  if (!rc) rc = dalloc(d->arena, &d->park, (size_t)2);
   d->twin = critic->twin;
   if (!rc && d->twin) rc = dalloc(d->arena, &d->td2, (size_t)d->maxB);
   d->dist_n = critic->dist_n; d->quant = critic->quant;
@@ -187,7 +195,7 @@
 static void reconfigured(cpp_ddpg* d) { invalidate_graphs(d); d->pre_variant = 0; }
 
 static void after_replay(cpp_ddpg* d, bool step) {
-  if (step) d->pre_variant = 0;
+  if (step) { d->pre_variant = 0; d->carry.valid = false; }
   d->loss_parts = d->heads_grid; d->loss_B = d->heads_B;
 }
 static int step_ran(cpp_ddpg* d, int rc, StepRan how) {
@@ -347,13 +355,16 @@
   OptSegs s; memset(&s, 0, sizeof(s));
   s.bump = bump;
   if (d->tps_pending) { s.bump2 = d->tps_n; d->tps_pending = false; }
-  if (d->targets_in_apply && !nx.b && do_actor && do_critic) {
+  const bool carry = d->carry_in_apply && nx.b, last = !nx.b || carry;
+  if (d->close_in_apply) { s.park = d->park; s.park_merge = d->warm_in_apply ? 1 : 0; }
+  d->close_in_apply = d->carry_in_apply = d->warm_in_apply = false; d->carry_built = false;
+  if (d->targets_in_apply && last && do_actor && do_critic) {
     s.tgt[0] = d->tactor->params; s.tgt[1] = d->tcritic->params; s.tgt_coeff = d->hp.target_update_rate;
     d->tactor->wimg_key = nullptr; d->tcritic->wimg_key = nullptr;
     d->targets_applied = true;
   }
   d->targets_in_apply = false;
-  if (d->publish_in_apply && !nx.b && d->ctx->route_pin_dev) {
+  if (d->publish_in_apply && last && d->ctx->route_pin_dev) {
     s.pub_wmax = d->ctx->white_max_dev; s.pub_tag = d->ctx->route_tag_dev; s.pub_pin = d->ctx->route_pin_dev;
   }
   d->publish_in_apply = false;
@@ -396,6 +407,14 @@
       if (j < 2 && s.kind != OPT_SGD) { s.img[j].mw = s.m[j] + L.w_off; s.img[j].mb = s.m[j] + L.b_off; }
       if (j < 2 && s.kind == OPT_ADAM) { s.img[j].vw = s.v[j] + L.w_off; s.img[j].vb = s.v[j] + L.b_off; }
     }
+    for (int j = 2; j < 4 && s.tgt[j - 2]; ++j) {
+      const ConvL& L = inets[j]->conv[0];
+      s.img[j] = s.img[j - 2];
+      s.img[j].rec = reinterpret_cast<unsigned char*>(inets[j]->wimg); s.img[j].col = 1;
+      s.img[j].white = nx.tables_done ? nx.b->white + (long)2 * nx.C : nullptr;
+      s.img_tgt[j].tw = inets[j]->params + L.w_off; s.img_tgt[j].tb = inets[j]->params + L.b_off;
+    }
+    d->carry_built = carry;
   }
   if (d->sac && do_actor && d->sac_lr > 0.f && d->sac_B > 0) RC(launch_sac_temperature(d->ctx, d->sac_part, d->sac_B, d->sac_lr, d->sac_w, d->sac_step));
   RC(launch_opt_apply(d->ctx, s, grad_scale, d->hp.gradient_clip, d->norm_part, NORM_PARTS, d->loss_norms + 1));
@@ -819,12 +838,26 @@
   return conv1_f16_pipes_ok(a->ctx, C, a->conv[0].H, a->conv[0].W, B, a->spec.use_batch_norm != 0);
 }
 
+static const float* carry_key(const cpp_ddpg* d, int j) { return d->step_batch->white + (long)(j < 2 ? 0 : 1) * 2 * d->actor->spec.C; }
 static int step_body(cpp_ddpg* d, cpp_replay* r, int B, int n_batches, const int32_t* rows_dev, uint64_t seed, bool targets = true,
-                     bool dp = false, cpp_comm* comm = nullptr) {
+                     bool dp = false, cpp_comm* comm = nullptr, int variant = -1, cpp_ddpg::StepEnd* end = nullptr) {
   d->pre_variant = 0;
+  d->carry.valid = false;
   cpp_ctx* ctx = d->ctx;
+  cpp_net* nets4[4] = {d->actor, d->critic, d->tactor, d->tcritic};
+  bool carried = false;
+  if (variant >= 0) {
+    cpp_batch* b = d->step_batch;
+    if (d->slot_set[0][0] == nullptr)
+      for (int k = 0; k < 2; ++k) { d->slot_set[0][k] = b->slot[k]; d->slot_set[1][k] = b->slot_alt[k]; }
+    const int cur = variant == 1 ? 1 : 0;
+    for (int k = 0; k < 2; ++k) { b->slot[k] = d->slot_set[cur][k]; b->slot_alt[k] = d->slot_set[1 - cur][k]; }
+  }
+  for (int j = 0; j < 4; ++j) nets4[j]->wimg_key = variant > 0 ? carry_key(d, j) : nullptr;
   MinibatchLoop L;
   L.ctx = ctx; L.r = r; L.step_batch = d->step_batch; L.trunk = d->actor;
+  static const bool no_tgt_ride_ = cpp_switch_off("CPP_RIDE_TARGETS");
+  L.carry_first = variant >= 0 && targets && !dp && !no_tgt_ride_; L.warm = variant > 0; L.park = d->park; L.carried = &carried;
   L.per_w = &d->per_w; L.per_hook = &d->per_hook; L.td = d->td; L.stats_switch = true;
   L.gradients = [=] {
     d->bump_in_heads = true;
@@ -839,9 +872,12 @@
     d->targets_applied = false;
     d->targets_in_apply = !more && targets && !dp && !no_tgt_ride;
     d->publish_in_apply = !more && (!targets || d->targets_in_apply);
+    d->close_in_apply = !more && variant >= 0 && d->targets_in_apply; d->carry_in_apply = d->close_in_apply && next.b; d->warm_in_apply = variant > 0;
     return apply(d, true, true, (dp && comm) ? 1.0f / (float)comm->world : 1.0f, rows_dev ? nullptr : r->counter, !dp, next);
   };
   RC(run_minibatches(L, B, n_batches, rows_dev, seed));
+  if (end) { end->carried = carried && d->carry_built; end->set = d->step_batch->slot_alt[0] == d->slot_set[0][0] ? 0 : 1; }
+  d->carry_built = false;
   if (targets && d->targets_applied) { d->targets_applied = false; return CPP_OK; }
   if (targets) { ctx->route_rider = true; return cpp_ddpg_update_targets(d); }
   return CPP_OK;
@@ -863,6 +899,7 @@
 
 extern "C" int cpp_ddpg_train_step(cpp_ddpg* d, cpp_replay* r, int B, int n_batches, const int32_t* idxs, uint64_t seed) {
   ARG_CHECK(d && r, "cpp_ddpg_train_step: NULL argument");
+  const uint64_t draw_gen = r->draw_gen;
   RC(train_entry_checks("cpp_ddpg_train_step", r, B, d->maxB, d->actor->state_elems, d->actor->spec.action_dim, d->hp.discount, &n_batches));
   route_check(d);
   cpp_ctx* ctx = d->ctx;
@@ -873,9 +910,29 @@
     return step_body(d, r, B, n_batches, r->rows_in, seed);
   }
   static const bool no_graph = cpp_switch_set("CPP_NO_GRAPH");
+  static const bool no_carry = cpp_switch_off("CPP_CARRY_FIRST");
+  const ConvL* L0 = d->actor->spec.pixel ? &d->actor->conv[0] : nullptr;
+  const bool boundary = !no_carry && !d->sac && !d->dist_n && L0 && B >= 2 && !d->actor->spec.use_batch_norm && !d->critic->spec.use_batch_norm &&
+                        conv_rs16_ok(ctx, L0->Cin, L0->H, L0->W, kConvOut) && conv1_opens_params(d->actor) && conv1_opens_params(d->critic) &&
+                        r->store_dtype == CPP_F16 && direct_replay_ok(d->actor, r, B);
+  const cpp_ddpg::Carry c = d->carry;
+  d->carry.valid = false;
+  bool warm = boundary && c.valid && c.B == B && c.seed == seed && c.uid == r->uid && c.graph_gen == d->graph_gen && c.write_gen == r->write_gen &&
+              c.draw_gen == draw_gen;
+  cpp_net* nets4[4] = {d->actor, d->critic, d->tactor, d->tcritic};
+  for (int j = 0; j < 4 && warm; ++j) warm = nets4[j]->wimg_key == carry_key(d, j);
+  const int v = !boundary ? -1 : !warm ? 0 : c.set == 1 ? 1 : 2;
+  StepGraph& G = v > 0 ? d->wgraph[v - 1] : d->graph;
+  cpp_ddpg::StepEnd& end = d->step_end[v > 0 ? v : 0];
   StepRan how;
-  const int rc = run_step_graph(ctx, d->graph, GraphKey{B, n_batches, seed, r->uid, 0, d->graph_gen}, [&] { return step_body(d, r, B, n_batches, nullptr, seed); }, &how, no_graph);
-  return step_ran(d, rc, how);
+  const int rc = run_step_graph(ctx, G, GraphKey{B, n_batches, seed, r->uid, (uint64_t)(v > 0 ? v : 0), d->graph_gen},
+                                [&] { return step_body(d, r, B, n_batches, nullptr, seed, true, false, nullptr, v, &end); }, &how, no_graph);
+  const int rc2 = step_ran(d, rc, how);
+  if (!rc2 && boundary) {
+    for (int j = 0; j < 4; ++j) nets4[j]->wimg_key = end.carried ? carry_key(d, j) : nullptr;
+    d->carry = cpp_ddpg::Carry{end.carried, end.set, B, seed, r->uid, d->graph_gen, r->write_gen, r->draw_gen};
+  }
+  return rc2;
 }
 
 static int half_step_body(cpp_ddpg* d, cpp_replay* r, int B, uint64_t seed, int variant, int* next, int phase) {
@@ -909,6 +966,8 @@
 
 static int half_step(cpp_ddpg* d, cpp_replay* r, int B, uint64_t seed, bool split, const std::function<int()>& between) {
   cpp_ctx* ctx = d->ctx;
+  d->carry.valid = false;
+  for (cpp_net* n : {d->actor, d->critic, d->tactor, d->tcritic}) n->wimg_key = nullptr;
   if (!d->step_batch) RC(cpp_batch_create(ctx, d->maxB, r->elems, r->A, &d->step_batch));
   if (d->slot_set[0][0] == nullptr)
     for (int k = 0; k < 2; ++k) { d->slot_set[0][k] = d->step_batch->slot[k]; d->slot_set[1][k] = d->step_batch->slot_alt[k]; }
@@ -1069,6 +1128,16 @@
   return CPP_OK;
 }
 
+extern "C" int cpp_ddpg_step_graphs(const cpp_ddpg* d, int* held, uint64_t* captures) {
+  ARG_CHECK(d, "cpp_ddpg_step_graphs: NULL argument");
+  const StepGraph* gs[3] = {&d->graph, &d->wgraph[0], &d->wgraph[1]};
+  int h = 0; uint64_t c = 0;
+  for (const StepGraph* g : gs) { h += g->ok ? 1 : 0; c += g->captures; }
+  if (held) *held = h;
+  if (captures) *captures = c;
+  return CPP_OK;
+}
+
 extern "C" int cpp_ddpg_last_stats(cpp_ddpg* d, float out[3]) {
   ARG_CHECK(d && out, "cpp_ddpg_last_stats: NULL argument");
   double parts[DDPG_HEADS_MAX_WGS];
diff --git a/cartpoleplusplus_amd/csrc/rt_internal.h b/cartpoleplusplus_amd/csrc/rt_internal.h
--- a/cartpoleplusplus_amd/csrc/rt_internal.h
+++ b/cartpoleplusplus_amd/csrc/rt_internal.h
@@ -118,6 +118,8 @@
   uint64_t uid;
   bool sampled;
   uint64_t write_gen;
+  uint64_t draw_gen;
+  int32_t* rows_carry;
   __half* lut; int* bad; uint16_t lut_host[256];
   double* slot_stats; int stats_C, stats_cap; int32_t* slot_list; size_t slot_list_cap;
   void* stage; size_t stage_cap;
@@ -189,6 +191,7 @@
 enum StepRan { STEP_EAGER, STEP_CAPTURED, STEP_REPLAYED, STEP_CAPTURE_FAILED };
 struct StepGraph {
   hipGraph_t g = nullptr; hipGraphExec_t e = nullptr; bool ok = false; GraphKey key;
+  uint64_t captures = 0;
   StepGraph() = default;
   StepGraph(const StepGraph&) = delete;
   StepGraph& operator=(const StepGraph&) = delete;
@@ -260,7 +263,7 @@
 int batch_ensure_stats(cpp_batch* b, int C);
 uint64_t replay_next_uid();
 int nstep_refuse(const cpp_replay* r, float discount, const char* who);
-int train_entry_checks(const char* who, const cpp_replay* r, int B, int maxB, long state_elems, int A, float discount, const int* n_batches = nullptr,
+int train_entry_checks(const char* who, cpp_replay* r, int B, int maxB, long state_elems, int A, float discount, const int* n_batches = nullptr,
                        bool nstep = true);
 GatherArgs replay_gather_args(cpp_replay* r, int B, const int32_t* rows_dev, uint64_t seed, const uint64_t* counter_dev, int channels, cpp_batch* out, bool direct, int* C_out,
                               bool augment = true);
@@ -351,6 +354,7 @@
   bool draws_bump = false;
   bool ride_ok = true;
   bool stats_switch = false;
+  bool carry_first = false, warm = false; unsigned* park = nullptr; bool* carried = nullptr;
   std::function<int()> gradients;
   std::function<int(bool more, const NextBatch& next)> apply;
 };
diff --git a/cartpoleplusplus_amd/csrc/rt_replay.cpp b/cartpoleplusplus_amd/csrc/rt_replay.cpp
--- a/cartpoleplusplus_amd/csrc/rt_replay.cpp
+++ b/cartpoleplusplus_amd/csrc/rt_replay.cpp
@@ -111,6 +111,7 @@
   if (!rc) rc = dalloc(r->arena, &r->s2, (size_t)buffer_size);
   if (!rc) rc = dalloc(r->arena, &r->rows_in, (size_t)65536);
   if (!rc) rc = dalloc(r->arena, &r->rows_out, (size_t)65536);
+  if (!rc) rc = dalloc(r->arena, &r->rows_carry, (size_t)65536);
   if (!rc) rc = dalloc(r->arena, &r->action, (size_t)buffer_size * action_dim);
   if (!rc) rc = dalloc(r->arena, &r->reward, (size_t)buffer_size);
   if (!rc) rc = dalloc(r->arena, &r->mask, (size_t)buffer_size);
@@ -360,6 +361,7 @@
                                      int channels, cpp_batch* out, bool direct, int* C_out, bool augment) {
   int C = channels;
   r->sampled = true;
+  ++r->draw_gen;
   if (C > 0) {
     int g = 8, c = C; while (c) { int t = g % c; g = c; c = t; }
     if (r->elems % 8 != 0 || C / g > 16 || r->elems % C != 0) C = 0;
@@ -622,7 +624,8 @@
   return CPP_OK;
 }
 
-int train_entry_checks(const char* who, const cpp_replay* r, int B, int maxB, long state_elems, int A, float discount, const int* n_batches, bool nstep) {
+int train_entry_checks(const char* who, cpp_replay* r, int B, int maxB, long state_elems, int A, float discount, const int* n_batches, bool nstep) {
+  ++r->draw_gen;
   ARG_CHECK(B >= 1 && B <= maxB, "%s: batch %d outside [1,%d]", who, B, maxB);
   ARG_CHECK(!n_batches || (*n_batches >= 1 && (size_t)*n_batches * B <= 65536), "%s: n_batches %d", who, n_batches ? *n_batches : 0);
   ARG_CHECK(r->elems == state_elems && r->A == A, "%s: replay shape does not match the networks", who);
diff --git a/cartpoleplusplus_amd/csrc/rt_step.cpp b/cartpoleplusplus_amd/csrc/rt_step.cpp
--- a/cartpoleplusplus_amd/csrc/rt_step.cpp
+++ b/cartpoleplusplus_amd/csrc/rt_step.cpp
@@ -79,15 +79,20 @@
     p.out_rows = r->per_rows; p.out_w = r->per_w;
   };
   PerScope per_scope(L.per_w, L.per_hook, r);
+  const bool carry_ok = L.carry_first && !rows_dev && !per && ride_ok && direct && !no_dwride && !no_stats_ride;
+  if (L.carried) *L.carried = false;
+  if (L.warm && !carry_ok) { cpp_set_error("run_minibatches: a carried minibatch on a path that cannot have produced it"); return CPP_ERR_STATE; }
   if (per) {
     PerArgs p = per_args(r);
     per_draw(p, 0, 0);
     RC(launch_per_update_sample(ctx, p));
   }
-  RC(sample(0));
+  if (L.warm) { sb->B = B; sb->dtype = CPP_F16; sb->stats_C = C; sb->direct_store = r->store; }
+  else RC(sample(0));
   for (int i = 0; i < n_batches; ++i) {
     GatherArgs ga; StatsRide sr; int Cg = 0;
     const bool more = i + 1 < n_batches;
+    const bool carry = !more && carry_ok;
     if (per) {
       PerArgs p = per_args(r);
       p.up_rows = rows_of(i); p.n_up = B; p.up_td = L.td; p.skip_if_set = L.skip_if_set;
@@ -97,22 +102,25 @@
     bool rode, tables_done; int rc;
     {
       RideScope ride(ctx);
-      if (more && ride_ok) {
+      if ((more || carry) && ride_ok) {
         ga = replay_gather_args(r, B, rows_of(i + 1), seed, rows_of(i + 1) ? nullptr : r->counter, C, sb, direct, &Cg);
         ga.counter_add = 1;
+        if (carry) { ga.rows_out = r->rows_carry; ga.rows_hand = (L.warm && n_batches == 1) ? r->rows_out : nullptr; }
         ride.arm(&ga, sb, r->store_dtype, direct, direct && !no_dwride);
       }
       if (ctx->ride && ctx->ride_at_dw && Cg > 0 && !no_stats_ride) {
         sr = next_stats_ride(ctx, NextBatch{sb, B, Cg, r->elems, false});
+        if (carry) sr.wmax = L.park + 1;
         ride.arm_stats(&sr);
       }
       rc = L.gradients();
       *L.per_hook = nullptr;
       rode = ride.rode(); tables_done = ride.tables_done();
     }
-    if (rode && direct) { std::swap(sb->slot[0], sb->slot_alt[0]); std::swap(sb->slot[1], sb->slot_alt[1]); }
+    if (rode && direct && !carry) { std::swap(sb->slot[0], sb->slot_alt[0]); std::swap(sb->slot[1], sb->slot_alt[1]); }
     RC(rc);
-    const bool stats_ride = rode && Cg > 0 && !(L.stats_switch && no_stats_ride);
+    const bool stats_ride = rode && Cg > 0 && !(L.stats_switch && no_stats_ride) && (!carry || tables_done);
+    if (carry && L.carried) *L.carried = stats_ride;
     RC(L.apply(more, stats_ride ? NextBatch{sb, B, Cg, r->elems, tables_done} : NextBatch{}));
     if (more) {
       if (stats_ride) { sb->B = B; sb->dtype = CPP_F16; sb->stats_C = Cg; }
diff --git a/include/cartpolepp_abi.h b/include/cartpolepp_abi.h
--- a/include/cartpolepp_abi.h
+++ b/include/cartpolepp_abi.h
@@ -195,6 +195,7 @@
 int cpp_naf_dp_train_step(cpp_naf* naf, cpp_replay* replay, cpp_comm* comm, int B, int n_batches, uint64_t seed,
                           int sync_every);
 int cpp_ddpg_dp_status(const cpp_ddpg* ddpg, int* mode, char* reason, int cap);
+int cpp_ddpg_step_graphs(const cpp_ddpg* ddpg, int* held, uint64_t* captures);
 int cpp_naf_dp_status(const cpp_naf* naf, int* mode, char* reason, int cap);
 
 typedef struct cpp_naf_hyper {
```
